# weiquan/salt

Hardware: AMD Instinct MI355X
Metric: Mreads/s aligned (100 bp SE, GRCh38+snp144) at 1/2/4/8 MI355X vs CPU ref (higher is better)
Workload: dtype u32; 1 GPU; GRCh38-scale synthetic (SURVEY 8d config 3 = BASELINE configs[2]): 3100000000 bp genome in 24 contigs, 14800000 SNPs, k=21, 1000000 x 100 bp SE reads per GPU per step, 8 distinct resident batches rotated, inputs and results resident in HBM; read_len=100, distinct_batches=8, options=default (-s 50 -m 1000, overlap = k), streams_per_gpu=4

## Files before the change

include/salt_gpu.h:

```cpp
#ifndef SALT_GPU_H
#define SALT_GPU_H
#include <stdint.h>
#include <stddef.h>

#ifdef __cplusplus
extern "C" {
#endif

#define SALT_OK              0
#define SALT_E_INVAL        -1
#define SALT_E_HIP          -2
#define SALT_E_NOMEM        -3
#define SALT_E_INDEX        -4
#define SALT_E_CAPACITY     -5
#define SALT_E_DATA         -6

#define SALT_MAX_READ_LEN   512
#define SALT_MAX_HITS       5
#define SALT_MAX_LOCATE     1024
#define SALT_MAX_SEED_SLOTS 512
#define SALT_MAX_CIGAR_OPS  64

typedef struct {
    uint32_t c_primary, c_L2[5], c_seq_len, c_bwt_size;
    const uint32_t *c_bwt;
    uint32_t c_sa_intv, c_n_sa;
    const uint32_t *c_sa;
    uint32_t lkt_len, lkt_n;
    const uint32_t *lkt;
    uint32_t r_text_len, r_inv_sa0, r_cum[6], r_bwt_words;
    const uint32_t *r_bwt;
    uint32_t r_occ_words;   const uint32_t *r_occ;
    uint32_t r_major_words; const uint32_t *r_major;
    uint32_t r_n_sa;        const uint32_t *r_sa;
    uint32_t ref_len;
    const uint32_t *ref;
    int32_t  l_seed;
} salt_host_index_t;

typedef struct {
    int32_t  l_seed;
    int32_t  l_overlap;
    uint32_t max_seed;
    uint32_t max_locate;
    int32_t  max_hits;
    int32_t  seed_only_ref;
    int32_t  collect_counters;
    int32_t  reserved;
} salt_aln_opt_t;

typedef struct {
    uint32_t pos;
    uint8_t  n_diff, is_gap;
    uint16_t strand;
} salt_hit_t;

typedef struct {
    uint32_t pos;
    uint8_t  strand, n_diff, is_gap, mapq;
    int32_t  b0, b1;
    uint16_t seq_start, seq_end;
    uint8_t  n_hits[2];
    uint8_t  n_cigar;
    uint8_t  skipped;
    salt_hit_t hits[2][SALT_MAX_HITS];
    uint8_t  hit_n_cigar[SALT_MAX_HITS];
    uint8_t  pad[3];
    uint16_t cigar[SALT_MAX_CIGAR_OPS];
    uint16_t hit_cigar[SALT_MAX_HITS][SALT_MAX_CIGAR_OPS];
} salt_result_t;

enum { SALT_CTR_LKT, SALT_CTR_OCC_C, SALT_CTR_OCC_R, SALT_CTR_SA_C, SALT_CTR_SA_R, SALT_CTR_VERIFY,
       SALT_CTR_VERIFY_WORDS, SALT_CTR_LV, SALT_CTR_READS, SALT_CTR_BASES, SALT_CTR_LOCI,
       SALT_CTR_T_LOAD, SALT_CTR_T_GATHER, SALT_CTR_T_LOCATE, SALT_CTR_T_SORT, SALT_CTR_T_DEDUP, SALT_CTR_T_VERIFY,
       SALT_CTR_T_SCAN, SALT_CTR_T_GAP, SALT_CTR_T_TAIL, SALT_CTR_HEAVY_READS, SALT_CTR_X0, SALT_CTR_X1, SALT_CTR_X2, SALT_CTR_X3,
       SALT_CTR_LT_SEEDS, SALT_CTR_LT_LOCATE, SALT_CTR_LT_SORT, SALT_CTR_LT_VERIFY, SALT_CTR_LT_OUT, SALT_CTR_LT_SAMPLES,
       SALT_CTR_MAX_HEAVY, SALT_CTR_MAX_GAPFIN,
       SALT_CTR_D_WLKT, SALT_CTR_D_COCC_SEED, SALT_CTR_D_ROCC_SEED, SALT_CTR_D_SA_SEED, SALT_CTR_D_TEXT_SEED,
       SALT_CTR_D_SA_LIGHT, SALT_CTR_D_VERIFY_LIGHT, SALT_CTR_D_OUT_LIGHT, SALT_CTR_D_SA_HEAVY, SALT_CTR_D_VERIFY_HEAVY, SALT_CTR_D_OUT_HEAVY,
       SALT_CTR_D_CTX_ROWS, SALT_CTR_D_CTX_REJECTED,
       SALT_CTR_N };

typedef struct salt_gpu_index salt_gpu_index_t;
typedef struct salt_gpu_ws    salt_gpu_ws_t;

int  salt_gpu_index_attach(const salt_host_index_t *host, int device, salt_gpu_index_t **out);
void salt_gpu_index_detach(salt_gpu_index_t *ix);
int  salt_gpu_index_image(const salt_gpu_index_t *ix, void **dev_ptr, uint64_t *bytes);
int  salt_gpu_index_attach_image(void *dev_ptr, uint64_t bytes, int device, salt_gpu_index_t **out);
int  salt_gpu_index_image_compact(const salt_gpu_index_t *ix, void **dev_ptr, uint64_t *bytes);
int  salt_gpu_index_attach_compact(const void *dev_ptr, uint64_t bytes, int device, salt_gpu_index_t **out);
int  salt_gpu_index_replicate(salt_gpu_index_t *src, const int *devices, int n, salt_gpu_index_t **out);
int  salt_gpu_index_image_copy(const salt_gpu_index_t *ix, void *dst_dev_ptr, uint64_t dst_bytes);

int  salt_gpu_ws_create(salt_gpu_index_t *ix, uint32_t max_reads, uint64_t max_bases, salt_gpu_ws_t **out);
void salt_gpu_ws_destroy(salt_gpu_ws_t *ws);

int  salt_gpu_align_se(salt_gpu_ws_t *ws, const salt_aln_opt_t *opt, uint32_t n_reads,
                       const uint8_t *seqs, const uint32_t *offs, salt_result_t *results);

typedef struct { uint32_t min_tlen, max_tlen; } salt_pe_opt_t;
int  salt_gpu_index_set_pac(salt_gpu_index_t *ix, const uint8_t *pac, uint64_t l_pac);
int  salt_gpu_align_pe(salt_gpu_ws_t *ws, const salt_aln_opt_t *opt, const salt_pe_opt_t *pe, uint32_t n_pairs,
                       const uint8_t *seqs, const uint32_t *offs, salt_result_t *results);
int  salt_gpu_align_pe_resident(salt_gpu_ws_t *ws, const salt_aln_opt_t *opt, const salt_pe_opt_t *pe, uint32_t n_pairs,
                                uint32_t max_read_len, const void *d_seqs, const void *d_offs, void *d_results, void *hip_stream);
int  salt_gpu_ws_pe_overflow(salt_gpu_ws_t *ws, uint32_t *n);
int  salt_gpu_ws_pe_counts(salt_gpu_ws_t *ws, uint32_t out[8]);

typedef struct { int32_t print_xa_cigar, print_nm_md; const char *rg_id; } salt_text_opt_t;
int  salt_gpu_index_set_contigs(salt_gpu_index_t *ix, int32_t n, const int64_t *offsets, const char *const *names);
int  salt_gpu_align_pe_text(salt_gpu_ws_t *ws, const salt_aln_opt_t *opt, const salt_pe_opt_t *pe, const salt_text_opt_t *topt,
                            const char *fastq1, uint64_t n1_bytes, const char *fastq2, uint64_t n2_bytes,
                            const char **sam, uint64_t *sam_bytes, uint32_t *n_pairs);
int  salt_gpu_ws_reserve_text(salt_gpu_ws_t *ws, const salt_aln_opt_t *opt, uint64_t max_block_bytes, uint32_t est_reads, uint32_t max_read_len,
                              uint64_t est_sam_bytes, void *host_sam, uint64_t host_sam_bytes);
int  salt_gpu_align_se_text(salt_gpu_ws_t *ws, const salt_aln_opt_t *opt, const salt_text_opt_t *topt, const char *fastq, uint64_t n_bytes,
                            const char **sam, uint64_t *sam_bytes, uint32_t *n_reads);
int  salt_gpu_ws_set_sam_bgzf(salt_gpu_ws_t *ws, int on);
int  salt_gpu_ws_set_sam_bam(salt_gpu_ws_t *ws, int on);
int  salt_gpu_bgzf_deflate(int device, const void *text, uint64_t n_bytes, void *out, uint64_t out_cap, uint64_t *out_bytes);
int  salt_gpu_bgzf_inflate(int device, const void *bgzf, uint64_t n_bytes, void *out, uint64_t out_cap, uint64_t *out_bytes);
int  salt_gpu_ws_inflate_bgzf(salt_gpu_ws_t *ws, const void *blocks, uint64_t n_cbytes, uint32_t n_blocks, const uint32_t *c_off, const uint32_t *u_off);
int  salt_gpu_ws_text_peek(salt_gpu_ws_t *ws, uint64_t off, uint64_t n, void *dst);
int  salt_gpu_align_se_text_dev(salt_gpu_ws_t *ws, const salt_aln_opt_t *opt, const salt_text_opt_t *topt, uint64_t off, uint64_t n_bytes, int add_newline,
                                const char **sam, uint64_t *sam_bytes, uint32_t *n_reads);
int  salt_gpu_host_alloc(uint64_t bytes, void **ptr);
void salt_gpu_host_free(void *ptr);
int  salt_gpu_device_numa_node(int device, int *node);
int  salt_gpu_device_count(int *n);

int  salt_gpu_align_se_resident(salt_gpu_ws_t *ws, const salt_aln_opt_t *opt, uint32_t n_reads,
                                uint32_t max_read_len, const void *d_seqs, const void *d_offs,
                                void *d_results, void *hip_stream);

#define SALT_N_KERNELS 10
int  salt_gpu_ws_timing(salt_gpu_ws_t *ws, int enable);
int  salt_gpu_ws_kernel_ms(salt_gpu_ws_t *ws, double ms[SALT_N_KERNELS], uint32_t *n_calls);

int  salt_gpu_ws_heavy_reads(salt_gpu_ws_t *ws, uint32_t *ids, uint32_t cap, uint32_t *n);

int  salt_gpu_buffer_alloc(int device, uint64_t bytes, void **dev_ptr);
int  salt_gpu_buffer_free(int device, void *dev_ptr);
int  salt_gpu_buffer_equal(int device, const void *a, const void *b, uint64_t bytes, int *equal);

int  salt_gpu_diag_rule(uint32_t n_cases, const uint32_t *pos, const uint8_t *val, const uint32_t *offs, const uint32_t *bound_in,
                        uint32_t L, uint32_t ref_len, int mode, uint32_t *out);

int  salt_gpu_diag_verify(const uint32_t *ref_words, uint32_t ref_len, uint32_t n_cases, const uint8_t *seqs, const uint32_t *offs,
                          const uint32_t *cand, const uint32_t *cand_offs, int mode, uint8_t *out);

int  salt_gpu_ws_queue_counts(salt_gpu_ws_t *ws, uint32_t out[8]);

int  salt_gpu_ws_counters(salt_gpu_ws_t *ws, uint64_t out[SALT_CTR_N]);

int  salt_gpu_diag_lv(const uint32_t *ref_words, uint32_t ref_len, uint32_t n_cases, const uint32_t *pos,
                      const uint32_t *kdiff, const uint8_t *seqs, const uint32_t *offs, int32_t *out4, uint16_t *cigars);

int  salt_gpu_diag_ssw(uint32_t n_cases, const uint8_t *aware, const uint8_t *ref_syms, const uint32_t *ref_offs,
                       const uint8_t *codes, const uint32_t *read_offs, int32_t *out6, uint16_t *cigars, uint16_t *n_cigar);

typedef struct { uint32_t read, offset, pool; uint16_t tlen; uint8_t strand, k; } salt_polish_item_t;
typedef struct salt_gpu_polish salt_gpu_polish_t;
int  salt_gpu_polish_open(int device, const uint8_t *pac, uint64_t l_pac, salt_gpu_polish_t **out);
void salt_gpu_polish_close(salt_gpu_polish_t *p);
int  salt_gpu_polish_lv(salt_gpu_polish_t *p, const uint8_t *codes, const uint32_t *offs, uint32_t n_reads, const salt_polish_item_t *items,
                        uint32_t n_items, const uint8_t *pool, uint32_t pool_stride, uint32_t n_pool, int want_cigar,
                        int32_t *dist, uint16_t *cigars, uint8_t *n_cigar);

int  salt_gpu_polish_sw(salt_gpu_polish_t *p, const uint8_t *codes, const uint32_t *offs, uint32_t n_reads, const salt_polish_item_t *items,
                        uint32_t n_items, int want_cigar, int32_t *score, int32_t *read_span, uint16_t *cigars, uint16_t *n_cigar);

int  salt_gpu_suffix_array(int device, const uint8_t *text, uint64_t n, int bits, uint32_t *sa_out);
uint64_t salt_gpu_idx_c_bwt_words(uint64_t n);
int  salt_gpu_idx_build_c(int device, const uint8_t *text, uint64_t n, uint32_t sa_intv, uint32_t *primary, uint32_t L2[5],
                          uint32_t *bwt, uint32_t *sa, uint32_t *lkt, uint32_t lkt_len);
int  salt_gpu_idx_build_r(int device, const uint8_t *rtext, uint64_t n, const uint32_t *sharp_off, const uint32_t *sharp_hdr, uint64_t n_sharp,
                          uint32_t cum4, uint32_t *inv_sa0, uint32_t *code, uint64_t code_words, uint32_t *rsa);
const char *salt_gpu_idx_last_error(void);

const char *salt_gpu_last_error(void);
uint32_t    salt_gpu_result_size(void);

#ifdef __cplusplus
}
// ... 3 lines not shown
```

salt_amd/api.py:

```python
import ctypes
import os
from dataclasses import dataclass

import numpy as np

_HERE = os.path.dirname(os.path.abspath(__file__))
LIB_DIR = os.path.join(_HERE, "lib")

MAX_HITS = 5
MAX_CIGAR_OPS = 64
CTR_NAMES = ["lkt", "occ_c", "occ_r", "sa_c", "sa_r", "verify", "verify_words", "lv", "reads", "bases", "loci",
             "t_load", "t_gather", "t_locate", "t_sort", "t_dedup", "t_verify", "t_scan", "t_gap", "t_tail", "heavy_reads", "x0", "x1", "x2", "x3",
             "lt_seeds", "lt_locate", "lt_sort", "lt_verify", "lt_out", "lt_samples", "max_heavy", "max_gapfin",
             "d_wlkt", "d_cocc_seed", "d_rocc_seed", "d_sa_seed", "d_text_seed", "d_sa_light", "d_verify_light", "d_out_light",
             "d_sa_heavy", "d_verify_heavy", "d_out_heavy", "d_ctx_rows", "d_ctx_rejected"]


class SaltError(RuntimeError):
    pass


HIT_DTYPE = np.dtype([("pos", "<u4"), ("n_diff", "u1"), ("is_gap", "u1"), ("strand", "<u2")])
RESULT_DTYPE = np.dtype([
    ("pos", "<u4"), ("strand", "u1"), ("n_diff", "u1"), ("is_gap", "u1"), ("mapq", "u1"),
# ... 411 lines not shown

    def image(self):
        p, n = ctypes.c_void_p(), ctypes.c_uint64()
        _gpu_check(gpu_lib().salt_gpu_index_image(self._ix, ctypes.byref(p), ctypes.byref(n)))
        return p.value, n.value

    def pe_counts(self):
        out = (ctypes.c_uint32 * 8)()
        _gpu_check(gpu_lib().salt_gpu_ws_pe_counts(self._ws, out))
        return list(out)

    def image_compact(self):
        p, n = ctypes.c_void_p(), ctypes.c_uint64()
        _gpu_check(gpu_lib().salt_gpu_index_image_compact(self._ix, ctypes.byref(p), ctypes.byref(n)))
        return p.value, n.value

    def image_copy(self, dst_ptr, dst_bytes):
        _gpu_check(gpu_lib().salt_gpu_index_image_copy(self._ix, dst_ptr, dst_bytes))

    def timing(self, enable=True):
        _gpu_check(gpu_lib().salt_gpu_ws_timing(self._ws, 1 if enable else 0))

    def kernel_ms(self):
        ms = (ctypes.c_double * len(KERNELS))()
        n = ctypes.c_uint32()
        _gpu_check(gpu_lib().salt_gpu_ws_kernel_ms(self._ws, ms, ctypes.byref(n)))
        return dict(zip(KERNELS, list(ms))), n.value

    def queue_counts(self):
        out = (ctypes.c_uint32 * 8)()
        _gpu_check(gpu_lib().salt_gpu_ws_queue_counts(self._ws, out))
        return list(out)

    def heavy_reads(self):
        n = ctypes.c_uint32()
        ids = np.zeros(self.max_reads, dtype=np.uint32)
        _gpu_check(gpu_lib().salt_gpu_ws_heavy_reads(self._ws, ids.ctypes.data, len(ids), ctypes.byref(n)))
        return ids[:n.value]

    def alnse_core1(self, opt, seqs, offs):
        seqs = np.ascontiguousarray(seqs, dtype=np.uint8)
        offs = np.ascontiguousarray(offs, dtype=np.uint32)
        n = len(offs) - 1
        res = np.zeros(n, dtype=RESULT_DTYPE)
        co = opt._c()
        done = 0
        while done < n:
            m = min(self.max_reads, n - done)
            while m > 1 and int(offs[done + m]) - int(offs[done]) > self.max_bases:
                m //= 2
            o = (offs[done:done + m + 1] - offs[done]).astype(np.uint32)
            s = seqs[int(offs[done]):int(offs[done + m])]
            _gpu_check(gpu_lib().salt_gpu_align_se(self._ws, ctypes.byref(co), m, s.ctypes.data, o.ctypes.data,
                                                   res[done:].ctypes.data))
            done += m
        return res

    def alnpe_core1(self, opt, index, seqs, offs):
        seqs = np.ascontiguousarray(seqs, dtype=np.uint8)
        offs = np.ascontiguousarray(offs, dtype=np.uint32)
        n = len(offs) - 1
        if n % 2:
            raise SaltError("paired end needs an even number of reads")
        lib = gpu_lib()
        if not getattr(self, "_pac_set", False):
            pac, l_pac = index.pac()
            _gpu_check(lib.salt_gpu_index_set_pac(self._ix, pac, l_pac))
            self._pac_set = True
        res = np.zeros(n, dtype=RESULT_DTYPE)
        co, pe = opt._c(), opt._pe()
        done = 0
        cap = self.max_reads & ~1
        while done < n:
            m = min(cap, n - done)
            while m > 2 and int(offs[done + m]) - int(offs[done]) > self.max_bases:
                m = (m // 2) & ~1
            o = (offs[done:done + m + 1] - offs[done]).astype(np.uint32)
            s = seqs[int(offs[done]):int(offs[done + m])]
            _gpu_check(lib.salt_gpu_align_pe(self._ws, ctypes.byref(co), ctypes.byref(pe), m // 2, s.ctypes.data,
                                             o.ctypes.data, res[done:].ctypes.data))
            done += m
        return res

    def set_pac(self, index):
        if not getattr(self, "_pac_set", False):
            pac, l_pac = index.pac()
            _gpu_check(gpu_lib().salt_gpu_index_set_pac(self._ix, pac, l_pac))
            self._pac_set = True

    def set_contigs(self, index):
        cs = index.contigs()
        offs = (ctypes.c_int64 * len(cs))(*[c[0] for c in cs])
        names = (ctypes.c_char_p * len(cs))(*[c[2] for c in cs])
        lib = gpu_lib()
        lib.salt_gpu_index_set_contigs.argtypes = [ctypes.c_void_p, ctypes.c_int32, ctypes.c_void_p, ctypes.c_void_p]
        _gpu_check(lib.salt_gpu_index_set_contigs(self._ix, len(cs), offs, names))

    def set_sam_bgzf(self, on=True):
        gpu_lib().salt_gpu_ws_set_sam_bgzf.argtypes = [ctypes.c_void_p, ctypes.c_int]
        _gpu_check(gpu_lib().salt_gpu_ws_set_sam_bgzf(self._ws, 1 if on else 0))

    def set_sam_bam(self, on=True):
        gpu_lib().salt_gpu_ws_set_sam_bam.argtypes = [ctypes.c_void_p, ctypes.c_int]
        _gpu_check(gpu_lib().salt_gpu_ws_set_sam_bam(self._ws, 1 if on else 0))

    def align_se_text(self, opt, fastq):
        lib = gpu_lib()
        lib.salt_gpu_align_se_text.argtypes = [ctypes.c_void_p, ctypes.POINTER(_AlnOpt), ctypes.POINTER(_TextOpt), ctypes.c_char_p, ctypes.c_uint64,
                                               ctypes.POINTER(ctypes.c_void_p), ctypes.POINTER(ctypes.c_uint64), ctypes.POINTER(ctypes.c_uint32)]
        fastq = bytes(fastq)
        co, to = opt._c(), _TextOpt(opt.print_xa_cigar, opt.print_nm_md, opt.rg_id.encode() if opt.rg_id else None)
        out, n, reads = ctypes.c_void_p(), ctypes.c_uint64(), ctypes.c_uint32()
        _gpu_check(lib.salt_gpu_align_se_text(self._ws, ctypes.byref(co), ctypes.byref(to), fastq, len(fastq), ctypes.byref(out), ctypes.byref(n), ctypes.byref(reads)))
        return ctypes.string_at(out.value, n.value) if n.value else b"", reads.value

    def align_pe_text(self, opt, index, fastq1, fastq2):
        lib = gpu_lib()
        lib.salt_gpu_align_pe_text.argtypes = [ctypes.c_void_p, ctypes.POINTER(_AlnOpt), ctypes.POINTER(_PeOpt), ctypes.POINTER(_TextOpt), ctypes.c_char_p,
                                               ctypes.c_uint64, ctypes.c_char_p, ctypes.c_uint64, ctypes.POINTER(ctypes.c_void_p), ctypes.POINTER(ctypes.c_uint64),
                                               ctypes.POINTER(ctypes.c_uint32)]
        self.set_pac(index)
        fastq1, fastq2 = bytes(fastq1), bytes(fastq2)
        co, pe, to = opt._c(), opt._pe(), _TextOpt(opt.print_xa_cigar, opt.print_nm_md, opt.rg_id.encode() if opt.rg_id else None)
        out, n, pairs = ctypes.c_void_p(), ctypes.c_uint64(), ctypes.c_uint32()
        _gpu_check(lib.salt_gpu_align_pe_text(self._ws, ctypes.byref(co), ctypes.byref(pe), ctypes.byref(to), fastq1, len(fastq1), fastq2, len(fastq2),
                                              ctypes.byref(out), ctypes.byref(n), ctypes.byref(pairs)))
        return ctypes.string_at(out.value, n.value) if n.value else b"", pairs.value

    def align_pe_resident(self, opt, index, n_pairs, max_read_len, d_seqs, d_offs, d_results, stream=0):
        lib = gpu_lib()
        self.set_pac(index)
        co, pe = opt._c(), opt._pe()
        _gpu_check(lib.salt_gpu_align_pe_resident(self._ws, ctypes.byref(co), ctypes.byref(pe), n_pairs, max_read_len, d_seqs, d_offs,
                                                  d_results, stream))

    def align_resident(self, opt, n_reads, max_read_len, d_seqs, d_offs, d_results, stream=0):
        co = opt._c()
        _gpu_check(gpu_lib().salt_gpu_align_se_resident(self._ws, ctypes.byref(co), n_reads, max_read_len, d_seqs, d_offs,
                                                        d_results, stream))

    def counters(self):
        out = (ctypes.c_uint64 * len(CTR_NAMES))()
        _gpu_check(gpu_lib().salt_gpu_ws_counters(self._ws, out))
        return dict(zip(CTR_NAMES, [int(x) for x in out]))

    def fork(self, max_reads=None, max_bases=None):
        other = GpuAligner.__new__(GpuAligner)
        other._ix, other._owns_ix = self._ix, False
        other._ws = ctypes.c_void_p()
        other.max_reads = max_reads or self.max_reads
        other.max_bases = max_bases or self.max_bases
        other.device = self.device
        other._pac_set = getattr(self, "_pac_set", False)
        _gpu_check(gpu_lib().salt_gpu_ws_create(self._ix, other.max_reads, other.max_bases, ctypes.byref(other._ws)))
        return other

    def close(self):
        lib = gpu_lib()
        if self._ws:
            lib.salt_gpu_ws_destroy(self._ws)
            self._ws = None
        if self._ix and getattr(self, "_owns_ix", True):
            lib.salt_gpu_index_detach(self._ix)
        self._ix = None


# ... 62 lines not shown
```

salt_amd/csrc/salt_align.hip:

```cpp
#include "salt_device.h"
#include "salt_kernels.h"

namespace salt {

#define WSYNC() do { __builtin_amdgcn_fence(__ATOMIC_ACQ_REL, "wavefront"); __builtin_amdgcn_wave_barrier(); \
                     __builtin_amdgcn_fence(__ATOMIC_ACQ_REL, "wavefront"); } while (0)

static constexpr int MAXL = SALT_MAX_READ_LEN;
static constexpr int SLOTS = SALT_MAX_SEED_SLOTS;
static constexpr int MAXLOC = SALT_MAX_LOCATE;
static constexpr int LVK = 31;
static_assert(offsetof(salt_result_t, strand) == 4 && offsetof(salt_result_t, mapq) == 7 && offsetof(salt_result_t, b0) == 8 &&
              offsetof(salt_result_t, b1) == 12 && offsetof(salt_result_t, seq_start) == 16 && offsetof(salt_result_t, seq_end) == 18 &&
              offsetof(salt_result_t, n_hits) == 20 && offsetof(salt_result_t, n_cigar) == 22 && offsetof(salt_result_t, skipped) == 23 &&
              offsetof(salt_result_t, hits) == 24 && sizeof(salt_hit_t) == 8, "salt_result_t header layout");
static constexpr int NHIT = 6;
__device__ __forceinline__ uint32_t mapq_quot(uint32_t x, uint32_t b0)
{
    const uint32_t v = 255u * x;
    return b0 == 1u ? v : b0 == 2u ? v / 2u : b0 == 3u ? v / 3u : v / b0;
}
static constexpr uint32_t INF = 255;

__device__ __forceinline__ uint32_t lane_id() { return threadIdx.x & 63u; }
// ... 282 lines not shown
            return true;
        }
        if (head_n || p0 < m) { row = dead; w.ph = WK_IDLE; return true; }
        w.p0 = p0; w.ph = WK_TEXT;
        return false;
    }
    if (!R && w.ph == WK_TEXT) {
        const uint32_t m = (uint32_t)w.i + 1u;
        bool ok = true;
        for (uint32_t done = 0, piece = 0; done < m && ok; ++piece) {
            const uint32_t cnt = (m - done) > 16u ? 16u : (m - done);
            const uint32_t r0 = s + (m - done - cnt), t0 = w.p0 - done - cnt;
            const uint32_t rel = r0 - (c.wb << 4), rr = rel & 15u;
            const uint64_t vr = rel < 16 ? (((uint64_t)c.w0 << 32) | c.w1) : (((uint64_t)c.w1 << 32) | c.w2);
            const uint32_t xr = (uint32_t)((vr >> (64 - 2 * rr - 2 * cnt)) & ((1ull << (2 * cnt)) - 1ull));
            const uint32_t tr = t0 & 15u;
            const uint64_t vt = piece == 0 ? (((uint64_t)ld.s[0] << 32) | ld.s[1]) : (((uint64_t)ld.t[0] << 32) | ld.t[1]);
            n_aux += 1u << 21;
            const uint32_t xt = (uint32_t)((vt >> (64 - 2 * tr - 2 * cnt)) & ((1ull << (2 * cnt)) - 1ull));
            ok = xr == xt;
            done += cnt;
        }
        row = ok ? make_uint4(w.p0 - m, w.p0 - m, s, 2) : dead; w.ph = WK_IDLE;
        return true;
    }
    const bool head = w.ph == WK_HEAD;
    const uint32_t pos = walk_pos(c, w);
    const bool inr = walk_pos_inreg(c, pos);
    const bool isn = inr ? seed_is_n(c, pos) : ((ld.t[0] >> (31 - (pos & 31u))) & 1u) != 0;
    const uint4 stop = head ? dead : make_uint4(w.k, w.l, s - w.ext, 1);
    if (isn && !(R && !head)) { row = stop; w.ph = WK_IDLE; return true; }
    const uint32_t b = isn ? 4u : inr ? seed_base2(c, pos) : (ld.s[0] >> (30 - 2 * (pos & 15u))) & 3u;
    uint32_t ok, ol;
    if (R) n_occ += r_occ2_eval(ix, ROcc2{ ROccBlk{ ld.a[0], ld.a[1], ld.a[2], ld.a[3] }, ROccBlk{ ld.b[0], ld.b[1], ld.b[2], ld.b[3] } }, w.k, w.l + 1u, b, ok, ol);
    else n_occ += c_occ2_eval(ix, COcc2{ ld.a[0], ld.a[1], ld.b[0], ld.b[1] }, w.k - 1u, w.l, b, ok, ol);
    if (ok + 1u > ol) { row = stop; w.ph = WK_IDLE; return true; }
    { const uint32_t first = R ? pick5(ix.r_cum, b) : pick4(ix.c_L2, b); w.k = first + ok + 1u; w.l = first + ol; }
    if (head) {
        if (--w.i >= 0) { if (!R && c.inreg && sp.resolve_unique && w.k == w.l) w.ph = WK_SA; return false; }
    } else ++w.ext;
    return walk_enter_ext(sp, c, w, row);
}

template <bool R>
__device__ __forceinline__ uint4 seed_walk_rest(const IndexView &ix, const SeedParams &sp, const SeedCtx c, uint32_t k, uint32_t l, int i_top,
                                                uint32_t &n_occ, uint32_t &n_aux)
{
    Walk w; uint4 row = make_uint4(1, 0, 0, 0);
    bool done = seed_walk_begin<R>(sp, c, k, l, i_top, w, row);
    while (!done) { const WalkLoads ld = walk_fetch(seed_walk_issue<R>(ix, sp, c, w)); done = seed_walk_finish<R>(ix, sp, c, w, ld, row, n_occ, n_aux); }
    return row;
}
__device__ __forceinline__ uint4 seed_c_rest(const IndexView &ix, const SeedParams &sp, const SeedCtx c, uint32_t kc, uint32_t lc, int i_top,
                                             uint32_t &n_occ_c, uint32_t &n_aux)
{
    return seed_walk_rest<false>(ix, sp, c, kc, lc, i_top, n_occ_c, n_aux);
}
__device__ __forceinline__ uint4 seed_r_rest(const IndexView &ix, const SeedParams &sp, const SeedCtx c, uint32_t kr, uint32_t lr, int i_top,
                                             uint32_t &n_occ_r)
{
    uint32_t n_aux = 0;
    return seed_walk_rest<true>(ix, sp, c, kr, lr, i_top, n_occ_r, n_aux);
}

static constexpr uint32_t WQ_SEG = 64, WQ_STRIDE = 64;
static constexpr uint32_t WQ_REC = 2;
__global__ void __launch_bounds__(256) __attribute__((amdgpu_waves_per_eu(8, 8)))
k_seed(IndexView ix, SeedParams sp, const uint32_t *__restrict__ tb,
       uint4 *__restrict__ sai_c, uint4 *__restrict__ sai_r, uint4 *__restrict__ wq, uint32_t *__restrict__ wq_cnt, uint32_t wq_seg_cap,
       unsigned long long *__restrict__ ctr)
{
    __shared__ uint32_t q_n[2], q_base[2];
    const uint64_t item = (uint64_t)blockIdx.x * blockDim.x + threadIdx.x, n_items = (uint64_t)sp.n_reads * 2u * sp.spr;
    const uint64_t lt = (1ull << lane_id()) - 1ull;
    uint32_t n_lkt = 0, n_occ_c = 0, n_occ_r = 0;
    if (threadIdx.x < 2) { q_n[threadIdx.x] = 0; q_base[threadIdx.x] = 0; }
    __syncthreads();
    bool pend_c = false, pend_r = false;
    uint32_t pk_c = 0, pl_c = 0, pk_r = 0, pl_r = 0, at_r = 0, at_c = 0;
    uint32_t cw0 = 0, cw1 = 0, cw2 = 0, cn0 = 0, cn1 = 0;
    if (item < n_items) {
        const SeedCtx c = seed_ctx(sp, tb, (uint32_t)item, ix.r_lkt_len);
        cw0 = c.w0; cw1 = c.w1; cw2 = c.w2; cn0 = c.n0; cn1 = c.n1;
        uint4 oc = make_uint4(1, 0, 0, 0), orr = make_uint4(1, 0, 0, 0);
        if (seed_valid(c)) {
            const uint32_t e = c.s + c.k - 1, W = c.W;
            uint32_t x = 0; bool has_n = false;
            const uint32_t a0 = e - W + 1;
            if (c.inreg) {
                const uint32_t rel = a0 - (c.wb << 4), rr = rel & 15u;
                const uint64_t v = rel < 16 ? (((uint64_t)c.w0 << 32) | c.w1) : rel < 32 ? (((uint64_t)c.w1 << 32) | c.w2) : ((uint64_t)c.w2 << 32);
                x = (uint32_t)((v >> (64 - 2 * rr - 2 * W)) & ((1ull << (2 * W)) - 1ull));
                const uint32_t reln = a0 - (c.nb << 5);
                const uint64_t vn = ((uint64_t)c.n0 << 32) | c.n1;
                has_n = ((vn >> (64 - reln - W)) & ((1ull << W) - 1ull)) != 0;
            } else {
                for (uint32_t t = 0; t < W; ++t) { has_n |= seed_is_n(c, a0 + t); x = (x << 2) | seed_base2(c, a0 + t); }
            }
            if (!has_n) {
                const uint4 v = ix.wlkt[2 * (uint64_t)x];
                const uint4 u = ix.wlkt[2 * (uint64_t)x + 1];
                ++n_lkt;
                const int i_top = (int)(c.k - W) - 1;
                if (v.x <= v.y) {
                    const uint32_t m = c.k - W;
                    if (v.x == v.y && c.inreg && sp.resolve_unique && m >= 1 && m <= 16) {
                        const uint32_t rel = c.s - (c.wb << 4), rr = rel & 15u;
                        const uint64_t vr = rel < 16 ? (((uint64_t)c.w0 << 32) | c.w1) : (((uint64_t)c.w1 << 32) | c.w2);
                        const uint32_t mk = m == 16 ? 0xFFFFFFFFu : ((1u << (2 * m)) - 1u);
                        const uint32_t xr = (uint32_t)(vr >> (64 - 2 * rr - 2 * m)) & mk;
                        const uint32_t reln2 = c.s - (c.nb << 5);
                        const uint64_t vn2 = ((uint64_t)c.n0 << 32) | c.n1;
                        const bool head_n = ((vn2 >> (64 - reln2 - m)) & ((1ull << m) - 1ull)) != 0;
                        if (!head_n && u.x >= m && xr == (u.y & mk)) oc = make_uint4(u.x - m, u.x - m, c.s, 2);
                    }
                    else if (v.y == v.x + 1u && c.inreg && sp.resolve_unique && m >= 1 && m <= 16) {
                        const uint32_t rel = c.s - (c.wb << 4), rr = rel & 15u;
                        const uint64_t vr = rel < 16 ? (((uint64_t)c.w0 << 32) | c.w1) : (((uint64_t)c.w1 << 32) | c.w2);
                        const uint32_t mk = m == 16 ? 0xFFFFFFFFu : ((1u << (2 * m)) - 1u);
                        const uint32_t xr = (uint32_t)(vr >> (64 - 2 * rr - 2 * m)) & mk;
                        const uint32_t reln2 = c.s - (c.nb << 5);
                        const uint64_t vn2 = ((uint64_t)c.n0 << 32) | c.n1;
                        const bool head_n = ((vn2 >> (64 - reln2 - m)) & ((1ull << m) - 1ull)) != 0;
                        const bool ok0 = !head_n && u.x >= m && xr == (u.y & mk), ok1 = !head_n && u.z >= m && xr == (u.w & mk);
                        if (ok0 && ok1) { pend_c = true; pk_c = v.x; pl_c = v.y; }
                        else if (ok0) oc = make_uint4(u.x - m, u.x - m, c.s, 2);
                        else if (ok1) oc = make_uint4(u.z - m, u.z - m, c.s, 2);
                    }
                    else {
                        Walk w;
                        if (!seed_walk_begin<false>(sp, c, v.x, v.y, i_top, w, oc)) { pend_c = true; pk_c = v.x; pl_c = v.y; }
                    }
                }
                if (!sp.seed_only_ref) {
                    if (v.z <= v.w) { pend_r = true; pk_r = v.z; pl_r = v.w; }
                }
            }
        }
        sai_c[item] = oc;
        sai_r[item] = orr;
    }
    {
        const uint64_t mr = __ballot(pend_r), mc = __ballot(pend_c);
        uint32_t br = 0, bc = 0;
        if (lane_id() == 0) { if (mr) br = atomicAdd(&q_n[0], (uint32_t)__popcll(mr)); if (mc) bc = atomicAdd(&q_n[1], (uint32_t)__popcll(mc)); }
        br = (uint32_t)__shfl((int)br, 0); bc = (uint32_t)__shfl((int)bc, 0);
        at_r = br + (uint32_t)__popcll(mr & lt); at_c = bc + (uint32_t)__popcll(mc & lt);
    }
    __syncthreads();
    const uint32_t seg = blockIdx.x & (WQ_SEG - 1u);
    if (threadIdx.x < 2 && q_n[threadIdx.x]) q_base[threadIdx.x] = atomicAdd(&wq_cnt[(threadIdx.x * WQ_SEG + seg) * WQ_STRIDE], q_n[threadIdx.x]);
    __syncthreads();
    if (pend_r) {
        uint4 *rec = wq + ((size_t)seg * wq_seg_cap + q_base[0] + at_r) * WQ_REC;
        rec[0] = make_uint4((uint32_t)item, pk_r, pl_r, cn0); rec[1] = make_uint4(cw0, cw1, cw2, cn1);
    }
    if (pend_c) {
        uint4 *rec = wq + (((size_t)WQ_SEG + seg) * wq_seg_cap + q_base[1] + at_c) * WQ_REC;
        rec[0] = make_uint4((uint32_t)item, pk_c, pl_c, cn0); rec[1] = make_uint4(cw0, cw1, cw2, cn1);
    }
    if (ctr) {
        for (int o = 32; o > 0; o >>= 1) {
            n_lkt += __shfl_down(n_lkt, o); n_occ_c += __shfl_down(n_occ_c, o); n_occ_r += __shfl_down(n_occ_r, o);
        }
        if (lane_id() == 0) {
            atomicAdd(ctr + SALT_CTR_LKT, n_lkt & 1023u); atomicAdd(ctr + SALT_CTR_OCC_C, n_occ_c); atomicAdd(ctr + SALT_CTR_OCC_R, n_occ_r);
            atomicAdd(ctr + SALT_CTR_D_WLKT, n_lkt & 1023u); atomicAdd(ctr + SALT_CTR_D_COCC_SEED, n_occ_c); atomicAdd(ctr + SALT_CTR_D_ROCC_SEED, n_occ_r);
            atomicAdd(ctr + SALT_CTR_D_SA_SEED, (n_lkt >> 10) & 2047u); atomicAdd(ctr + SALT_CTR_D_TEXT_SEED, n_lkt >> 21);
        }
    }
}

__global__ void __launch_bounds__(256) __attribute__((amdgpu_waves_per_eu(4, 4)))
k_seed_walk(IndexView ix, SeedParams sp, const uint32_t *__restrict__ tb, uint4 *__restrict__ sai_c, uint4 *__restrict__ sai_r,
            const uint4 *__restrict__ wq, const uint32_t *__restrict__ wq_cnt, uint32_t wq_seg_cap, uint32_t r_first, unsigned long long *__restrict__ ctr)
{
    const uint32_t seg = blockIdx.x & (WQ_SEG - 1u);
    const uint32_t wv = (blockIdx.x / WQ_SEG) * 4u + (uint32_t)__builtin_amdgcn_readfirstlane((int)(threadIdx.x >> 6)), nw = (gridDim.x / WQ_SEG) * 4u;
    const uint64_t lt = (1ull << lane_id()) - 1ull;
    const uint32_t la = r_first ? 0u : 1u, lb = la ^ 1u;
    const uint32_t na = wq_cnt[(la * WQ_SEG + seg) * WQ_STRIDE], nb = wq_cnt[(lb * WQ_SEG + seg) * WQ_STRIDE];
    const uint32_t a0 = (uint32_t)((uint64_t)na * wv / nw), a1 = (uint32_t)((uint64_t)na * (wv + 1u) / nw);
    const uint32_t b0 = (uint32_t)((uint64_t)nb * wv / nw), b1 = (uint32_t)((uint64_t)nb * (wv + 1u) / nw);
    const uint4 *qa = wq + (((size_t)la * WQ_SEG + seg) * wq_seg_cap + a0) * WQ_REC, *qb = wq + (((size_t)lb * WQ_SEG + seg) * wq_seg_cap + b0) * WQ_REC;
    const uint32_t tot_a = a1 - a0, tot = tot_a + (b1 - b0);
    const int i_top = (int)((uint32_t)sp.l_seed - ix.r_lkt_len) - 1;
    uint32_t n_aux = 0, n_sa = 0, n_text = 0, n_occ_c = 0, n_occ_r = 0;
    Walk w; w.ph = WK_IDLE; w.k = w.l = w.ext = w.p0 = 0; w.i = 0;
    SeedCtx c = seed_ctx_geom(sp, tb, 0, ix.r_lkt_len);
    uint32_t item = 0, cur = 0;
    bool is_r = false;
    const uint4 *qp = qa;
    for (;;) {
        const uint64_t idle = __ballot(w.ph == WK_IDLE);
        if (cur >= tot && idle == ~0ull) break;
        if (cur < tot) {
            const uint32_t t = cur + (uint32_t)__popcll(idle & lt);
            if (w.ph == WK_IDLE && t < tot) {
                const bool in_a = t < tot_a;
                qp = in_a ? qa + (size_t)t * WQ_REC : qb + (size_t)(t - tot_a) * WQ_REC; is_r = (in_a ? la : lb) == 0u; w.ph = WK_REC;
            }
            const uint32_t nx = cur + (uint32_t)__popcll(idle);
            cur = nx < tot ? nx : tot;
        }
        WalkReq q = walk_req_none();
        if (w.ph == WK_REC) { q.pa = qp; q.na = WQ_REC; }
        else if (w.ph != WK_IDLE) q = is_r ? seed_walk_issue<true>(ix, sp, c, w) : seed_walk_issue<false>(ix, sp, c, w);
        const WalkLoads ld = walk_fetch(q);
        bool done = false;
        uint4 row = make_uint4(1, 0, 0, 0);
        if (w.ph == WK_REC) {
            item = ld.a[0].x;
            c = seed_ctx_geom(sp, tb, item, ix.r_lkt_len);
            c.w0 = ld.a[1].x; c.w1 = ld.a[1].y; c.w2 = ld.a[1].z; c.n0 = ld.a[0].w; c.n1 = ld.a[1].w;
            done = is_r ? seed_walk_begin<true>(sp, c, ld.a[0].y, ld.a[0].z, i_top, w, row) : seed_walk_begin<false>(sp, c, ld.a[0].y, ld.a[0].z, i_top, w, row);
        } else if (w.ph != WK_IDLE) {
            done = is_r ? seed_walk_finish<true>(ix, sp, c, w, ld, row, n_occ_r, n_aux) : seed_walk_finish<false>(ix, sp, c, w, ld, row, n_occ_c, n_aux);
        }
        if (done && row.x <= row.y) (is_r ? sai_r : sai_c)[item] = row;
        n_sa += (n_aux >> 10) & 2047u; n_text += n_aux >> 21; n_aux = 0;
    }
    if (ctr) {
        for (int o = 32; o > 0; o >>= 1) { n_sa += __shfl_down(n_sa, o); n_text += __shfl_down(n_text, o); n_occ_c += __shfl_down(n_occ_c, o); n_occ_r += __shfl_down(n_occ_r, o); }
        if (lane_id() == 0) {
            atomicAdd(ctr + SALT_CTR_OCC_C, n_occ_c); atomicAdd(ctr + SALT_CTR_OCC_R, n_occ_r);
            atomicAdd(ctr + SALT_CTR_D_COCC_SEED, n_occ_c); atomicAdd(ctr + SALT_CTR_D_ROCC_SEED, n_occ_r);
            atomicAdd(ctr + SALT_CTR_D_SA_SEED, n_sa); atomicAdd(ctr + SALT_CTR_D_TEXT_SEED, n_text);
        }
    }
}

template <int NS> struct SaiListsT { uint32_t sp[2][NS], ep[2][NS], off[2][NS]; };
struct SaiLists { uint32_t *sp[2], *ep[2], *off[2]; };
template <int NS> __device__ __forceinline__ SaiLists sai_ref(SaiListsT<NS> &a) { return SaiLists{ { a.sp[0], a.sp[1] }, { a.ep[0], a.ep[1] }, { a.off[0], a.off[1] } }; }
struct LvTables { short L[LVK][64]; char A[LVK][64]; };
static constexpr int LLV_K = 12;
static constexpr int LLV_TW = 22;
static constexpr int LLV_W = 2 * LLV_K + 3;
static constexpr int LLV_N = 64;
struct LaneLv { uint32_t T[LLV_N * LLV_TW]; uint8_t rows[2][LLV_W][LLV_N]; };
struct LvBytes { uint8_t T[MAXL + 4 + 64]; uint8_t P[MAXL + 64]; };
template <int NS, bool LLV>
struct WaveLdsT {
    static constexpr bool HAS_LLV = LLV;
    static constexpr int N_SLOTS = NS;
    uint32_t pm[2][MAXL / 8];
    union U { SaiListsT<NS> sai; typename std::conditional<LLV, LaneLv, uint32_t>::type llv; LvBytes lvb; } u;
    uint8_t  cand_e[MAXLOC];
    uint32_t loci[MAXLOC];
    uint32_t hit_pos[2][NHIT];
    uint8_t  hit_nd[2][NHIT], hit_gap[2][NHIT];
    uint16_t cig[SALT_MAX_CIGAR_OPS];
    int      n_cig;
    alignas(8) uint8_t cargs[128];
};
typedef WaveLdsT<SLOTS, true> WaveLds;
typedef WaveLdsT<32, false> WaveLdsSmall;
typedef WaveLdsT<1, false> WaveLdsCigar;

struct Sai { uint32_t sp, ep, off; };
__device__ __forceinline__ Sai sai_get(const SaiLists &s, int w, int i) { return Sai{ s.sp[w][i], s.ep[w][i], s.off[w][i] }; }
__device__ __forceinline__ void sai_set(SaiLists &s, int w, int i, Sai v) { s.sp[w][i] = v.sp; s.ep[w][i] = v.ep; s.off[w][i] = v.off; }
__device__ __forceinline__ bool sai_ltv(Sai a, Sai b) { return a.ep - a.sp < b.ep - b.sp; }
__device__ __forceinline__ bool sai_lt(const SaiLists &s, int w, int i, int j) { return sai_ltv(sai_get(s, w, i), sai_get(s, w, j)); }
__device__ __forceinline__ void sai_swap(SaiLists &s, int w, int i, int j) { Sai a = sai_get(s, w, i), b = sai_get(s, w, j); sai_set(s, w, i, b); sai_set(s, w, j, a); }

__device__ void sai_insertsort(SaiLists &s, int w, int lo, int hi)
{
    for (int i = lo + 1; i < hi; ++i)
        for (int j = i; j > lo && sai_lt(s, w, j, j - 1); --j) sai_swap(s, w, j, j - 1);
}

__device__ void sai_combsort(SaiLists &s, int w, int base, int n)
{
    const double shrink = 1.2473309501039786540366528676643;
    int gap = n; bool do_swap;
    do {
        if (gap > 2) { gap = (int)(gap / shrink); if (gap == 9 || gap == 10) gap = 11; }
        do_swap = false;
        for (int i = 0; i < n - gap; ++i)
            if (sai_lt(s, w, base + i + gap, base + i)) { sai_swap(s, w, base + i, base + i + gap); do_swap = true; }
    } while (do_swap || gap > 2);
    if (gap != 1) sai_insertsort(s, w, base, base + n);
}

__device__ __attribute__((noinline)) void sai_introsort(SaiLists &s, int w, int n)
{
    if (n < 1) return;
    if (n == 2) { if (sai_lt(s, w, 1, 0)) sai_swap(s, w, 0, 1); return; }
    int d; for (d = 2; (1 << d) < n; ++d) { }
    d <<= 1;
    int st_l[24], st_r[24], st_d[24], top = 0;
    int lo = 0, hi = n - 1;
    for (;;) {
        if (lo < hi) {
            if (--d == 0) { sai_combsort(s, w, lo, hi - lo + 1); hi = lo; continue; }
            int i = lo, j = hi, k = i + ((j - i) >> 1) + 1;
            if (sai_lt(s, w, k, i)) { if (sai_lt(s, w, k, j)) k = j; }
            else k = sai_lt(s, w, j, i) ? i : j;
            Sai rp = sai_get(s, w, k);
            if (k != hi) sai_swap(s, w, k, hi);
            for (;;) {
                do ++i; while (sai_ltv(sai_get(s, w, i), rp));
                do --j; while (i <= j && sai_ltv(rp, sai_get(s, w, j)));
                if (j <= i) break;
                sai_swap(s, w, i, j);
            }
            sai_swap(s, w, i, hi);
            if (i - lo > hi - i) {
                if (i - lo > 16 && top < 24) { st_l[top] = lo; st_r[top] = i - 1; st_d[top] = d; ++top; }
                lo = hi - i > 16 ? i + 1 : hi;
            } else {
                if (hi - i > 16 && top < 24) { st_l[top] = i + 1; st_r[top] = hi; st_d[top] = d; ++top; }
                hi = i - lo > 16 ? i - 1 : lo;
            }
        } else {
            if (top == 0) { sai_insertsort(s, w, 0, n); return; }
            --top; lo = st_l[top]; hi = st_r[top]; d = st_d[top];
        }
    }
}

__device__ void sort_loci(uint32_t *a, uint32_t n)
{
    if (n < 2) return;
    uint32_t P = 2; while (P < n) P <<= 1;
    for (uint32_t i = n + lane_id(); i < P; i += 64) a[i] = 0xFFFFFFFFu;
    WSYNC();
    for (uint32_t k = 2; k <= P; k <<= 1) {
        for (uint32_t j = k >> 1; j > 0; j >>= 1) {
            for (uint32_t t = lane_id(); t < (P >> 1); t += 64) {
                uint32_t i = ((t & ~(j - 1)) << 1) | (t & (j - 1));
                uint32_t p = i | j;
                uint32_t x = a[i], y = a[p];
                bool up = (i & k) == 0;
                if ((x > y) == up) { a[i] = y; a[p] = x; }
            }
            WSYNC();
        }
    }
}

__device__ __forceinline__ uint32_t dedup_loci(uint32_t *loci, uint32_t n, bool gap_mode, uint32_t L, uint32_t ref_len)
{
    const uint32_t lane = lane_id();
    const uint64_t lt = (1ull << lane) - 1ull;
    uint32_t n_out = 0;
    for (uint32_t b = 0; b < n; b += 64) {
        uint32_t i = b + lane;
        bool keep = false; uint32_t pos = 0;
        if (i < n) {
            pos = loci[i];
            bool dup = i > 0 && loci[i - 1] == pos;
            bool out = gap_mode ? (pos + L + 4 >= ref_len) : (pos >= ref_len);
            keep = !dup && !out;
        }
        uint64_t m = __ballot(keep);
        WSYNC();
        if (keep) loci[n_out + (uint32_t)__popcll(m & lt)] = pos;
        n_out += (uint32_t)__popcll(m);
        WSYNC();
    }
    return n_out;
}

struct CandStats { uint32_t n_cand, n_sa_c, n_sa_r, n_loci; uint32_t in_lds; uint32_t n_ctx_rej, n_ctx_rows; };
struct CandArgs {
    const uint32_t *c_sa, *r_pos; const uint4 *sai_c, *sai_r;
    uint32_t ref_len, spr, max_locate, r, L; int strand; bool gap_mode; unsigned long long *phase;
    uint32_t *loci; uint32_t loci_cap; int pe;
    bool finish;
    const uint4 *r_ctx;
    const uint4 *c_ctx; uint32_t ctx_k;
};

__device__ __forceinline__ CtxRead ctx_read(const uint32_t *pm, uint32_t L, uint32_t off, uint32_t ctx_k)
{
    const int p = ctx_face(lane_id(), off, ctx_a_start(ctx_k));
    const bool v = p >= 0 && p < (int)L;
    const uint32_t nib = v ? (pm[(uint32_t)p >> 3] >> (4u * ((uint32_t)p & 7u))) & 15u : 0u;
    CtxRead rd;
    rd.lo = __ballot(v && ctx_nib_lo(nib));
    rd.hi = __ballot(v && ctx_nib_hi(nib));
    rd.use = __ballot(v && ctx_nib_use(nib));
    return rd;
}
template <bool PE, bool GL, class W>
__device__ __attribute__((noinline)) CandStats build_candidates(W &w)
{
    const CandArgs a = *reinterpret_cast<const CandArgs *>(w.cargs);
    const uint32_t lane = lane_id();
    const uint64_t lt = (1ull << lane) - 1ull;
    const uint32_t L = a.L, r = a.r; const int strand = a.strand; const bool gap_mode = a.gap_mode;
    const gp_u32x4 sai_c = as_global(a.sai_c), sai_r = as_global(a.sai_r);
    struct { gp_u32 c_sa, r_pos; uint32_t ref_len; } ix = { as_global(a.c_sa), as_global(a.r_pos), a.ref_len };
    struct { uint32_t spr, max_locate; } ap = { a.spr, a.max_locate };
    uint32_t n_sa_c = 0, n_sa_r = 0, n_loci_out = 0;
    constexpr bool glob = GL;
    uint32_t *loci = glob ? a.loci : w.loci;
    PhaseClock pc(a.phase);
    const uint64_t base_item = ((uint64_t)r * 2u + (uint32_t)strand) * ap.spr;
    uint32_t n_list[2] = { 0, 0 };
    const uint32_t cap_total = PE ? a.loci_cap : ap.max_locate;
    uint32_t rows = 0;
    for (uint32_t b = 0; b < ap.spr; b += 64) {
        const uint32_t slot = b + lane;
        uint4 v2[2] = { make_uint4(1, 0, 0, 0), make_uint4(1, 0, 0, 0) };
        if (slot < ap.spr) {
            const u32x4_t tc = sai_c[base_item + slot], tr = sai_r[base_item + slot];
            v2[0] = make_uint4(tc.x, tc.y, tc.z, tc.w); v2[1] = make_uint4(tr.x, tr.y, tr.z, tr.w);
        }
#pragma unroll
        for (int which = 0; which < 2; ++which) {
            const uint4 v = v2[which];
            const uint32_t n = n_list[which];
            uint64_t m = __ballot(v.w != 0);
            uint32_t sz = 0;
            if (v.w) {
                uint32_t at = n + (uint32_t)__popcll(m & lt); w.u.sai.sp[which][at] = v.x; w.u.sai.ep[which][at] = v.y; w.u.sai.off[which][at] = v.z | (v.w == 2 ? 0x80000000u : 0u);
                sz = v.y - v.x + 1u;
                if (which == 1 && !PE) { uint32_t skip = sz / 0x40000u; if (skip > 1) sz = (sz + skip - 1) / skip; }
                if (PE && which == 0 && sz > ap.max_locate + 1u) sz = ap.max_locate + 1u;
                if (PE && which == 1 && v.y - v.x > ap.max_locate) sz = (v.y - v.x) / ((v.y - v.x) / ap.max_locate) + 1u;
                if (sz > cap_total) sz = cap_total + 1u;
            }
            for (int o = 32; o > 0; o >>= 1) sz += (uint32_t)__shfl_xor((int)sz, o);
            rows = rows + sz > cap_total ? cap_total + 1u : rows + sz;
            n_list[which] = n + (uint32_t)__popcll(m);
        }
    }
    WSYNC();
    if (rows > cap_total && lane < 2) { SaiLists sl = sai_ref(w.u.sai); sai_introsort(sl, (int)lane, (int)n_list[lane]); }
    const bool pe_in_lds = !glob || rows <= (uint32_t)MAXLOC;
    if (pe_in_lds) loci = w.loci;
    WSYNC();
    pc.stamp(SALT_CTR_T_GATHER);
    uint32_t n = 0, ns = 0, n_ctx_rows = 0;
    bool full = false;
    const gp_u32x4 c_ctx = as_global(a.c_ctx);
    const bool use_ctx = a.c_ctx != nullptr && !gap_mode;
    for (uint32_t i = 0; i < n_list[0] && !full; ++i) {
        const uint32_t sp = w.u.sai.sp[0][i], off = w.u.sai.off[0][i] & 0x7FFFFFFFu;
        const bool located = (w.u.sai.off[0][i] >> 31) != 0;
        uint32_t ep = w.u.sai.ep[0][i];
        if (PE && ep - sp > ap.max_locate) ep = sp + ap.max_locate;
        const bool ctx_here = use_ctx && !located;
        CtxRead rd = { 0, 0, 0 };
        if (ctx_here) rd = ctx_read(w.pm[strand], L, off, a.ctx_k);
        for (uint64_t j0 = sp; j0 <= ep && !full; j0 += 64) {
            pc.add(SALT_CTR_X0, 1);
            uint64_t j = j0 + lane;
            bool in = j <= ep, keep = false, rej = false;
            uint32_t pos = 0;
            if (in) {
                uint32_t sa;
                if (ctx_here) { const u32x4_t rc = c_ctx[j]; sa = rc.x; rej = ctx_reject(make_uint4(rc.x, rc.y, rc.z, rc.w), rd, 3u); }
                else sa = located ? (uint32_t)j : ix.c_sa[j];
                pos = sa - off; keep = !(pos + L > ix.ref_len);
            }
            uint64_t m = __ballot(keep);
            uint32_t rank = (uint32_t)__popcll(m & lt);
            const bool st = keep && !rej && n + rank < cap_total;
            const uint64_t ms = __ballot(st);
            if (st) loci[ns + (uint32_t)__popcll(ms & lt)] = pos;
            ns += (uint32_t)__popcll(ms);
            uint32_t tot = (uint32_t)__popcll(m);
            if (n + tot >= cap_total) {
                uint64_t last = m;
                uint32_t need = cap_total - n;
                for (uint32_t q = 1; q < need; ++q) last &= last - 1;
                uint32_t stop_lane = (uint32_t)__ffsll((long long)last) - 1;
                n_sa_c += stop_lane + 1; if (ctx_here) n_ctx_rows += stop_lane + 1;
                n = cap_total; full = true;
            } else { n += tot; const uint32_t looked = (uint32_t)__popcll(__ballot(in)); n_sa_c += looked; if (ctx_here) n_ctx_rows += looked; }
        }
    }
    pc.stamp(SALT_CTR_X2);
    const gp_u32x4 r_ctx = as_global(a.r_ctx);
    const bool use_rctx = use_ctx && a.r_ctx != nullptr;
    for (uint32_t i = 0; i < n_list[1] && !full; ++i) {
        const uint32_t sp = w.u.sai.sp[1][i], ep = w.u.sai.ep[1][i], off = w.u.sai.off[1][i];
        uint32_t skip = (ep + 1 - sp) / 0x40000u;
        if ((int)skip <= 0) skip = 1;
        if (PE) skip = ep - sp > ap.max_locate ? (ep - sp) / ap.max_locate : 1;
        CtxRead rd = { 0, 0, 0 };
        if (use_rctx) rd = ctx_read(w.pm[strand], L, off, a.ctx_k);
        for (uint64_t j0 = sp; j0 <= ep && !full; j0 += 64ull * skip) {
            pc.add(SALT_CTR_X1, 1);
            uint64_t j = j0 + (uint64_t)lane * skip;
            bool in = j <= ep, keep = false, rej = false;
            uint32_t pos = 0;
            if (in) {
                uint32_t rp;
// ... 516 lines not shown
{
    const uint32_t w0 = pos >> 3, sh = (pos & 7u) * 4u, nwt = (tl + 7) >> 3;
    uint32_t wv[LLV_TW + 1];
#pragma unroll
    for (int j = 0; j <= LLV_TW; ++j) wv[j] = (uint32_t)j <= nwt ? ref[w0 + (uint32_t)j] : 0u;
#pragma unroll
    for (int j = 0; j < LLV_TW; ++j) {
        uint32_t word = 0;
        if ((uint32_t)j < nwt) {
            word = __funnelshift_r(wv[j], wv[j + 1], sh);
            const uint32_t rem = tl - (uint32_t)j * 8;
            if (rem < 8) word &= (1u << (4 * rem)) - 1u;
        }
        T[j] = word;
    }
}

__device__ __forceinline__ uint32_t store_gap_list(const uint32_t *loci, uint32_t n, uint32_t L, uint32_t ref_len, uint32_t *__restrict__ dst)
{
    const uint32_t lane = lane_id();
    const uint64_t lt = (1ull << lane) - 1ull;
    uint32_t n_out = 0;
    for (uint32_t b = 0; b < n; b += 64) {
        const uint32_t i = b + lane;
        const uint32_t pos = i < n ? loci[i] : 0u;
        const bool keep = i < n && !(pos + L + 4 >= ref_len);
        const uint64_t m = __ballot(keep);
        if (keep) dst[n_out + (uint32_t)__popcll(m & lt)] = pos;
        n_out += (uint32_t)__popcll(m);
    }
    return n_out;
}

template <bool PE, bool GL, class W>
__device__ __forceinline__ void align_general(const IndexView ix, const AlignParams ap, W &w, const uint32_t r,
                              const uint32_t *__restrict__ pm,
                              const uint4 *__restrict__ sai_c, const uint4 *__restrict__ sai_r,
                              salt_result_t *__restrict__ results, unsigned long long *__restrict__ ctr,
                              unsigned long long *phase, LvTables *lvtab, const GapBufs g, uint32_t *pe_loci, uint8_t *pe_cand)
{
    const uint32_t lane = lane_id();
    const uint64_t lt = (1ull << lane) - 1ull;
    const uint32_t *rec = pm + (uint64_t)r * ap.pg.pm_stride;
    const uint32_t L = rec[2 * ap.pg.nw8];
    salt_result_t *out = results + r;
    uint32_t c_sa_c = 0, c_sa_r = 0, c_verify = 0, c_vwords = 0, c_lv = 0, c_loci = 0, c_ctx_rej = 0, c_ctx_rows = 0;
    PhaseClock pc(phase);
    const uint64_t rt0 = phase ? __builtin_amdgcn_s_memrealtime() : 0;
    constexpr bool glob = GL;
    uint32_t *loci = glob ? pe_loci : w.loci;
    uint8_t *cand_e = glob ? pe_cand : w.cand_e;
    const uint32_t loci_cap = PE ? PE_LOCI_CAP : (uint32_t)MAXLOC;

    const uint32_t nw = (L + 7) >> 3;
    uint32_t n_amb = 0;
    for (uint32_t t = lane; t < 2 * nw; t += 64) {
        const uint32_t s = t >= nw, j = s ? t - nw : t;
        const uint32_t word = rec[s * ap.pg.nw8 + j];
        w.pm[s][j] = word;
        if (!s) n_amb += (uint32_t)__popc(word & (word >> 1) & (word >> 2) & (word >> 3) & 0x11111111u);
    }
    if (ap.max_amb < L) { for (int o = 32; o > 0; o >>= 1) n_amb += (uint32_t)__shfl_xor((int)n_amb, o); }
    else n_amb = 0;
    WSYNC();
    uint32_t q_pos = 0xFFFFFFFFu; uint32_t q_strand = 3, q_ndiff = 255, q_gap = 255;
    const bool too_short = L < (uint32_t)ap.l_seed;
    if (n_amb > ap.max_amb) {
        if (lane == 0) {
            out->pos = q_pos; out->strand = 3; out->n_diff = 255; out->is_gap = 255; out->mapq = 0;
            out->b0 = -1; out->b1 = -1; out->seq_start = 0; out->seq_end = (uint16_t)(L - 1);
            out->n_hits[0] = out->n_hits[1] = 0; out->n_cigar = 0; out->skipped = 1;
        }
        return;
    }
    pc.stamp(SALT_CTR_T_LOAD);
    uint32_t bound = 3;
    bool found[2] = { false, false };
    uint32_t n_hits_s[2] = { 0, 0 };
    uint32_t a0[2] = { 0, 0 };
    uint32_t n_cand_nogap = 0, n_loc_s[2] = { 0, 0 };
    if (!too_short)
    for (int strand = 0; strand < 2; ++strand) {
        pc.stamp(SALT_CTR_T_SCAN);
        const CandStats cs = build_candidates_call<PE, GL>(CandArgs{ ix.c_sa, ix.r_pos, sai_c, sai_r, ix.ref_len, ap.spr, ap.max_locate, r, L, strand, false, phase, pe_loci, loci_cap, ap.pe, false, ix.r_ctx, ix.c_ctx, ix.ctx_k }, w);
        if (glob) { loci = cs.in_lds ? w.loci : pe_loci; cand_e = cs.in_lds ? w.cand_e : pe_cand; }
        pc.t = phase ? __builtin_amdgcn_s_memtime() : 0;
        const uint32_t n_loc = cs.n_cand; c_sa_c += cs.n_sa_c; c_sa_r += cs.n_sa_r; c_loci += cs.n_loci; c_ctx_rej += cs.n_ctx_rej; c_ctx_rows += cs.n_ctx_rows;
        uint32_t call_best_n = INF, call_best_pos = 0;
        if (SALT_DIAG_VAL(ap.heavy_stop) == 1) continue;
        auto verify_all = [&](uint32_t n) {
            if (L <= 120) verify_quads<8>(ix.ref, ix.ref_len, w.pm[strand], L, loci, n, cand_e);
            else if (L <= 248) verify_two_phase(ix.ref, ix.ref_len, w.pm[strand], L, loci, n, cand_e);
            else for (uint32_t i = lane; i < n; i += 64) cand_e[i] = (uint8_t)mismatch_capped(ix, w.pm[strand], L, loci[i]);
            WSYNC();
        };
        verify_all(n_loc);
        pc.stamp(SALT_CTR_T_VERIFY);
        if (SALT_DIAG_VAL(ap.heavy_stop) == 2) continue;
        {
            bool any = false; uint32_t bp = 0, bv = 0, nh = 0, a0s = 0;
            rule_unsorted<3, false>(loci, cand_e, n_loc, L, ix.ref_len, bound, any, bp, bv, nh, a0s, w.hit_pos[strand], w.hit_nd[strand]);
            if (any) {
                found[strand] = true; call_best_pos = bp; call_best_n = bv; n_hits_s[strand] = nh; a0[strand] = a0s;
                if (lane < NHIT) w.hit_gap[strand][lane] = 0;
            }
        }
        const uint32_t n_cand = n_loc;
        c_verify += n_loc; n_cand_nogap += n_loc + cs.n_ctx_rej; n_loc_s[strand] = n_loc;
        for (uint32_t b = lane; b < n_cand; b += 64) c_vwords += ((loci[b] & 7u) + L + 7) >> 3;
        if (found[strand]) { q_pos = call_best_pos; q_ndiff = call_best_n; q_gap = 0; q_strand = (uint32_t)strand; }
        WSYNC();
        pc.stamp(SALT_CTR_T_SCAN);
    }

    if (SALT_DIAG_VAL(ap.heavy_stop)) return;
    if (!too_short && !found[0] && !found[1]) {
        int maxd = PE ? 3 : (int)(L / 10);
        const int gap_k0 = maxd;
        const bool lanes_fit = gap_k0 <= LLV_K && L + 4 <= 8u * (LLV_TW - 1);
        if (lanes_fit && g.cap && n_cand_nogap > 0) {
            uint32_t slot = 0;
            if (lane == 0) slot = atomicAdd(&g.gctl->gap_slots, 1u);
            slot = (uint32_t)__shfl((int)slot, 0);
            if (slot < g.cap) {
                uint32_t ns[2], off[2];
                bool ok = true;
                for (int k = 0; k < 2 && ok; ++k) {
                    const int strand = 1 - k;
                    uint32_t n = n_loc_s[1];
                    if (strand == 0 || ix.c_ctx != nullptr) {
                        WSYNC();
                        const CandStats cs = build_candidates_call<PE, GL>(CandArgs{ ix.c_sa, ix.r_pos, sai_c, sai_r, ix.ref_len, ap.spr, ap.max_locate, r, L, strand, true, phase, pe_loci, loci_cap, ap.pe, false, nullptr, nullptr, 0 }, w);
                        if (glob) { loci = cs.in_lds ? w.loci : pe_loci; cand_e = cs.in_lds ? w.cand_e : pe_cand; }
                        c_sa_c += cs.n_sa_c; c_sa_r += cs.n_sa_r; c_loci += cs.n_loci;
                        n = cs.n_cand;
                    }
                    if (n > 1024u * LLV_N) { ok = false; break; }
                    uint32_t o = 0;
                    if (lane == 0) o = atomicAdd(&g.gctl->pool_used, n);
                    o = (uint32_t)__shfl((int)o, 0);
                    ok = (uint64_t)o + n <= g.pool;
                    if (ok) for (uint32_t i = lane; i < n; i += 64) g.gloci[o + i] = loci[i];
                    ns[strand] = n; off[strand] = o;
                }
                const uint32_t ch0 = ok ? (ns[0] + LLV_N - 1) / LLV_N : 0, ch1 = ok ? (ns[1] + LLV_N - 1) / LLV_N : 0;
                uint32_t base = 0;
                if (ok && lane == 0) base = atomicAdd(&g.gctl->gap_items, ch0 + ch1);
                base = (uint32_t)__shfl((int)base, 0);
                ok = ok && (uint64_t)base + ch0 + ch1 <= g.items_cap;
                if (lane == 0) {
                    g.gq[slot] = ok ? r : 0xFFFFFFFFu;
                    g.gn[2 * slot] = ok ? ns[0] : 0; g.gn[2 * slot + 1] = ok ? ns[1] : 0;
                    g.goff[2 * slot] = off[0]; g.goff[2 * slot + 1] = off[1];
                }
                if (ok) {
                    for (uint32_t c = lane; c < ch0 + ch1; c += 64) g.gitems[base + c] = (slot << 11) | (c >= ch0 ? (0x400u | (c - ch0)) : c);
                    if (ctr) {
                        for (int o2 = 32; o2 > 0; o2 >>= 1) c_vwords += __shfl_down(c_vwords, o2);
                        if (lane == 0) {
                            atomicAdd(ctr + SALT_CTR_SA_C, c_sa_c); atomicAdd(ctr + SALT_CTR_SA_R, c_sa_r);
                            atomicAdd(ctr + SALT_CTR_VERIFY, c_verify); atomicAdd(ctr + SALT_CTR_VERIFY_WORDS, c_vwords);
                            atomicAdd(ctr + SALT_CTR_LV, ns[0] + ns[1]); atomicAdd(ctr + SALT_CTR_READS, 1ull);
                            atomicAdd(ctr + SALT_CTR_BASES, L); atomicAdd(ctr + SALT_CTR_LOCI, c_loci);
                            atomicAdd(ctr + SALT_CTR_D_SA_HEAVY, c_sa_c + c_sa_r);
                            atomicAdd(ctr + SALT_CTR_D_VERIFY_HEAVY, c_verify * (L <= 248 ? 4u : (((L + 7) >> 3) + 4u) / 4u));
                            atomicAdd(ctr + SALT_CTR_D_OUT_HEAVY, 5u * (ns[0] + ns[1]) + 16u);
                            if (ix.c_ctx) { atomicAdd(ctr + SALT_CTR_D_CTX_ROWS, c_ctx_rows); atomicAdd(ctr + SALT_CTR_D_CTX_REJECTED, c_ctx_rej); }
                        }
                    }
                    return;
                }
                WSYNC();
            }
        }
        if constexpr (!W::HAS_LLV) {
            if (lanes_fit && n_cand_nogap > 0) {
                if (lane == 0) g.ovq[atomicAdd(&g.gctl->ovq_count, 1u)] = r;
                return;
            }
        }
        for (int strand = 0; strand < 2; ++strand) {
            pc.stamp(SALT_CTR_T_GAP);
            const CandStats cs = build_candidates_call<PE, GL>(CandArgs{ ix.c_sa, ix.r_pos, sai_c, sai_r, ix.ref_len, ap.spr, ap.max_locate, r, L, strand, true, phase, pe_loci, loci_cap, ap.pe, true, nullptr, nullptr, 0 }, w);
            if (glob) { loci = cs.in_lds ? w.loci : pe_loci; cand_e = cs.in_lds ? w.cand_e : pe_cand; }
            pc.t = phase ? __builtin_amdgcn_s_memtime() : 0;
            const uint32_t n_cand = cs.n_cand; c_sa_c += cs.n_sa_c; c_sa_r += cs.n_sa_r; c_loci += cs.n_loci;
            bool any = false;
            const bool lanes_ok = lanes_fit && W::HAS_LLV;
            if constexpr (W::HAS_LLV) if (lanes_ok) {
                const int k0 = gap_k0;
                for (uint32_t b = 0; b < n_cand; b += LLV_N) {
                    WSYNC();
                    const uint32_t i = b + lane;
                    bool act = false;
                    if (lane < LLV_N && i < n_cand) {
                        const uint32_t pos = loci[i];
                        act = !(pos > ix.ref_len || pos + L + 4 > ix.ref_len);
                        if (act) lane_text(ix.ref, w.u.llv.T + lane * LLV_TW, pos, L + 4);
                    }
                    const uint32_t e = lv_lanes(w.u.llv, w.pm[strand], (int)L, (int)L + 4, k0, act);
                    if (lane < LLV_N && i < n_cand) cand_e[i] = (uint8_t)e;
                }
                WSYNC();
            }
            for (uint32_t i = 0; i < n_cand; ++i) {
                uint32_t pos = loci[i];
                int e = -1;
                if (lanes_ok) { const uint32_t ev = cand_e[i]; e = (ev != 255 && (int)ev <= maxd) ? (int)ev : -1; }
                else if (!(pos > ix.ref_len || pos + L + 4 > ix.ref_len)) {
                    lv_unpack(ix.ref, w, strand, L, pos);
                    int dd;
                    e = lv_wave(w.u.lvb.T, (int)L + 4, w.u.lvb.P, (int)L, maxd, nullptr, dd);
                    WSYNC();
                }
                ++c_lv;
                if (e >= 0) {
                    if (e < maxd || !any) { maxd = e; q_gap = 1; q_ndiff = (uint32_t)e; q_strand = (uint32_t)strand; q_pos = pos; }
                    if (n_hits_s[strand] < NHIT && lane == 0) {
                        uint32_t h = n_hits_s[strand];
                        w.hit_pos[strand][h] = pos; w.hit_nd[strand][h] = (uint8_t)e; w.hit_gap[strand][h] = 1;
                    }
                    if (n_hits_s[strand] == 0) a0[strand] = (uint32_t)e;
                    if (n_hits_s[strand] < NHIT) ++n_hits_s[strand];
                    any = true;
                }
            }
            found[strand] = any;
            WSYNC();
        }
    }
    WSYNC();
    pc.stamp(SALT_CTR_T_GAP);

    int b0 = (int)q_ndiff, b1 = 100000, tot = 0;
    uint32_t nh[2] = { 0, 0 };
    uint32_t sel_idx[2][SALT_MAX_HITS];
    for (int s = 0; s < 2 && tot < ap.max_hits; ++s) {
        for (uint32_t j = 0; j < n_hits_s[s]; ++j) {
            uint32_t p = w.hit_pos[s][j];
            if (p == 0xFFFFFFFFu || p == q_pos) continue;
            if (a0[s] <= q_ndiff) {
                if ((int)a0[s] <= b1) b1 = (int)a0[s];
                if (nh[s] < SALT_MAX_HITS) sel_idx[s][nh[s]] = j;
                ++nh[s]; ++tot;
            }
            if (tot == ap.max_hits) break;
        }
    }
    uint32_t mapq = 0;
    if (b0 != 0) {
        uint32_t x = (uint32_t)(b0 > b1 ? b0 - b1 : b1 - b0);
        uint64_t q = mapq_quot(x, (uint32_t)b0);
        mapq = q < 254 ? (uint32_t)q : 254u;
    }
    if (lane == 0) {
        out->pos = q_pos; out->strand = (uint8_t)q_strand; out->n_diff = (uint8_t)q_ndiff; out->is_gap = (uint8_t)q_gap;
        out->mapq = (uint8_t)mapq; out->b0 = b0; out->b1 = b1; out->seq_start = 0; out->seq_end = (uint16_t)(L - 1);
        out->n_hits[0] = (uint8_t)nh[0]; out->n_hits[1] = (uint8_t)nh[1]; out->skipped = 0;
        for (int s = 0; s < 2; ++s)
            for (uint32_t j = 0; j < nh[s]; ++j) {
                uint32_t h = sel_idx[s][j];
                out->hits[s][j].pos = w.hit_pos[s][h]; out->hits[s][j].n_diff = w.hit_nd[s][h];
                out->hits[s][j].is_gap = w.hit_gap[s][h]; out->hits[s][j].strand = (uint16_t)s;
            }
    }
    if (q_pos != 0xFFFFFFFFu) {
// ... 264 lines not shown
{
    const uint32_t s = (r >> 2) & (QUEUE_RANGES - 1u);
    qseg[(size_t)s * qseg_cap(n_reads) + atomicAdd(&ranges[s].push, 1u)] = r;
}
__global__ void __launch_bounds__(256)
k_queue_pack(const uint32_t *__restrict__ qseg, const QueueRange *__restrict__ ranges, uint32_t n_reads, uint32_t *__restrict__ queue, SeCtl *__restrict__ ctl)
{
    __shared__ uint32_t base_s, cnt_s;
    if (threadIdx.x == 0) {
        uint32_t base = 0, total = 0;
        for (uint32_t s = 0; s < QUEUE_RANGES; ++s) { const uint32_t c = ranges[s].push; if (s < blockIdx.x) base += c; total += c; }
        base_s = base; cnt_s = ranges[blockIdx.x].push;
        if (blockIdx.x == 0) ctl->light_queued = total;
    }
    __syncthreads();
    const uint32_t *src = qseg + (size_t)blockIdx.x * qseg_cap(n_reads);
    for (uint32_t i = threadIdx.x; i < cnt_s; i += 256) queue[base_s + i] = src[i];
}

static constexpr int LT_SLOTS = 16;
static constexpr int LT_LOCI = 128;
static constexpr int LT_MAXL = 160;

struct LightLds {
    uint32_t pm[2][LT_MAXL / 8];
    uint32_t sp[4][LT_SLOTS], off[4][LT_SLOTS];
    uint32_t pre[4][LT_SLOTS + 1];
    uint32_t loci[2][LT_LOCI];
    uint32_t hit_pos[2][NHIT];
    uint8_t  hit_nd[2][NHIT];
    uint8_t  val[2][LT_LOCI];
};

static constexpr int LT_WAVES = 2;
__global__ void __launch_bounds__(64 * LT_WAVES) __attribute__((amdgpu_waves_per_eu(8, 8)))
k_light(IndexView ix, AlignParams ap, const uint32_t *__restrict__ pm,
        const uint4 *__restrict__ sai_c, const uint4 *__restrict__ sai_r, salt_result_t *__restrict__ results,
        uint32_t *__restrict__ queue , QueueRange *__restrict__ ranges, unsigned long long *__restrict__ ctr)
{
    __shared__ LightLds w_all[LT_WAVES];
    LightLds &w = w_all[threadIdx.x >> 6];
    const uint32_t lane = lane_id();
    const uint64_t lt = (1ull << lane) - 1ull;
    const uint32_t r = __builtin_amdgcn_readfirstlane(blockIdx.x * LT_WAVES + (threadIdx.x >> 6));
    if (r >= ap.n_reads) return;
    const uint32_t *rec = pm + (uint64_t)r * ap.pg.pm_stride;
    const uint32_t L = rec[2 * ap.pg.nw8];
    bool heavy = L > LT_MAXL || L < (uint32_t)ap.l_seed || ap.spr > LT_SLOTS || ap.max_locate < 2 * 64;
    uint32_t c_sa_c = 0, c_sa_r = 0, c_verify = 0, c_vwords = 0, c_loci = 0;
    const bool prof = ctr && (r & 127u) == 0;
    uint64_t tp = prof ? __builtin_amdgcn_s_memtime() : 0;
    auto stamp = [&](int slot) {
        if (!prof) return;
        const uint64_t n = __builtin_amdgcn_s_memtime();
        if (lane == 0) atomicAdd(ctr + slot, (unsigned long long)(n - tp));
        tp = n;
    };

    if (!heavy) {
        const uint32_t nw = (L + 7) >> 3;
        uint32_t n_amb = 0;
        if (lane < 2 * nw) {
            const uint32_t s = lane >= nw, j = s ? lane - nw : lane;
            const uint32_t word = rec[s * ap.pg.nw8 + j];
            w.pm[s][j] = word;
            if (!s) n_amb = (uint32_t)__popc(word & (word >> 1) & (word >> 2) & (word >> 3) & 0x11111111u);
        }
        if (ap.max_amb < L)
            for (int o = 32; o > 0; o >>= 1) n_amb += (uint32_t)__shfl_xor((int)n_amb, o);
        if (n_amb > ap.max_amb) {
            if (lane == 0) {
                salt_result_t *out = results + r;
                out->pos = 0xFFFFFFFFu; out->strand = 3; out->n_diff = 255; out->is_gap = 255; out->mapq = 0;
                out->b0 = -1; out->b1 = -1; out->seq_start = 0; out->seq_end = (uint16_t)(L - 1);
                out->n_hits[0] = out->n_hits[1] = 0; out->n_cigar = 0; out->skipped = 1;
            }
            return;
        }
        uint32_t tot[4] = { 0, 0, 0, 0 };
        bool small = false;
        {
            const uint32_t l = lane >> 4, slot = lane & 15u;
            uint4 v = make_uint4(1, 0, 0, 0);
            if (slot < ap.spr) v = ((l & 1) ? sai_r : sai_c)[((uint64_t)r * 2u + (l >> 1)) * ap.spr + slot];
            uint32_t sz = v.w ? v.y - v.x + 1u : 0u;
            if (sz > 65u) sz = 65u;
            uint32_t inc = sz;
            for (int o = 1; o < 16; o <<= 1) { const uint32_t t = (uint32_t)__shfl_up((int)inc, o, 16); if (slot >= (uint32_t)o) inc += t; }
            for (int q = 0; q < 4; ++q) tot[q] = (uint32_t)__builtin_amdgcn_readlane((int)inc, 16 * q + 15);
            small = tot[0] <= 16 && tot[1] <= 16 && tot[2] <= 16 && tot[3] <= 16;
            if (small) {
                for (uint32_t k2 = 0; k2 < sz; ++k2) { w.sp[l][inc - sz + k2] = v.x + k2; w.off[l][inc - sz + k2] = v.z | (v.w == 2 ? 0x80000000u : 0u); }
            } else {
                w.sp[l][slot] = v.x; w.off[l][slot] = v.z | (v.w == 2 ? 0x80000000u : 0u);
                w.pre[l][slot + 1] = inc;
                if (slot == 0) w.pre[l][0] = 0;
            }
        }
        WSYNC();
        stamp(SALT_CTR_LT_SEEDS);
        for (int l = 0; l < 4; ++l) heavy |= tot[l] > 64;
        if (ap.dbg_stop == 1) { if (lane == 0) results[r].pos = tot[0] + tot[1] + tot[2] + tot[3] + w.pm[0][0] + w.pm[1][1]; return; }
        if (!heavy) {
            uint32_t n_s[2];
            if (small) {
                const uint32_t l = lane >> 4, x = lane & 15u;
                const uint32_t tl = l == 0 ? tot[0] : l == 1 ? tot[1] : l == 2 ? tot[2] : tot[3];
                bool keep = false; uint32_t p = 0;
                if (x < tl) {
                    const uint32_t j = w.sp[l][x], of = w.off[l][x];
                    p = ((of >> 31) ? j : (l & 1) ? ix.r_pos[j] : ix.c_sa[j]) - (of & 0x7FFFFFFFu);
                    keep = (l & 1) ? !(p > ix.ref_len || p + L > ix.ref_len) : !(p + L > ix.ref_len);
                }
                stamp(SALT_CTR_LT_LOCATE);
                if (ap.dbg_stop == 2) { if (__ballot(p == 12345u) == 1) results[r].pos = p; return; }
                const uint64_t km = __ballot(keep);
                const uint32_t s = lane >> 5, ms = (uint32_t)(km >> (32 * s));
                WSYNC();
                if (keep) w.loci[s][(uint32_t)__popc(ms & ((1u << (lane & 31u)) - 1u))] = p;
                n_s[0] = (uint32_t)__popc((uint32_t)km); n_s[1] = (uint32_t)__popc((uint32_t)(km >> 32));
                c_sa_c += tot[0] + tot[2]; c_sa_r += tot[1] + tot[3]; c_loci += n_s[0] + n_s[1];
            } else {
            uint32_t pos4[4]; bool keep4[4];
            for (int l = 0; l < 4; ++l) {
                keep4[l] = false; pos4[l] = 0;
                if (lane < tot[l]) {
                    uint32_t i = 0;
                    while (w.pre[l][i + 1] <= lane) ++i;
                    const uint32_t j = w.sp[l][i] + (lane - w.pre[l][i]), of = w.off[l][i];
                    const uint32_t p = ((of >> 31) ? j : (l & 1) ? ix.r_pos[j] : ix.c_sa[j]) - (of & 0x7FFFFFFFu);
                    pos4[l] = p;
                    keep4[l] = (l & 1) ? !(p > ix.ref_len || p + L > ix.ref_len) : !(p + L > ix.ref_len);
                }
            }
            stamp(SALT_CTR_LT_LOCATE);
            if (ap.dbg_stop == 2) { const uint32_t x = pos4[0] + pos4[1] + pos4[2] + pos4[3]; if (__ballot(x == 12345u) == 1) results[r].pos = x; return; }
            for (int s = 0; s < 2; ++s) {
                const uint64_t mc = __ballot(keep4[2 * s]), mr = __ballot(keep4[2 * s + 1]);
                const uint32_t nc = (uint32_t)__popcll(mc);
                if (keep4[2 * s]) w.loci[s][(uint32_t)__popcll(mc & lt)] = pos4[2 * s];
                if (keep4[2 * s + 1]) w.loci[s][nc + (uint32_t)__popcll(mr & lt)] = pos4[2 * s + 1];
                n_s[s] = nc + (uint32_t)__popcll(mr);
                c_sa_c += tot[2 * s]; c_sa_r += tot[2 * s + 1]; c_loci += n_s[s];
            }
            }
            WSYNC();
            stamp(SALT_CTR_LT_SORT);
            if (ap.dbg_stop == 3) { if (lane == 0) results[r].pos = w.loci[0][0] + w.loci[1][0] + n_s[0] + n_s[1]; return; }
            uint32_t bound = 3, q_pos = 0xFFFFFFFFu, q_strand = 3, q_ndiff = 255;
            uint32_t n_hits_s[2] = { 0, 0 }, a0[2] = { 0, 0 };
            bool found[2] = { false, false };
            {
                if (L <= 120) verify_quads_2(ix.ref, ix.ref_len, w.pm[0], w.pm[1], L, w.loci[0], n_s[0], w.loci[1], n_s[1], w.val[0], w.val[1]);
                else if (L <= 248) verify_quads_2<8>(ix.ref, ix.ref_len, w.pm[0], w.pm[1], L, w.loci[0], n_s[0], w.loci[1], n_s[1], w.val[0], w.val[1]);
                else
                    for (int s = 0; s < 2; ++s)
                        for (uint32_t i = lane; i < n_s[s]; i += 64) w.val[s][i] = (uint8_t)mismatch_capped(ix, w.pm[s], L, w.loci[s][i]);
                WSYNC();
                stamp(SALT_CTR_LT_VERIFY);
                if (ap.dbg_stop == 4) { if (__ballot(w.val[0][0] + w.val[1][0] == 12345u) == 1) results[r].pos = w.val[0][0]; return; }
                c_verify += n_s[0] + n_s[1];
                for (int s = 0; s < 2; ++s) {
                    bool any = false; uint32_t bp = 0, bv = 0;
                    rule_sparse<3, false>(w.loci[s], w.val[s], n_s[s], L, ix.ref_len, bound, any, bp, bv, n_hits_s[s], a0[s], w.hit_pos[s], w.hit_nd[s]);
                    if (any) { found[s] = true; q_pos = bp; q_ndiff = bv; q_strand = (uint32_t)s; }
                }
            }
// ... 106 lines not shown
        uint32_t m = HB(v <= bound && p < ref_len);
        while (m) {
            const int l = __ffs((int)m) - 1;
            const uint32_t pl = SHF(p, l), vl = SHF(v, l);
#pragma unroll
            for (int t = 0; t <= 3; ++t) if (vl == (uint32_t)t && pl < mp[t]) mp[t] = pl;
            m &= m - 1;
        }
    }
    uint32_t before[4];
    before[0] = NONE;
#pragma unroll
    for (int t = 1; t <= 3; ++t) before[t] = mp[t - 1] < before[t - 1] ? mp[t - 1] : before[t - 1];
#pragma unroll
    for (int t = 3; t >= 0; --t) if (mp[t] != NONE) { any = true; best_v = (uint32_t)t; best_pos = mp[t]; }
    if (!any) return;
    uint32_t last_p = 0;
    for (uint32_t h = 0; h < (uint32_t)NHIT; ++h) {
        uint32_t cur_p = NONE, cur_v = 0;
        for (uint32_t b = 0; b < n; b += 32) {
            const uint32_t i = b + hl;
            uint32_t p = 0, v = NONE;
            if (i < n) { p = pos[i]; v = val[i]; }
            const uint32_t lim = v == 1 ? before[1] : v == 2 ? before[2] : v == 3 ? before[3] : NONE;
            uint32_t m = HB(v <= bound && p < ref_len && p < lim && (h == 0 || p > last_p));
            while (m) {
                const int l = __ffs((int)m) - 1;
                const uint32_t pl = SHF(p, l);
                if (pl < cur_p) { cur_p = pl; cur_v = SHF(v, l); }
                m &= m - 1;
            }
        }
        if (cur_p == NONE) break;
        if (hl == 0) { hit_pos[h] = cur_p; hit_nd[h] = (uint8_t)cur_v; }
        if (h == 0) a0 = cur_v;
        last_p = cur_p; ++n_hits;
    }
    bound = best_v < bound ? best_v : bound;
}

template <int L2_WAVES, int LN = 4>
__global__ void __launch_bounds__(64 * L2_WAVES) __attribute__((amdgpu_waves_per_eu(8, 8)))
k_light2(IndexView ix, AlignParams ap, const uint32_t *__restrict__ pm,
         const uint4 *__restrict__ sai_c, const uint4 *__restrict__ sai_r, salt_result_t *__restrict__ results,
         uint32_t *__restrict__ queue , QueueRange *__restrict__ ranges)
{
    __shared__ LightLds2 w2[2 * L2_WAVES];
    const uint32_t lane = lane_id(), hl = lane & 31u, hb = lane & 32u, half = lane >> 5;
    LightLds2 &w = w2[2u * (threadIdx.x >> 6) + half];
    const uint32_t lt = (1u << hl) - 1u;
    auto HB = [&](bool x) -> uint32_t { const uint64_t m = __ballot(x); return hb ? (uint32_t)(m >> 32) : (uint32_t)m; };
    auto SHF = [&](uint32_t v, int src) -> uint32_t { return (uint32_t)__shfl((int)v, (int)hb + src); };
    const uint32_t r = 2u * (blockIdx.x * (uint32_t)L2_WAVES + (threadIdx.x >> 6)) + half;
    if (r >= ap.n_reads) return;
    const uint32_t *rec = pm + (uint64_t)r * ap.pg.pm_stride;
    const uint32_t L = rec[2 * ap.pg.nw8];
    bool heavy = L > (LN == 8 ? 248u : 120u) || L < (uint32_t)ap.l_seed || ap.spr > (uint32_t)L2_SLOTS || ap.max_locate < 2 * 64;
    if (!heavy) {
        const uint32_t nw = (L + 7) >> 3;
        uint32_t n_amb = 0;
        for (uint32_t x = hl; x < 2 * nw; x += 32) {
            const uint32_t s = x >= nw, j = s ? x - nw : x;
            const uint32_t word = rec[s * ap.pg.nw8 + j];
            w.pm[s][j] = word;
            if (!s) n_amb += (uint32_t)__popc(word & (word >> 1) & (word >> 2) & (word >> 3) & 0x11111111u);
        }
        if (ap.max_amb < L) {
            for (int o = 16; o > 0; o >>= 1) n_amb += (uint32_t)__shfl_xor((int)n_amb, o);
            if (n_amb > ap.max_amb) {
                if (hl == 0) {
                    salt_result_t *out = results + r;
                    out->pos = 0xFFFFFFFFu; out->strand = 3; out->n_diff = 255; out->is_gap = 255; out->mapq = 0;
                    out->b0 = -1; out->b1 = -1; out->seq_start = 0; out->seq_end = (uint16_t)(L - 1);
                    out->n_hits[0] = out->n_hits[1] = 0; out->n_cigar = 0; out->skipped = 1;
                }
                return;
            }
        }
        uint32_t tot[4];
        bool small;
        {
            const uint32_t l = hl >> 3, slot = hl & 7u;
            uint4 v = make_uint4(1, 0, 0, 0);
            if (slot < ap.spr) v = ((l & 1) ? sai_r : sai_c)[((uint64_t)r * 2u + (l >> 1)) * ap.spr + slot];
            uint32_t sz = v.w ? v.y - v.x + 1u : 0u;
            if (sz > 65u) sz = 65u;
            uint32_t inc = sz;
            for (int o = 1; o < 8; o <<= 1) { const uint32_t t = (uint32_t)__shfl_up((int)inc, o, 8); if (slot >= (uint32_t)o) inc += t; }
            for (int q = 0; q < 4; ++q) tot[q] = SHF(inc, 8 * q + 7);
            small = tot[0] <= 8 && tot[1] <= 8 && tot[2] <= 8 && tot[3] <= 8;
            if (small) {
                for (uint32_t k2 = 0; k2 < sz; ++k2) { w.sp[l][inc - sz + k2] = v.x + k2; w.off[l][inc - sz + k2] = v.z | (v.w == 2 ? 0x80000000u : 0u); }
            } else {
                w.sp[l][slot] = v.x; w.off[l][slot] = v.z | (v.w == 2 ? 0x80000000u : 0u);
                w.pre[l][slot + 1] = inc;
                if (slot == 0) w.pre[l][0] = 0;
            }
        }
        WSYNC();
        for (int l = 0; l < 4; ++l) heavy |= tot[l] > 64;
        if (!heavy) {
            uint32_t n_s[2] = { 0, 0 };
            if (small) {
                const uint32_t l = hl >> 3, x = hl & 7u;
                const uint32_t tl = l == 0 ? tot[0] : l == 1 ? tot[1] : l == 2 ? tot[2] : tot[3];
                bool keep = false; uint32_t p = 0;
                if (x < tl) {
                    const uint32_t j = w.sp[l][x], of = w.off[l][x];
                    p = ((of >> 31) ? j : (l & 1) ? ix.r_pos[j] : ix.c_sa[j]) - (of & 0x7FFFFFFFu);
                    keep = (l & 1) ? !(p > ix.ref_len || p + L > ix.ref_len) : !(p + L > ix.ref_len);
                }
                const uint32_t km = HB(keep);
                const uint32_t s = hl >> 4, ms = (km >> (16 * s)) & 0xFFFFu;
                if (keep) w.loci[s][(uint32_t)__popc(ms & ((1u << (hl & 15u)) - 1u))] = p;
                n_s[0] = (uint32_t)__popc(km & 0xFFFFu); n_s[1] = (uint32_t)__popc(km >> 16);
            } else {
                for (int l = 0; l < 4; ++l) {
                    const int s = l >> 1;
                    for (uint32_t x = hl; x - hl < tot[l]; x += 32) {
                        bool keep = false; uint32_t p = 0;
                        if (x < tot[l]) {
                            uint32_t i = 0;
                            while (w.pre[l][i + 1] <= x) ++i;
                            const uint32_t j = w.sp[l][i] + (x - w.pre[l][i]), of = w.off[l][i];
                            p = ((of >> 31) ? j : (l & 1) ? ix.r_pos[j] : ix.c_sa[j]) - (of & 0x7FFFFFFFu);
                            keep = (l & 1) ? !(p > ix.ref_len || p + L > ix.ref_len) : !(p + L > ix.ref_len);
                        }
                        const uint32_t km = HB(keep);
                        if (keep) w.loci[s][n_s[s] + (uint32_t)__popc(km & lt)] = p;
                        n_s[s] += (uint32_t)__popc(km);
                    }
                }
            }
            WSYNC();
            {
                constexpr uint32_t RPG = 32u / LN;
                const uint32_t sub = hl & (uint32_t)(LN - 1), q = hl / (uint32_t)LN, n = n_s[0] + n_s[1];
                const uint32_t nvalid = L > 32u * sub ? (L - 32u * sub < 32u ? L - 32u * sub : 32u) : 0u;
                uint32_t pa[4], pb[4];
#pragma unroll
                for (int t = 0; t < 4; ++t) { const bool in = (4 * sub + t) < nw; pa[t] = in ? w.pm[0][4 * sub + t] : 0u; pb[t] = in ? w.pm[1][4 * sub + t] : 0u; }
                for (uint32_t b = 0; b < n; b += 4u * RPG) {
                    uint32_t pos[4]; u32x4_a4 x[4]; bool act[4], rev[4];
#pragma unroll
                    for (int g = 0; g < 4; ++g) {
                        if (b + RPG * g >= n) break;
                        const uint32_t c = b + RPG * g + q;
                        act[g] = c < n; rev[g] = c >= n_s[0];
                        pos[g] = act[g] ? (rev[g] ? w.loci[1][c - n_s[0]] : w.loci[0][c]) : 0u;
                        if (pos[g] >= ix.ref_len) pos[g] = 0xFFFFFFFFu;
                        if (LN == 8 && !(4u * sub < nw + 1u)) x[g] = u32x4_a4{ 0u, 0u, 0u, 0u };
                        else x[g] = *reinterpret_cast<const u32x4_a4 *>(ix.ref + ((pos[g] == 0xFFFFFFFFu ? 0u : pos[g]) >> 3) + 4 * sub);
                    }
#pragma unroll
                    for (int g = 0; g < 4; ++g) {
                        if (b + RPG * g >= n) break;
                        const uint32_t pw[4] = { rev[g] ? pb[0] : pa[0], rev[g] ? pb[1] : pa[1], rev[g] ? pb[2] : pa[2], rev[g] ? pb[3] : pa[3] };
                        const uint32_t mism = quad_mismatch<LN>(x[g], pos[g], pw, nvalid);
                        if (act[g] && sub == 0) {
                            const uint32_t c = b + RPG * g + q;
                            const uint8_t v = (uint8_t)((mism > 3 || pos[g] == 0xFFFFFFFFu) ? INF : mism);
                            if (rev[g]) w.val[1][c - n_s[0]] = v; else w.val[0][c] = v;
                        }
                    }
                }
            }
            WSYNC();
// ... 417 lines not shown
```

salt_amd/csrc/salt_device.h:

```cpp
#pragma once
#include <hip/hip_runtime.h>
#include <stdint.h>
#include "salt_ctx_record.h"

namespace salt {

struct COcc { uint32_t cnt[4]; uint64_t lo, hi; };
struct ROcc { uint32_t cnt[4]; uint64_t b0[2], b1[2], b2[2]; };
static_assert(sizeof(COcc) == 32, "COcc");
static_assert(sizeof(ROcc) == 64, "ROcc");

struct ImageHeader {
    uint64_t magic, bytes;
    uint32_t c_primary, c_L2[5], c_seq_len, c_sa_intv;
    uint32_t lkt_len, lkt_n;
    uint32_t r_text_len, r_inv_sa0, r_cum[6];
    uint32_t ref_len, r_lkt_len;
    uint64_t off_c_occ, off_c_sa, off_lkt, off_r_occ, off_r_pos, off_wlkt, off_ref, off_text;
    uint64_t n_c_blocks, n_r_blocks;
    uint64_t off_ctx;
    uint32_t ctx_k, pad0;
    uint64_t reserved[5];
};
static const uint64_t IMAGE_MAGIC = 0x53414c5447465841ull;

struct IndexView {
    const COcc *c_occ; const uint32_t *c_sa; const uint32_t *lkt;
    const ROcc *r_occ; const uint32_t *r_pos; const uint4 *wlkt; const uint32_t *ref; const uint32_t *text;
    const uint4 *c_ctx; uint32_t ctx_k;
    const uint4 *r_ctx;
    uint32_t c_primary, c_L2[5], c_seq_len;
    uint32_t r_text_len, r_inv_sa0, r_cum[6];
    uint32_t ref_len, lkt_len, r_lkt_len;
};


__device__ __forceinline__ uint32_t sel4(uint4 v, uint32_t c)
{
    return c == 0 ? v.x : c == 1 ? v.y : c == 2 ? v.z : v.w;
}

__device__ __forceinline__ uint32_t pick4(const uint32_t *a, uint32_t c) { return c == 0 ? a[0] : c == 1 ? a[1] : c == 2 ? a[2] : a[3]; }
__device__ __forceinline__ uint32_t pick5(const uint32_t *a, uint32_t c) { return c == 0 ? a[0] : c == 1 ? a[1] : c == 2 ? a[2] : c == 3 ? a[3] : a[4]; }

__device__ __forceinline__ uint32_t c_occ(const IndexView &ix, uint32_t k, uint32_t c)
{
    if (k == ix.c_seq_len) return ix.c_L2[c + 1] - ix.c_L2[c];
    if (k == 0xFFFFFFFFu) return 0;
    k -= (k >= ix.c_primary);
    const uint4 *p = reinterpret_cast<const uint4 *>(ix.c_occ + (k >> 6));
    uint4 cnt = p[0];
    uint4 pl = p[1];
    uint64_t lo = (uint64_t)pl.x | ((uint64_t)pl.y << 32), hi = (uint64_t)pl.z | ((uint64_t)pl.w << 32);
    uint32_t m = (k & 63u) + 1u;
    uint64_t mask = m == 64 ? ~0ull : ((1ull << m) - 1ull);
    uint64_t eq = ((c & 1) ? lo : ~lo) & ((c & 2) ? hi : ~hi) & mask;
    return sel4(cnt, c) + (uint32_t)__popcll(eq);
}

__device__ __forceinline__ uint32_t c_occ_eval(const uint4 cnt, const uint4 pl, const uint32_t k, const uint32_t c)
{
    const uint64_t lo = (uint64_t)pl.x | ((uint64_t)pl.y << 32), hi = (uint64_t)pl.z | ((uint64_t)pl.w << 32);
    const uint32_t m = (k & 63u) + 1u;
    const uint64_t mask = m == 64 ? ~0ull : ((1ull << m) - 1ull);
    const uint64_t eq = ((c & 1) ? lo : ~lo) & ((c & 2) ? hi : ~hi) & mask;
    return sel4(cnt, c) + (uint32_t)__popcll(eq);
}
__device__ __forceinline__ uint32_t c_occ2(const IndexView &ix, const uint32_t k, const uint32_t l, const uint32_t c, uint32_t &ok, uint32_t &ol)
{
    const uint32_t full = pick4(ix.c_L2 + 1, c) - pick4(ix.c_L2, c);
    const bool ks = k == ix.c_seq_len || k == 0xFFFFFFFFu, ls = l == ix.c_seq_len || l == 0xFFFFFFFFu;
    const uint32_t kk = k - (k >= ix.c_primary), ll = l - (l >= ix.c_primary);
    uint4 cnt = make_uint4(0, 0, 0, 0), pl = make_uint4(0, 0, 0, 0);
    if (!ks) { const uint4 *p = reinterpret_cast<const uint4 *>(ix.c_occ + (kk >> 6)); cnt = p[0]; pl = p[1]; }
    ok = ks ? (k == ix.c_seq_len ? full : 0u) : c_occ_eval(cnt, pl, kk, c);
    if (ls) { ol = l == ix.c_seq_len ? full : 0u; return ks ? 0u : 1u; }
    const bool second = ks || (ll >> 6) != (kk >> 6);
    if (second) { const uint4 *p = reinterpret_cast<const uint4 *>(ix.c_occ + (ll >> 6)); cnt = p[0]; pl = p[1]; }
    ol = c_occ_eval(cnt, pl, ll, c);
    return (ks ? 0u : 1u) + (second ? 1u : 0u);
}

struct COcc2 { uint4 cntk, plk, cntl, pll; };
__device__ __forceinline__ void c_occ2_addr(const IndexView &ix, const uint32_t k, const uint32_t l, const uint4 *&pk, const uint4 *&pl)
{
    const bool ks = k == ix.c_seq_len || k == 0xFFFFFFFFu, ls = l == ix.c_seq_len || l == 0xFFFFFFFFu;
    const uint32_t kk = k - (k >= ix.c_primary), ll = l - (l >= ix.c_primary);
    pk = ks ? nullptr : reinterpret_cast<const uint4 *>(ix.c_occ + (kk >> 6));
    pl = ls || (!ks && (ll >> 6) == (kk >> 6)) ? nullptr : reinterpret_cast<const uint4 *>(ix.c_occ + (ll >> 6));
}
__device__ __forceinline__ uint32_t c_occ2_eval(const IndexView &ix, const COcc2 r, const uint32_t k, const uint32_t l, const uint32_t c, uint32_t &ok, uint32_t &ol)
{
    const uint32_t full = pick4(ix.c_L2 + 1, c) - pick4(ix.c_L2, c);
    const bool ks = k == ix.c_seq_len || k == 0xFFFFFFFFu, ls = l == ix.c_seq_len || l == 0xFFFFFFFFu;
    const uint32_t kk = k - (k >= ix.c_primary), ll = l - (l >= ix.c_primary);
    ok = ks ? (k == ix.c_seq_len ? full : 0u) : c_occ_eval(r.cntk, r.plk, kk, c);
    const bool second = !ls && (ks || (ll >> 6) != (kk >> 6));
    ol = ls ? (l == ix.c_seq_len ? full : 0u) : c_occ_eval(second ? r.cntl : r.cntk, second ? r.pll : r.plk, ll, c);
    return (ks ? 0u : 1u) + (second ? 1u : 0u);
}

__device__ __forceinline__ uint32_t c_sym(const IndexView &ix, uint32_t k)
{
    const COcc *r = ix.c_occ + (k >> 6);
    uint32_t b = k & 63u;
    return (uint32_t)((r->lo >> b) & 1ull) | ((uint32_t)((r->hi >> b) & 1ull) << 1);
}

__device__ __forceinline__ uint32_t r_occ(const IndexView &ix, uint32_t index, uint32_t c)
{
    index -= (index > ix.r_inv_sa0);
    uint32_t blk = index >> 7, m = index & 127u;
    const uint4 *p = reinterpret_cast<const uint4 *>(ix.r_occ + blk);
    uint4 cnt = p[0], q0 = p[1], q1 = p[2], q2 = p[3];
    uint64_t b0l = (uint64_t)q0.x | ((uint64_t)q0.y << 32), b0h = (uint64_t)q0.z | ((uint64_t)q0.w << 32);
    uint64_t b1l = (uint64_t)q1.x | ((uint64_t)q1.y << 32), b1h = (uint64_t)q1.z | ((uint64_t)q1.w << 32);
    uint64_t b2l = (uint64_t)q2.x | ((uint64_t)q2.y << 32), b2h = (uint64_t)q2.z | ((uint64_t)q2.w << 32);
    uint64_t ml = m >= 64 ? ~0ull : ((1ull << m) - 1ull);
// ... 64 lines not shown
```

salt_amd/csrc/salt_gpu.hip:

```cpp
#include <hip/hip_runtime.h>
#include <stdio.h>
#include <stdlib.h>
#include <string.h>
#include <time.h>
#include <cstddef>
#include <cctype>
#include <string>
#include <thread>
#include <vector>
#include <algorithm>
#include "salt_kernels.h"
#include "salt_inflate_block.h"
#include <rccl/rccl.h>

using namespace salt;

static thread_local std::string g_err;
static int fail(int code, const std::string &msg) { g_err = msg; return code; }

#define HIPCHK(x) do { hipError_t e_ = (x); if (e_ != hipSuccess) \
    return fail(SALT_E_HIP, std::string(#x) + ": " + hipGetErrorString(e_)); } while (0)
#define DONECHK(x) do { hipError_t e_ = (x); if (e_ != hipSuccess) return done(fail(SALT_E_HIP, std::string(#x) + ": " + hipGetErrorString(e_))); } while (0)

struct salt_gpu_index {
    int device = 0;
    uint8_t *image = nullptr;
    uint64_t bytes = 0;
    bool owns = true;
    ImageHeader hdr;
    IndexView view;
    uint8_t *d_pac = nullptr; uint64_t l_pac = 0;
    uint4 *d_rctx = nullptr;
    int64_t *d_c_off = nullptr; uint32_t *d_c_name_off = nullptr; char *d_c_names = nullptr; int32_t n_contigs = 0;
};

struct salt_gpu_ws {
    salt_gpu_index *ix = nullptr;
    uint32_t max_reads = 0; uint64_t max_bases = 0;
    uint8_t *d_seqs = nullptr; uint32_t *d_offs = nullptr; salt_result_t *d_results = nullptr;
    uint4 *d_sai_c = nullptr, *d_sai_r = nullptr; uint64_t sai_cap = 0;
    uint4 *d_wq = nullptr; uint32_t *d_wq_cnt = nullptr; uint32_t walk_blocks = 512; bool no_unique = false;
    uint32_t *d_pm = nullptr, *d_tb = nullptr; uint64_t pm_cap = 0, tb_cap = 0;
    uint8_t *d_heads = nullptr, *h_heads = nullptr;
    unsigned long long *d_ctr = nullptr;
    uint32_t *d_queue = nullptr; SeCtl *d_qctl = nullptr;
    void *d_lvtab = nullptr;
    uint8_t *d_gap = nullptr; uint32_t gcap = 0; GapBufs gap{};
    uint8_t *d_pe_scr = nullptr;
    PePair *d_pairs = nullptr; PeSwReq *d_req = nullptr; PeSwRes *d_swres = nullptr; PeCtl *d_pctl = nullptr;
    uint8_t *d_sw_scr = nullptr; uint64_t sw_scr_bytes = 0; uint32_t sw_blocks = 0; uint32_t pe_pairs_cap = 0;
    uint32_t *d_pcq = nullptr;
    uint8_t *d_raw = nullptr; uint64_t raw_cap = 0; uint32_t *d_tile = nullptr; uint64_t tile_cap = 0; uint32_t *d_lines = nullptr; uint64_t lines_cap = 0;
    FqRec *d_rec = nullptr; uint32_t *d_tctl = nullptr, *d_samoff = nullptr; void *d_scan = nullptr; size_t scan_bytes = 0;
    char *d_sam = nullptr, *h_sam = nullptr; uint64_t sam_cap = 0; char *d_rg = nullptr; std::string rg;
    char *d_samslot = nullptr; SamSeg *d_samseg = nullptr;
    bool h_sam_owned = true;
    bool sam_bgzf = false;
    bool sam_bam = false;
    uint32_t *d_bz_slots = nullptr, *d_bz_sizes = nullptr; unsigned long long *d_bz_offs = nullptr; uint8_t *d_bz_out = nullptr; uint64_t bz_blocks_cap = 0;
    char *h_bz = nullptr; uint64_t h_bz_cap = 0;
    uint8_t *d_zin = nullptr; uint64_t zin_cap = 0; unsigned long long *d_zoff = nullptr; uint32_t *d_zstat = nullptr; uint64_t zblocks_cap = 0;
    uint8_t *d_text = nullptr; uint64_t text_cap = 0, text_bytes = 0;
    std::vector<unsigned long long> h_zoff; std::vector<uint32_t> h_zstat;
    uint32_t text_calls = 0;
    uint32_t heavy_blocks = 2048, gap_blocks = 2048;
    QueueRange *d_ranges = nullptr;
    uint8_t *d_zero = nullptr; size_t zero_bytes = 0;
    int all_heavy = 0;
    hipStream_t stream = nullptr;
    bool timing = false;
    std::vector<hipEvent_t> ev;
    std::vector<uint8_t> ev_pe;
    uint32_t n_timed = 0;
};
static const uint32_t MAX_TIMED = 256, EV_PER_CALL = 12;

static inline uint64_t align_up(uint64_t x, uint64_t a) { return (x + a - 1) / a * a; }

static void make_view(salt_gpu_index *ix)
{
    const ImageHeader &h = ix->hdr;
    IndexView &v = ix->view;
    uint8_t *b = ix->image;
    v.c_occ = reinterpret_cast<const COcc *>(b + h.off_c_occ);
    v.c_sa = reinterpret_cast<const uint32_t *>(b + h.off_c_sa);
    v.lkt = reinterpret_cast<const uint32_t *>(b + h.off_lkt);
    v.r_occ = reinterpret_cast<const ROcc *>(b + h.off_r_occ);
    v.r_pos = reinterpret_cast<const uint32_t *>(b + h.off_r_pos);
    v.wlkt = reinterpret_cast<const uint4 *>(b + h.off_wlkt);
    v.ref = reinterpret_cast<const uint32_t *>(b + h.off_ref);
    v.text = reinterpret_cast<const uint32_t *>(b + h.off_text);
    v.c_ctx = h.off_ctx ? reinterpret_cast<const uint4 *>(b + h.off_ctx) : nullptr; v.ctx_k = h.ctx_k;
    v.r_ctx = ix->d_rctx;
    v.c_primary = h.c_primary; memcpy(v.c_L2, h.c_L2, sizeof v.c_L2); v.c_seq_len = h.c_seq_len;
    v.r_text_len = h.r_text_len; v.r_inv_sa0 = h.r_inv_sa0; memcpy(v.r_cum, h.r_cum, sizeof v.r_cum);
    v.ref_len = h.ref_len; v.lkt_len = h.lkt_len; v.r_lkt_len = h.r_lkt_len;
}

extern "C" const char *salt_gpu_last_error(void) { return g_err.c_str(); }
extern "C" uint32_t salt_gpu_result_size(void) { return (uint32_t)sizeof(salt_result_t); }

extern "C" int salt_gpu_index_attach(const salt_host_index_t *h, int device, salt_gpu_index_t **out)
{
    if (!h || !out) return fail(SALT_E_INVAL, "null argument");
    if (!h->c_bwt || !h->c_sa || !h->lkt || !h->r_bwt || !h->r_sa || !h->ref) return fail(SALT_E_INDEX, "missing index array");
    if (h->c_sa_intv == 0 || h->c_n_sa != (h->c_seq_len + h->c_sa_intv) / h->c_sa_intv) return fail(SALT_E_INDEX, "inconsistent C suffix-array sampling");
    if (h->lkt_len < 1 || h->lkt_len > 14 || h->lkt_n != (1u << (2 * h->lkt_len)) + 1) return fail(SALT_E_INDEX, "unsupported lookup-table length");
    if (h->r_n_sa != h->r_text_len - h->r_cum[4] + 1) return fail(SALT_E_INDEX, "R suffix array size does not match '#' count");
    if ((uint64_t)h->r_bwt_words * 8 < h->r_text_len) return fail(SALT_E_INDEX, "R BWT shorter than its text length");
    int n_dev = 0;
    HIPCHK(hipGetDeviceCount(&n_dev));
    if (n_dev <= 0) return fail(SALT_E_HIP, "no HIP device visible: the salt GPU path cannot run (there is no CPU fallback)");
    HIPCHK(hipSetDevice(device));

    salt_gpu_index *ix = new salt_gpu_index();
    ix->device = device;
    ImageHeader &hd = ix->hdr;
    memset(&hd, 0, sizeof hd);
    hd.magic = IMAGE_MAGIC;
    hd.c_primary = h->c_primary; memcpy(hd.c_L2, h->c_L2, sizeof hd.c_L2); hd.c_seq_len = h->c_seq_len; hd.c_sa_intv = h->c_sa_intv;
    hd.lkt_len = h->lkt_len; hd.lkt_n = h->lkt_n;
    hd.r_text_len = h->r_text_len; hd.r_inv_sa0 = h->r_inv_sa0; memcpy(hd.r_cum, h->r_cum, sizeof hd.r_cum);
    hd.ref_len = h->ref_len;
    const uint64_t ctx_bytes = (((uint64_t)h->c_seq_len + 1) * 16 + 255) / 256 * 256;
    bool want_ctx = h->l_seed > 0 && !(getenv("SALT_GPU_NO_CTX") && atoi(getenv("SALT_GPU_NO_CTX")));
    {
        uint32_t w = 14;
        size_t free_b = 0, total_b = 0;
        if (hipMemGetInfo(&free_b, &total_b) == hipSuccess) {
            if (want_ctx && (uint64_t)free_b < ctx_bytes + (24ull << 30)) want_ctx = false;
            const uint64_t avail = (uint64_t)free_b - (want_ctx ? ctx_bytes : 0);
            w = avail >= (200ull << 30) ? 16 : avail >= (72ull << 30) ? 15 : 14;
        }
        if (const char *e = getenv("SALT_GPU_LKT_LEN")) w = (uint32_t)atoi(e);
        if (h->l_seed > 0 && w > (uint32_t)h->l_seed) w = (uint32_t)h->l_seed;
        if (h->l_seed <= 0) w = h->lkt_len;
        if (w < h->lkt_len) w = h->lkt_len;
        if (w > 16) w = 16;
        hd.r_lkt_len = w;
    }
    hd.n_c_blocks = (uint64_t)h->c_seq_len / 64 + 1;
    hd.n_r_blocks = (uint64_t)h->r_text_len / 128 + 1;
    const uint64_t ref_words = ((uint64_t)h->ref_len + 7) / 8;
    uint64_t off = align_up(sizeof(ImageHeader), 256);
    hd.off_c_occ = off; off = align_up(off + hd.n_c_blocks * sizeof(COcc), 256);
    hd.off_c_sa = off;  off = align_up(off + ((uint64_t)h->c_seq_len + 1) * 4, 256);
    hd.off_lkt = off;   off = align_up(off + (uint64_t)h->lkt_n * 4, 256);
    hd.off_r_occ = off; off = align_up(off + hd.n_r_blocks * sizeof(ROcc), 256);
    hd.off_r_pos = off; off = align_up(off + ((uint64_t)h->r_text_len + 1) * 4, 256);
    hd.off_ref = off;   off = align_up(off + (ref_words + 4) * 4, 256);
    hd.off_text = off;  off = align_up(off + ((uint64_t)h->c_seq_len / 16 + 4) * 4, 256);
    hd.off_wlkt = off; off = align_up(off + (1ull << (2 * hd.r_lkt_len)) * 32, 256);
    if (want_ctx) { hd.off_ctx = off; hd.ctx_k = (uint32_t)h->l_seed; off += ctx_bytes; }
    hd.bytes = off;
    ix->bytes = off;

    hipError_t e = hipMalloc((void **)&ix->image, ix->bytes);
    if (e != hipSuccess) { delete ix; return fail(SALT_E_NOMEM, std::string("hipMalloc(index image): ") + hipGetErrorString(e)); }
    uint32_t *d_sa_s = nullptr, *d_r_sa = nullptr, *d_raw = nullptr, *d_minor = nullptr, *d_major = nullptr, *d_err = nullptr;
#define CHK2(x) do { hipError_t e2 = (x); if (e2 != hipSuccess) { hipFree(ix->image); hipFree(d_sa_s); hipFree(d_r_sa); hipFree(d_raw); hipFree(d_minor); hipFree(d_major); hipFree(d_err); delete ix; \
    return fail(SALT_E_HIP, std::string(#x) + ": " + hipGetErrorString(e2)); } } while (0)
    CHK2(hipMemset(ix->image, 0, hd.off_wlkt));
    CHK2(hipMemcpy(ix->image, &hd, sizeof hd, hipMemcpyHostToDevice));
    CHK2(hipMalloc((void **)&d_err, 4)); CHK2(hipMemset(d_err, 0, 4));
    {
        CHK2(hipMalloc((void **)&d_raw, (uint64_t)h->c_bwt_size * 4 + 4));
        CHK2(hipMemcpy(d_raw, h->c_bwt, (uint64_t)h->c_bwt_size * 4, hipMemcpyHostToDevice));
        launch_pack_c_occ(d_raw, h->c_bwt_size, h->c_seq_len, hd.n_c_blocks, reinterpret_cast<COcc *>(ix->image + hd.off_c_occ), d_err, nullptr);
        CHK2(hipGetLastError()); CHK2(hipDeviceSynchronize());
        hipFree(d_raw); d_raw = nullptr;
    }
    {
        CHK2(hipMalloc((void **)&d_raw, (uint64_t)h->r_bwt_words * 4 + 4));
        CHK2(hipMemcpy(d_raw, h->r_bwt, (uint64_t)h->r_bwt_words * 4, hipMemcpyHostToDevice));
        CHK2(hipMalloc((void **)&d_minor, (uint64_t)h->r_occ_words * 4 + 4)); CHK2(hipMemcpy(d_minor, h->r_occ, (uint64_t)h->r_occ_words * 4, hipMemcpyHostToDevice));
        CHK2(hipMalloc((void **)&d_major, (uint64_t)h->r_major_words * 4 + 4)); CHK2(hipMemcpy(d_major, h->r_major, (uint64_t)h->r_major_words * 4, hipMemcpyHostToDevice));
        launch_pack_r_occ(d_raw, h->r_bwt_words, d_minor, h->r_occ_words, d_major, h->r_major_words, h->r_text_len, hd.n_r_blocks,
                          reinterpret_cast<ROcc *>(ix->image + hd.off_r_occ), d_err, nullptr);
        CHK2(hipGetLastError()); CHK2(hipDeviceSynchronize());
        hipFree(d_raw); hipFree(d_minor); hipFree(d_major); d_raw = d_minor = d_major = nullptr;
    }
    {
        uint32_t perr = 0;
        CHK2(hipMemcpy(&perr, d_err, 4, hipMemcpyDeviceToHost));
        hipFree(d_err); d_err = nullptr;
        if (perr) {
            hipFree(ix->image); delete ix;
            return fail(SALT_E_INDEX, perr & 1 ? "C BWT array shorter than seq_len" : perr & 4 ? "R BWT holds a symbol outside {A,C,G,T,#}" : "R BWT / Occ arrays shorter than the text length");
        }
    }
    CHK2(hipMemcpy(ix->image + hd.off_lkt, h->lkt, (uint64_t)h->lkt_n * 4, hipMemcpyHostToDevice));
    CHK2(hipMemcpy(ix->image + hd.off_ref, h->ref, ref_words * 4, hipMemcpyHostToDevice));
    make_view(ix);
    CHK2(hipMalloc((void **)&d_sa_s, (uint64_t)h->c_n_sa * 4));
    CHK2(hipMalloc((void **)&d_r_sa, (uint64_t)h->r_n_sa * 4));
    CHK2(hipMemcpy(d_sa_s, h->c_sa, (uint64_t)h->c_n_sa * 4, hipMemcpyHostToDevice));
    CHK2(hipMemcpy(d_r_sa, h->r_sa, (uint64_t)h->r_n_sa * 4, hipMemcpyHostToDevice));
    launch_build_c_sa(ix->view, d_sa_s, h->c_sa_intv, reinterpret_cast<uint32_t *>(ix->image + hd.off_c_sa), nullptr);
    launch_build_r_pos(ix->view, d_r_sa, reinterpret_cast<uint32_t *>(ix->image + hd.off_r_pos), nullptr);
    launch_build_text(ix->view, reinterpret_cast<uint32_t *>(ix->image + hd.off_text), nullptr);
    launch_build_wlkt(ix->view, hd.r_lkt_len, reinterpret_cast<uint4 *>(ix->image + hd.off_wlkt), nullptr);
    if (hd.off_ctx) launch_build_c_ctx(ix->view, hd.ctx_k, reinterpret_cast<uint4 *>(ix->image + hd.off_ctx), nullptr);
    CHK2(hipGetLastError());
    CHK2(hipDeviceSynchronize());
    hipFree(d_sa_s); hipFree(d_r_sa);
#undef CHK2
    *out = ix;
    return SALT_OK;
}

extern "C" void salt_gpu_index_detach(salt_gpu_index_t *ix)
{
    if (!ix) return;
    if (ix->owns && ix->image) { hipSetDevice(ix->device); hipFree(ix->image); }
    if (ix->d_pac) { hipSetDevice(ix->device); hipFree(ix->d_pac); }
    if (ix->d_rctx) { hipSetDevice(ix->device); hipFree(ix->d_rctx); }
    if (ix->d_c_off) { hipSetDevice(ix->device); hipFree(ix->d_c_off); hipFree(ix->d_c_name_off); hipFree(ix->d_c_names); }
    delete ix;
}

extern "C" int salt_gpu_index_image(const salt_gpu_index_t *ix, void **dev_ptr, uint64_t *bytes)
{
    if (!ix || !dev_ptr || !bytes) return fail(SALT_E_INVAL, "null argument");
    *dev_ptr = ix->image; *bytes = ix->bytes;
    return SALT_OK;
}

extern "C" int salt_gpu_index_attach_image(void *dev_ptr, uint64_t bytes, int device, salt_gpu_index_t **out)
{
    if (!dev_ptr || !out || bytes < sizeof(ImageHeader)) return fail(SALT_E_INVAL, "bad image");
    HIPCHK(hipSetDevice(device));
    salt_gpu_index *ix = new salt_gpu_index();
    ix->device = device; ix->image = static_cast<uint8_t *>(dev_ptr); ix->bytes = bytes; ix->owns = false;
    hipError_t e = hipMemcpy(&ix->hdr, dev_ptr, sizeof(ImageHeader), hipMemcpyDeviceToHost);
    if (e != hipSuccess) { delete ix; return fail(SALT_E_HIP, std::string("hipMemcpy(image header): ") + hipGetErrorString(e)); }
    if (ix->hdr.magic != IMAGE_MAGIC || ix->hdr.bytes != bytes) { delete ix; return fail(SALT_E_INDEX, "not a salt device-index image"); }
    make_view(ix);
    *out = ix;
    return SALT_OK;
}

extern "C" int salt_gpu_index_image_compact(const salt_gpu_index_t *ix, void **dev_ptr, uint64_t *bytes)
{
    if (!ix || !dev_ptr || !bytes) return fail(SALT_E_INVAL, "null argument");
    *dev_ptr = ix->image; *bytes = ix->hdr.off_wlkt;
    return SALT_OK;
}

static int rebuild_wlkt(salt_gpu_index *ix)
{
    launch_build_wlkt(ix->view, ix->hdr.r_lkt_len, reinterpret_cast<uint4 *>(ix->image + ix->hdr.off_wlkt), nullptr);
    if (ix->hdr.off_ctx) launch_build_c_ctx(ix->view, ix->hdr.ctx_k, reinterpret_cast<uint4 *>(ix->image + ix->hdr.off_ctx), nullptr);
    HIPCHK(hipGetLastError());
    HIPCHK(hipDeviceSynchronize());
    return SALT_OK;
}

extern "C" int salt_gpu_index_attach_compact(const void *dev_ptr, uint64_t bytes, int device, salt_gpu_index_t **out)
{
    if (!dev_ptr || !out || bytes < sizeof(ImageHeader)) return fail(SALT_E_INVAL, "bad image");
    HIPCHK(hipSetDevice(device));
    ImageHeader hd;
    HIPCHK(hipMemcpy(&hd, dev_ptr, sizeof hd, hipMemcpyDeviceToHost));
    if (hd.magic != IMAGE_MAGIC || hd.off_wlkt != bytes || hd.bytes < bytes) return fail(SALT_E_INDEX, "not a compact salt device-index image");
    salt_gpu_index *ix = new salt_gpu_index();
    ix->device = device; ix->bytes = hd.bytes; ix->owns = true; ix->hdr = hd;
    hipError_t e = hipMalloc((void **)&ix->image, hd.bytes);
    if (e != hipSuccess) { delete ix; return fail(SALT_E_NOMEM, std::string("hipMalloc(index image): ") + hipGetErrorString(e)); }
    e = hipMemcpy(ix->image, dev_ptr, bytes, hipMemcpyDeviceToDevice);
    if (e != hipSuccess) { hipFree(ix->image); delete ix; return fail(SALT_E_HIP, std::string("hipMemcpy(compact image): ") + hipGetErrorString(e)); }
    make_view(ix);
    int rc = rebuild_wlkt(ix);
    if (rc) { hipFree(ix->image); delete ix; return rc; }
    *out = ix;
    return SALT_OK;
}

extern "C" int salt_gpu_ws_create(salt_gpu_index_t *ix, uint32_t max_reads, uint64_t max_bases, salt_gpu_ws_t **out)
{
    if (!ix || !out || max_reads == 0) return fail(SALT_E_INVAL, "bad workspace size");
    HIPCHK(hipSetDevice(ix->device));
    salt_gpu_ws *ws = new salt_gpu_ws();
    ws->ix = ix; ws->max_reads = max_reads; ws->max_bases = max_bases;
#define CHKW(x) do { hipError_t e2 = (x); if (e2 != hipSuccess) { salt_gpu_ws_destroy(ws); \
    return fail(SALT_E_NOMEM, std::string(#x) + ": " + hipGetErrorString(e2)); } } while (0)
    CHKW(hipMalloc((void **)&ws->d_seqs, max_bases + 64));
    CHKW(hipMalloc((void **)&ws->d_offs, ((uint64_t)max_reads + 1) * 4));
    CHKW(hipMalloc((void **)&ws->d_results, (uint64_t)max_reads * sizeof(salt_result_t)));
    CHKW(hipMemset(ws->d_results, 0, (uint64_t)max_reads * sizeof(salt_result_t)));
    CHKW(hipMalloc((void **)&ws->d_queue, queue_words(max_reads) * 4));
    {
        const size_t a = 256, n_ranges = (QUEUE_RANGES * sizeof(QueueRange) + a - 1) / a * a, n_ctl = (sizeof(SeCtl) + a - 1) / a * a;
        const size_t n_cnt = ((size_t)seed_wq_cnt_words() * 4 + a - 1) / a * a;
        CHKW(hipMalloc((void **)&ws->d_zero, n_ranges + n_ctl + n_cnt));
        ws->zero_bytes = n_ranges + n_ctl + n_cnt;
        ws->d_ranges = reinterpret_cast<QueueRange *>(ws->d_zero); ws->d_qctl = reinterpret_cast<SeCtl *>(ws->d_zero + n_ranges);
        ws->d_wq_cnt = reinterpret_cast<uint32_t *>(ws->d_zero + n_ranges + n_ctl);
    }
    ws->gcap = max_reads < (1u << 20) ? max_reads : (1u << 20);
    if (const char *e3 = getenv("SALT_GPU_NO_GAP_DEFER")) if (atoi(e3)) ws->gcap = 0;
    if (const char *e3 = getenv("SALT_GPU_GAP_SLOTS")) { const int v = atoi(e3); if (v > 0 && (uint32_t)v < ws->gcap) ws->gcap = (uint32_t)v; }
    if (ws->gcap) {
        size_t gbytes = 0;
        gap_bufs_layout(nullptr, ws->gcap, nullptr, &gbytes);
        CHKW(hipMalloc((void **)&ws->d_gap, gbytes));
    }
    {
        hipDeviceProp_t prop;
        CHKW(hipGetDeviceProperties(&prop, ix->device));
        uint32_t per_cu = heavy_blocks_per_cu();
        if (const char *e2 = getenv("SALT_GPU_HEAVY_PER_CU")) { int v = atoi(e2); if (v > 0 && (uint32_t)v <= heavy_blocks_per_cu()) per_cu = (uint32_t)v; }
        ws->heavy_blocks = (uint32_t)prop.multiProcessorCount * per_cu;
        uint32_t gap_per_cu = 16;
        if (const char *e2 = getenv("SALT_GPU_GAP_PER_CU")) { int v = atoi(e2); if (v > 0 && v <= 16) gap_per_cu = (uint32_t)v; }
        ws->gap_blocks = (uint32_t)prop.multiProcessorCount * gap_per_cu;
        ws->walk_blocks = (uint32_t)prop.multiProcessorCount * 2u;
        if (const char *e2 = getenv("SALT_GPU_WALK_PER_CU")) { int v = atoi(e2); if (v > 0 && v <= 16) ws->walk_blocks = (uint32_t)prop.multiProcessorCount * (uint32_t)v; }
        if (const char *e2 = getenv("SALT_GPU_NO_UNIQUE")) ws->no_unique = atoi(e2) != 0;
        if (const char *e2 = getenv("SALT_GPU_WALK_BLOCKS")) { int v = atoi(e2); if (v > 0 && v <= 65536) ws->walk_blocks = (uint32_t)v; }
        CHKW(hipMalloc(&ws->d_lvtab, (uint64_t)ws->heavy_blocks * lv_table_bytes()));
        const char *e = getenv("SALT_GPU_ALL_HEAVY");
        ws->all_heavy = e && atoi(e) != 0;
    }
    CHKW(hipMalloc((void **)&ws->d_ctr, SALT_CTR_N * sizeof(unsigned long long)));
    CHKW(hipMemset(ws->d_ctr, 0, SALT_CTR_N * sizeof(unsigned long long)));
    CHKW(hipStreamCreate(&ws->stream));
#undef CHKW
    *out = ws;
    return SALT_OK;
}

extern "C" void salt_gpu_ws_destroy(salt_gpu_ws_t *ws)
{
    if (!ws) return;
    hipSetDevice(ws->ix->device);
    hipFree(ws->d_seqs); hipFree(ws->d_offs); hipFree(ws->d_results); hipFree(ws->d_sai_c); hipFree(ws->d_sai_r); hipFree(ws->d_wq); hipFree(ws->d_pm); hipFree(ws->d_tb); hipFree(ws->d_heads); if (ws->h_heads) hipHostFree(ws->h_heads); hipFree(ws->d_ctr); hipFree(ws->d_queue); hipFree(ws->d_zero); hipFree(ws->d_lvtab); hipFree(ws->d_gap);
    hipFree(ws->d_raw); hipFree(ws->d_tile); hipFree(ws->d_lines); hipFree(ws->d_rec); hipFree(ws->d_tctl); hipFree(ws->d_samoff); hipFree(ws->d_samslot); hipFree(ws->d_samseg); hipFree(ws->d_scan); hipFree(ws->d_sam); hipFree(ws->d_rg);
    hipFree(ws->d_zin); hipFree(ws->d_zoff); hipFree(ws->d_zstat); hipFree(ws->d_text);
    if (ws->h_sam && ws->h_sam_owned) hipHostFree(ws->h_sam);
    hipFree(ws->d_bz_slots); hipFree(ws->d_bz_sizes); hipFree(ws->d_bz_offs); hipFree(ws->d_bz_out); if (ws->h_bz) hipHostFree(ws->h_bz);
    hipFree(ws->d_pe_scr); hipFree(ws->d_pairs); hipFree(ws->d_req); hipFree(ws->d_swres); hipFree(ws->d_pctl); hipFree(ws->d_sw_scr); hipFree(ws->d_pcq);
    if (ws->stream) hipStreamDestroy(ws->stream);
    for (auto &e : ws->ev) if (e) hipEventDestroy(e);
    delete ws;
}

static int check_opt(const salt_gpu_index *ix, const salt_aln_opt_t *o, uint32_t max_len, uint32_t *spr_out)
{
    if (o->l_seed < (int32_t)ix->hdr.r_lkt_len) return fail(SALT_E_INVAL, "l_seed shorter than the device k-mer table (set SALT_GPU_LKT_LEN or pass l_seed at attach)");
    if (o->l_overlap <= 0) return fail(SALT_E_INVAL, "l_overlap must be positive (aln.c:223 sets it to l_seed when -r is absent)");
    if (o->max_locate == 0 || o->max_locate > PE_LOCI_CAP) return fail(SALT_E_INVAL, "max_locate (-m) must be in 1..262144");
    if (o->max_hits != SALT_MAX_HITS) return fail(SALT_E_INVAL, "max_hits is fixed at 5 (aln.h:133)");
    if (max_len > SALT_MAX_READ_LEN) return fail(SALT_E_INVAL, "read longer than SALT_MAX_READ_LEN (512)");
    uint32_t spr = 1;
    if (max_len >= (uint32_t)o->l_seed) spr = (max_len - (uint32_t)o->l_seed) / (uint32_t)o->l_overlap + 1;
    if (spr > SALT_MAX_SEED_SLOTS) return fail(SALT_E_INVAL, "more seeds per strand than SALT_MAX_SEED_SLOTS (512): raise -r or shorten the reads");
    *spr_out = spr;
    return SALT_OK;
}

static int align_resident_impl(salt_gpu_ws_t *ws, const salt_aln_opt_t *o, uint32_t n_reads, uint32_t max_read_len,
                               const void *d_seqs, const void *d_offs, void *d_results, void *hip_stream, int pe);

extern "C" int salt_gpu_align_se_resident(salt_gpu_ws_t *ws, const salt_aln_opt_t *o, uint32_t n_reads, uint32_t max_read_len,
                                          const void *d_seqs, const void *d_offs, void *d_results, void *hip_stream)
{
    return align_resident_impl(ws, o, n_reads, max_read_len, d_seqs, d_offs, d_results, hip_stream, 0);
}

static int align_resident_impl(salt_gpu_ws_t *ws, const salt_aln_opt_t *o, uint32_t n_reads, uint32_t max_read_len,
                               const void *d_seqs, const void *d_offs, void *d_results, void *hip_stream, int pe)
{
    if (!ws || !o || !d_seqs || !d_offs || !d_results) return fail(SALT_E_INVAL, "null argument");
    if (n_reads == 0) return SALT_OK;
    uint32_t spr = 0;
    int rc = check_opt(ws->ix, o, max_read_len, &spr);
    if (rc) return rc;
    HIPCHK(hipSetDevice(ws->ix->device));
    hipStream_t st = static_cast<hipStream_t>(hip_stream);
    uint64_t items = (uint64_t)n_reads * 2u * spr;
    if (items > ws->sai_cap) {
        HIPCHK(hipStreamSynchronize(st));
        hipFree(ws->d_sai_c); hipFree(ws->d_sai_r); hipFree(ws->d_wq); ws->d_sai_c = ws->d_sai_r = ws->d_wq = nullptr; ws->sai_cap = 0;
        HIPCHK(hipMalloc((void **)&ws->d_sai_c, items * sizeof(uint4)));
        HIPCHK(hipMalloc((void **)&ws->d_sai_r, items * sizeof(uint4)));
        HIPCHK(hipMalloc((void **)&ws->d_wq, seed_wq_words(items) * 4));
        ws->sai_cap = items;
    }
    const PackGeom pg = PackGeom::make(max_read_len);
    if ((uint64_t)n_reads * pg.pm_stride > ws->pm_cap || (uint64_t)n_reads * pg.tb_stride > ws->tb_cap) {
        HIPCHK(hipStreamSynchronize(st));
        hipFree(ws->d_pm); hipFree(ws->d_tb); ws->d_pm = ws->d_tb = nullptr; ws->pm_cap = ws->tb_cap = 0;
        const uint64_t nr = n_reads > ws->max_reads ? n_reads : ws->max_reads;
        HIPCHK(hipMalloc((void **)&ws->d_pm, nr * pg.pm_stride * 4));
        HIPCHK(hipMalloc((void **)&ws->d_tb, nr * pg.tb_stride * 4));
        ws->pm_cap = nr * pg.pm_stride; ws->tb_cap = nr * pg.tb_stride;
    }
    SeedParams sp; sp.pg = pg; sp.n_reads = n_reads; sp.spr = spr; sp.l_seed = o->l_seed; sp.l_overlap = o->l_overlap;
    sp.max_seed = o->max_seed; sp.seed_only_ref = o->seed_only_ref;
    sp.resolve_unique = !ws->no_unique;
    if (n_reads > ws->max_reads) return fail(SALT_E_CAPACITY, "more reads than the workspace holds");
    AlignParams ap; ap.pg = pg; ap.n_reads = n_reads; ap.spr = spr; ap.l_seed = o->l_seed; ap.max_locate = o->max_locate; ap.max_hits = o->max_hits;
    ap.all_heavy = ws->all_heavy; ap.pe = pe; ap.dbg_stop = 0; ap.heavy_stop = 0; ap.max_amb = pe ? 5u : 200u;
#ifdef SALT_DIAG
    { const char *e = getenv("SALT_GPU_LIGHT_STOP"); ap.dbg_stop = e ? atoi(e) : 0; } { static const int hs = getenv("SALT_GPU_HEAVY_STOP") ? atoi(getenv("SALT_GPU_HEAVY_STOP")) : 0; ap.heavy_stop = hs; }
#endif
    const bool glob_loci = pe || o->max_locate > SALT_MAX_LOCATE;
    if (glob_loci && !ws->d_pe_scr) HIPCHK(hipMalloc((void **)&ws->d_pe_scr, (uint64_t)ws->heavy_blocks * PE_LOCI_CAP * 5));
    unsigned long long *ctr = o->collect_counters ? ws->d_ctr : nullptr;
    const bool timed = ws->timing && ws->n_timed < MAX_TIMED;
    hipEvent_t *ev = timed ? &ws->ev[(size_t)ws->n_timed * EV_PER_CALL] : nullptr;
    HIPCHK(hipMemsetAsync(ws->d_zero, 0, ws->zero_bytes, st));
    if (timed) HIPCHK(hipEventRecord(ev[0], st));
    launch_pack(pg, n_reads, static_cast<const uint8_t *>(d_seqs), static_cast<const uint32_t *>(d_offs), ws->d_pm, ws->d_tb, st);
    if (timed) HIPCHK(hipEventRecord(ev[1], st));
    launch_seed(ws->ix->view, sp, ws->d_tb, ws->d_sai_c, ws->d_sai_r, ws->d_wq, ws->d_wq_cnt, ws->walk_blocks, ctr, st);
    if (timed) HIPCHK(hipEventRecord(ev[2], st));
    if (!ap.all_heavy)
        launch_light(ws->ix->view, ap, ws->d_pm, static_cast<const uint8_t *>(d_seqs), static_cast<const uint32_t *>(d_offs), ws->d_sai_c, ws->d_sai_r,
                     static_cast<salt_result_t *>(d_results), ws->d_queue, ws->d_qctl, ws->d_queue + 2 * (size_t)ws->max_reads, ws->d_ranges, ctr, st);
    if (timed) HIPCHK(hipEventRecord(ev[3], st));
    launch_heavy(ws->ix->view, ap, ws->d_pm, ws->d_sai_c, ws->d_sai_r,
                 static_cast<salt_result_t *>(d_results), ws->d_queue, ctr, ws->heavy_blocks, ws->gap_blocks, ws->d_lvtab,
                 gap_bufs_layout(ws->d_gap, ws->gcap, ws->d_qctl, nullptr), ws->d_queue + ws->max_reads, ws->d_ranges, glob_loci ? ws->d_pe_scr : nullptr, timed ? ev + 4 : nullptr, st);
    if (timed) { HIPCHK(hipEventRecord(ev[7], st)); ws->ev_pe[ws->n_timed] = 0; ++ws->n_timed; }
    HIPCHK(hipGetLastError());
    return SALT_OK;
}

static const uint32_t HEAD_BYTES = 128;
static_assert(offsetof(salt_result_t, cigar) + 8 * sizeof(uint16_t) == HEAD_BYTES, "result head");
static int fetch_results(salt_gpu_ws_t *ws, uint32_t n_reads, salt_result_t *results, hipStream_t st)
{
    if (!ws->d_heads) {
        HIPCHK(hipMalloc((void **)&ws->d_heads, (uint64_t)ws->max_reads * HEAD_BYTES));
        HIPCHK(hipHostMalloc((void **)&ws->h_heads, (uint64_t)ws->max_reads * HEAD_BYTES, hipHostMallocDefault));
    }
    launch_heads(ws->d_results, n_reads, ws->d_heads, st);
    HIPCHK(hipMemcpyAsync(ws->h_heads, ws->d_heads, (uint64_t)n_reads * HEAD_BYTES, hipMemcpyDeviceToHost, st));
    HIPCHK(hipStreamSynchronize(st));
    std::vector<uint32_t> full;
    const uint32_t n_thr = n_reads >= 262144 ? 4u : 1u;
    std::vector<std::vector<uint32_t>> full_t(n_thr);
    auto scatter = [&](uint32_t t) {
        const uint32_t lo = (uint32_t)((uint64_t)n_reads * t / n_thr), hi = (uint32_t)((uint64_t)n_reads * (t + 1) / n_thr);
        for (uint32_t i = lo; i < hi; ++i) {
            memcpy(&results[i], ws->h_heads + (uint64_t)i * HEAD_BYTES, HEAD_BYTES);
            const salt_result_t &r = results[i];
            bool more = r.n_cigar > 8;
            for (int h = 0; h < SALT_MAX_HITS; ++h) more |= r.hit_n_cigar[h] != 0;
            if (more) full_t[t].push_back(i);
        }
    };
    {
        std::vector<std::thread> th;
        for (uint32_t t = 1; t < n_thr; ++t) th.emplace_back(scatter, t);
        scatter(0);
        for (auto &x : th) x.join();
    }
    for (auto &v : full_t) full.insert(full.end(), v.begin(), v.end());
    if (full.size() > 4096) {
        HIPCHK(hipMemcpyAsync(results, ws->d_results, (uint64_t)n_reads * sizeof(salt_result_t), hipMemcpyDeviceToHost, st));
    } else {
        for (uint32_t i : full) HIPCHK(hipMemcpyAsync(&results[i], ws->d_results + i, sizeof(salt_result_t), hipMemcpyDeviceToHost, st));
    }
    HIPCHK(hipStreamSynchronize(st));
    return SALT_OK;
}

extern "C" int salt_gpu_align_se(salt_gpu_ws_t *ws, const salt_aln_opt_t *o, uint32_t n_reads, const uint8_t *seqs,
                                 const uint32_t *offs, salt_result_t *results)
{
    if (!ws || !o || !seqs || !offs || !results) return fail(SALT_E_INVAL, "null argument");
    if (n_reads == 0) return SALT_OK;
    if (n_reads > ws->max_reads) return fail(SALT_E_CAPACITY, "more reads than the workspace holds");
    if (offs[0] != 0) return fail(SALT_E_INVAL, "offs[0] must be 0");
    uint64_t bases = offs[n_reads];
    if (bases > ws->max_bases) return fail(SALT_E_CAPACITY, "more bases than the workspace holds");
    uint32_t max_len = 0;
    for (uint32_t i = 0; i < n_reads; ++i) {
        if (offs[i + 1] < offs[i]) return fail(SALT_E_INVAL, "offs must be non-decreasing");
        uint32_t l = offs[i + 1] - offs[i];
        if (l == 0) return fail(SALT_E_INVAL, "empty read");
        max_len = l > max_len ? l : max_len;
    }
    HIPCHK(hipSetDevice(ws->ix->device));
    HIPCHK(hipMemcpyAsync(ws->d_seqs, seqs, bases, hipMemcpyHostToDevice, ws->stream));
    HIPCHK(hipMemcpyAsync(ws->d_offs, offs, ((uint64_t)n_reads + 1) * 4, hipMemcpyHostToDevice, ws->stream));
    int rc = salt_gpu_align_se_resident(ws, o, n_reads, max_len, ws->d_seqs, ws->d_offs, ws->d_results, ws->stream);
    if (rc) return rc;
    return fetch_results(ws, n_reads, results, ws->stream);
}

extern "C" int salt_gpu_index_set_contigs(salt_gpu_index_t *ix, int32_t n, const int64_t *offsets, const char *const *names)
{
    if (!ix || n <= 0 || !offsets || !names) return fail(SALT_E_INVAL, "bad contig table");
    HIPCHK(hipSetDevice(ix->device));
    std::vector<uint32_t> noff((size_t)n + 1, 0); std::string blob;
    for (int i = 0; i < n; ++i) { if (!names[i]) return fail(SALT_E_INVAL, "contig without a name"); blob += names[i]; noff[(size_t)i + 1] = (uint32_t)blob.size(); }
    if (ix->d_c_off) { hipFree(ix->d_c_off); hipFree(ix->d_c_name_off); hipFree(ix->d_c_names); ix->d_c_off = nullptr; ix->d_c_name_off = nullptr; ix->d_c_names = nullptr; ix->n_contigs = 0; }
    HIPCHK(hipMalloc((void **)&ix->d_c_off, (size_t)n * 8));
    HIPCHK(hipMalloc((void **)&ix->d_c_name_off, ((size_t)n + 1) * 4));
    HIPCHK(hipMalloc((void **)&ix->d_c_names, blob.size() + 1));
    HIPCHK(hipMemcpy(ix->d_c_off, offsets, (size_t)n * 8, hipMemcpyHostToDevice));
    HIPCHK(hipMemcpy(ix->d_c_name_off, noff.data(), ((size_t)n + 1) * 4, hipMemcpyHostToDevice));
    HIPCHK(hipMemcpy(ix->d_c_names, blob.data(), blob.size(), hipMemcpyHostToDevice));
    ix->n_contigs = n;
    HIPCHK(text_warm());
    return SALT_OK;
}

extern "C" int salt_gpu_host_alloc(uint64_t bytes, void **ptr)
{
    if (!ptr || !bytes) return fail(SALT_E_INVAL, "null argument");
    HIPCHK(hipHostMalloc(ptr, bytes, hipHostMallocDefault));
    return SALT_OK;
}
extern "C" void salt_gpu_host_free(void *ptr) { if (ptr) hipHostFree(ptr); }

extern "C" int salt_gpu_device_numa_node(int device, int *node)
{
    if (!node) return fail(SALT_E_INVAL, "null argument");
    *node = -1;
    char bus[64] = { 0 };
    HIPCHK(hipDeviceGetPCIBusId(bus, (int)sizeof bus, device));
    for (char *c = bus; *c; ++c) *c = (char)tolower((unsigned char)*c);
    const std::string path = std::string("/sys/bus/pci/devices/") + bus + "/numa_node";
    if (FILE *f = fopen(path.c_str(), "r")) { int v = -1; if (fscanf(f, "%d", &v) == 1) *node = v; fclose(f); }
    return SALT_OK;
}
extern "C" int salt_gpu_device_count(int *n)
{
    if (!n) return fail(SALT_E_INVAL, "null argument");
    HIPCHK(hipGetDeviceCount(n));
    return SALT_OK;
}

#define REGROW(ptr, cap, need, type) do { if ((need) > (cap)) { HIPCHK(hipStreamSynchronize(st)); hipFree(ptr); (ptr) = nullptr; (cap) = 0; \
    const uint64_t want_ = (need) + (need) / 4; HIPCHK(hipMalloc((void **)&(ptr), want_ * sizeof(type))); (cap) = want_; } } while (0)

extern "C" int salt_gpu_ws_reserve_text(salt_gpu_ws_t *ws, const salt_aln_opt_t *o, uint64_t max_block_bytes, uint32_t est_reads, uint32_t max_read_len,
                                        uint64_t est_sam_bytes, void *host_sam, uint64_t host_sam_bytes)
{
    if (!ws || !o || max_block_bytes == 0 || est_reads == 0) return fail(SALT_E_INVAL, "bad reserve arguments");
    if (est_reads > ws->max_reads) est_reads = ws->max_reads;
    uint32_t spr = 0;
    int rc = check_opt(ws->ix, o, max_read_len, &spr);
    if (rc) return rc;
    HIPCHK(hipSetDevice(ws->ix->device));
    hipStream_t st = ws->stream;
    REGROW(ws->d_raw, ws->raw_cap, max_block_bytes + 64, uint8_t);
    if (!ws->d_tctl) HIPCHK(hipMalloc((void **)&ws->d_tctl, 32));
    REGROW(ws->d_tile, ws->tile_cap, ws->raw_cap / FQ_TILE + 4, uint32_t);
    {
        const size_t need = text_scan_bytes(std::max<uint64_t>(ws->tile_cap, (uint64_t)ws->max_reads + 2));
        if (need > ws->scan_bytes) { hipFree(ws->d_scan); ws->d_scan = nullptr; ws->scan_bytes = 0; HIPCHK(hipMalloc(&ws->d_scan, need)); ws->scan_bytes = need; }
    }
    REGROW(ws->d_lines, ws->lines_cap, 4ull * est_reads + 8, uint32_t);
    if (!ws->d_rec) HIPCHK(hipMalloc((void **)&ws->d_rec, (uint64_t)ws->max_reads * sizeof(FqRec)));
    if (!ws->d_samoff) HIPCHK(hipMalloc((void **)&ws->d_samoff, ((uint64_t)ws->max_reads + 2) * 4));
    if (!ws->d_samslot) { HIPCHK(hipMalloc((void **)&ws->d_samslot, (uint64_t)ws->max_reads * SAM_SLOT)); HIPCHK(hipMalloc((void **)&ws->d_samseg, (uint64_t)ws->max_reads * sizeof(SamSeg))); }
    const uint64_t items = (uint64_t)est_reads * 2u * spr;
    if (items > ws->sai_cap) {
        hipFree(ws->d_sai_c); hipFree(ws->d_sai_r); hipFree(ws->d_wq); ws->d_sai_c = ws->d_sai_r = ws->d_wq = nullptr; ws->sai_cap = 0;
        HIPCHK(hipMalloc((void **)&ws->d_sai_c, items * sizeof(uint4)));
        HIPCHK(hipMalloc((void **)&ws->d_sai_r, items * sizeof(uint4)));
        HIPCHK(hipMalloc((void **)&ws->d_wq, seed_wq_words(items) * 4));
        ws->sai_cap = items;
    }
    const PackGeom pg = PackGeom::make(max_read_len);
    if ((uint64_t)ws->max_reads * pg.pm_stride > ws->pm_cap || (uint64_t)ws->max_reads * pg.tb_stride > ws->tb_cap) {
        hipFree(ws->d_pm); hipFree(ws->d_tb); ws->d_pm = ws->d_tb = nullptr; ws->pm_cap = ws->tb_cap = 0;
        HIPCHK(hipMalloc((void **)&ws->d_pm, (uint64_t)ws->max_reads * pg.pm_stride * 4));
        HIPCHK(hipMalloc((void **)&ws->d_tb, (uint64_t)ws->max_reads * pg.tb_stride * 4));
        ws->pm_cap = (uint64_t)ws->max_reads * pg.pm_stride; ws->tb_cap = (uint64_t)ws->max_reads * pg.tb_stride;
    }
    if (host_sam && host_sam_bytes > est_sam_bytes + 64) est_sam_bytes = host_sam_bytes - 64;
    if (est_sam_bytes + 64 > ws->sam_cap) {
        hipFree(ws->d_sam); ws->d_sam = nullptr; if (ws->h_sam && ws->h_sam_owned) hipHostFree(ws->h_sam); ws->h_sam = nullptr; ws->sam_cap = 0;
        HIPCHK(hipMalloc((void **)&ws->d_sam, est_sam_bytes + 64));
        if (host_sam && host_sam_bytes >= est_sam_bytes + 64) { ws->h_sam = static_cast<char *>(host_sam); ws->h_sam_owned = false; }
        else { HIPCHK(hipHostMalloc((void **)&ws->h_sam, est_sam_bytes + 64, hipHostMallocDefault)); ws->h_sam_owned = true; }
        ws->sam_cap = est_sam_bytes + 64;
    }
    return SALT_OK;
}

struct BgzfBufs { uint32_t *slots = nullptr, *sizes = nullptr; unsigned long long *offs = nullptr; uint8_t *out = nullptr; };
static int bgzf_alloc(uint64_t n_blocks, BgzfBufs &b)
{
    HIPCHK(hipMalloc((void **)&b.slots, n_blocks * BGZF_SLOT_BYTES));
    HIPCHK(hipMalloc((void **)&b.sizes, n_blocks * 4));
    HIPCHK(hipMalloc((void **)&b.offs, (n_blocks + 1) * 8));
    HIPCHK(hipMalloc((void **)&b.out, n_blocks * (BGZF_CUT_BYTES + 31)));
    return SALT_OK;
}
static void bgzf_free(BgzfBufs &b) { hipFree(b.slots); hipFree(b.sizes); hipFree(b.offs); hipFree(b.out); b = BgzfBufs(); }

static int ws_sam_bgzf(salt_gpu_ws_t *ws, uint64_t total, hipStream_t st, const char **sam, uint64_t *sam_bytes)
{
    const uint64_t n_blocks = bgzf_blocks(total);
    if (n_blocks > ws->bz_blocks_cap) {
        HIPCHK(hipStreamSynchronize(st));
        BgzfBufs b; b.slots = ws->d_bz_slots; b.sizes = ws->d_bz_sizes; b.offs = ws->d_bz_offs; b.out = ws->d_bz_out;
        bgzf_free(b); ws->d_bz_slots = ws->d_bz_sizes = nullptr; ws->d_bz_offs = nullptr; ws->d_bz_out = nullptr; ws->bz_blocks_cap = 0;
        const uint64_t want = n_blocks + n_blocks / 4 + 1;
        const int rc = bgzf_alloc(want, b);
        ws->d_bz_slots = b.slots; ws->d_bz_sizes = b.sizes; ws->d_bz_offs = b.offs; ws->d_bz_out = b.out;
        if (rc) return rc;
        ws->bz_blocks_cap = want;
    }
    HIPCHK(launch_bgzf_deflate(reinterpret_cast<const uint8_t *>(ws->d_sam), total, ws->d_bz_slots, ws->d_bz_sizes, ws->d_bz_offs, ws->d_bz_out, st));
    unsigned long long bytes = 0;
    HIPCHK(hipMemcpyAsync(&bytes, ws->d_bz_offs + n_blocks, 8, hipMemcpyDeviceToHost, st));
    HIPCHK(hipStreamSynchronize(st));
    if (bytes > bgzf_bound(total)) return fail(SALT_E_HIP, "BGZF blocks larger than their bound");
    char *dst = ws->h_sam;
    if (bytes > ws->sam_cap) {
        if (bytes > ws->h_bz_cap) {
            if (ws->h_bz) hipHostFree(ws->h_bz);
            ws->h_bz = nullptr; ws->h_bz_cap = 0;
            HIPCHK(hipHostMalloc((void **)&ws->h_bz, bytes + bytes / 4, hipHostMallocDefault));
            ws->h_bz_cap = bytes + bytes / 4;
        }
        dst = ws->h_bz;
    }
    HIPCHK(hipMemcpyAsync(dst, ws->d_bz_out, bytes, hipMemcpyDeviceToHost, st));
    HIPCHK(hipStreamSynchronize(st));
    *sam = dst; *sam_bytes = bytes;
    return SALT_OK;
}

extern "C" int salt_gpu_ws_set_sam_bgzf(salt_gpu_ws_t *ws, int on)
{
    if (!ws) return fail(SALT_E_INVAL, "null argument");
    ws->sam_bgzf = on != 0;
    return SALT_OK;
}

static const char *const BAM_NAME_ERROR = "BAM: a read name in this block is longer than 254 bytes, the most a BAM record holds (its length byte counts the NUL)";

extern "C" int salt_gpu_ws_set_sam_bam(salt_gpu_ws_t *ws, int on)
{
    if (!ws) return fail(SALT_E_INVAL, "null argument");
    ws->sam_bam = on != 0;
    return SALT_OK;
}

extern "C" int salt_gpu_bgzf_deflate(int device, const void *text, uint64_t n_bytes, void *out, uint64_t out_cap, uint64_t *out_bytes)
// ... 724 lines not shown
    uint32_t *d_pos = nullptr, *d_offs = nullptr, *d_b = nullptr, *d_out = nullptr; uint8_t *d_val = nullptr;
    const uint64_t ow = (uint64_t)n_cases * diag_rule_words();
    HIPCHK(hipMalloc((void **)&d_pos, (n + 64) * 4)); HIPCHK(hipMemcpy(d_pos, pos, n * 4, hipMemcpyHostToDevice));
    HIPCHK(hipMalloc((void **)&d_val, n + 64)); HIPCHK(hipMemcpy(d_val, val, n, hipMemcpyHostToDevice));
    HIPCHK(hipMalloc((void **)&d_offs, ((uint64_t)n_cases + 1) * 4)); HIPCHK(hipMemcpy(d_offs, offs, ((uint64_t)n_cases + 1) * 4, hipMemcpyHostToDevice));
    HIPCHK(hipMalloc((void **)&d_b, (uint64_t)n_cases * 4)); HIPCHK(hipMemcpy(d_b, bound_in, (uint64_t)n_cases * 4, hipMemcpyHostToDevice));
    HIPCHK(hipMalloc((void **)&d_out, ow * 4));
    launch_diag_rule(n_cases, d_pos, d_val, d_offs, d_b, L, ref_len, mode, d_out, nullptr);
    HIPCHK(hipGetLastError());
    HIPCHK(hipDeviceSynchronize());
    HIPCHK(hipMemcpy(out, d_out, ow * 4, hipMemcpyDeviceToHost));
    hipFree(d_pos); hipFree(d_val); hipFree(d_offs); hipFree(d_b); hipFree(d_out);
    return SALT_OK;
}

extern "C" int salt_gpu_diag_verify(const uint32_t *ref_words, uint32_t ref_len, uint32_t n_cases, const uint8_t *seqs, const uint32_t *offs,
                                    const uint32_t *cand, const uint32_t *cand_offs, int mode, uint8_t *out)
{
    if (!ref_words || !seqs || !offs || !cand || !cand_offs || !out) return fail(SALT_E_INVAL, "null argument");
    if (mode < 0 || mode > 4) return fail(SALT_E_INVAL, "mode must be 0..4");
    if (n_cases == 0) return SALT_OK;
    int n_dev = 0;
    HIPCHK(hipGetDeviceCount(&n_dev));
    if (n_dev <= 0) return fail(SALT_E_HIP, "no HIP device visible");
    for (uint32_t i = 0; i < n_cases; ++i) {
        const uint32_t L = offs[i + 1] - offs[i];
        if (L == 0 || L > SALT_MAX_READ_LEN || ((mode == 1 || mode == 3) && L > 120) || ((mode == 2 || mode == 4) && L > 248)) return fail(SALT_E_INVAL, "read length outside the verifier's range");
        if (cand_offs[i + 1] - cand_offs[i] > 256) return fail(SALT_E_INVAL, "at most 256 candidates per case");
    }
    const uint64_t nw = ((uint64_t)ref_len + 7) / 8 + 36, bases = offs[n_cases], nc = cand_offs[n_cases];
    uint32_t *d_ref = nullptr, *d_offs = nullptr, *d_cand = nullptr, *d_coffs = nullptr; uint8_t *d_seqs = nullptr, *d_out = nullptr;
    HIPCHK(hipMalloc((void **)&d_ref, nw * 4)); HIPCHK(hipMemset(d_ref, 0, nw * 4));
    HIPCHK(hipMemcpy(d_ref, ref_words, (nw - 36) * 4, hipMemcpyHostToDevice));
    HIPCHK(hipMalloc((void **)&d_offs, ((uint64_t)n_cases + 1) * 4)); HIPCHK(hipMemcpy(d_offs, offs, ((uint64_t)n_cases + 1) * 4, hipMemcpyHostToDevice));
    HIPCHK(hipMalloc((void **)&d_coffs, ((uint64_t)n_cases + 1) * 4)); HIPCHK(hipMemcpy(d_coffs, cand_offs, ((uint64_t)n_cases + 1) * 4, hipMemcpyHostToDevice));
    HIPCHK(hipMalloc((void **)&d_cand, (nc + 1) * 4)); HIPCHK(hipMemcpy(d_cand, cand, nc * 4, hipMemcpyHostToDevice));
    HIPCHK(hipMalloc((void **)&d_seqs, bases + 64)); HIPCHK(hipMemcpy(d_seqs, seqs, bases, hipMemcpyHostToDevice));
    HIPCHK(hipMalloc((void **)&d_out, nc + 1));
    launch_diag_verify(d_ref, ref_len, n_cases, d_seqs, d_offs, d_cand, d_coffs, mode, d_out, nullptr);
    HIPCHK(hipGetLastError());
    HIPCHK(hipDeviceSynchronize());
    HIPCHK(hipMemcpy(out, d_out, nc, hipMemcpyDeviceToHost));
    hipFree(d_ref); hipFree(d_offs); hipFree(d_coffs); hipFree(d_cand); hipFree(d_seqs); hipFree(d_out);
    return SALT_OK;
}

extern "C" int salt_gpu_ws_queue_counts(salt_gpu_ws_t *ws, uint32_t out[8])
{
    if (!ws || !out) return fail(SALT_E_INVAL, "null argument");
    HIPCHK(hipSetDevice(ws->ix->device));
    HIPCHK(hipDeviceSynchronize());
    SeCtl c; HIPCHK(hipMemcpy(&c, ws->d_qctl, sizeof c, hipMemcpyDeviceToHost));
    memset(out, 0, 32);
    out[0] = c.light_queued; out[2] = c.gap_slots; out[5] = c.gap_items; out[6] = c.cigar_items; out[7] = c.cigar_head;
    {
        std::vector<uint32_t> wc(seed_wq_cnt_words());
        HIPCHK(hipMemcpy(wc.data(), ws->d_wq_cnt, wc.size() * 4, hipMemcpyDeviceToHost));
        const uint32_t per_list = seed_wq_cnt_words() / 2u, stride = per_list / 64u;
        for (uint32_t i = 0; i < 64u; ++i) { out[1] = std::max(out[1], wc[i * stride]); out[3] = std::max(out[3], wc[per_list + i * stride]); }
    }
    return SALT_OK;
}

extern "C" int salt_gpu_ws_heavy_reads(salt_gpu_ws_t *ws, uint32_t *ids, uint32_t cap, uint32_t *n)
{
    if (!ws || !n) return fail(SALT_E_INVAL, "null argument");
    HIPCHK(hipSetDevice(ws->ix->device));
    HIPCHK(hipDeviceSynchronize());
    HIPCHK(hipMemcpy(n, &ws->d_qctl->light_queued, 4, hipMemcpyDeviceToHost));
    if (ids && cap) HIPCHK(hipMemcpy(ids, ws->d_queue, (uint64_t)(*n < cap ? *n : cap) * 4, hipMemcpyDeviceToHost));
    return SALT_OK;
}

extern "C" int salt_gpu_index_set_pac(salt_gpu_index_t *ix, const uint8_t *pac, uint64_t l_pac)
{
    if (!ix || !pac || l_pac == 0) return fail(SALT_E_INVAL, "null argument");
    HIPCHK(hipSetDevice(ix->device));
    if (ix->d_pac) { hipFree(ix->d_pac); ix->d_pac = nullptr; }
    const uint64_t bytes = l_pac / 4 + 2;
    HIPCHK(hipMalloc((void **)&ix->d_pac, bytes + 16));
    HIPCHK(hipMemset(ix->d_pac, 0, bytes + 16));
    HIPCHK(hipMemcpy(ix->d_pac, pac, bytes, hipMemcpyHostToDevice));
    ix->l_pac = l_pac;
    if (ix->view.c_ctx && !ix->d_rctx && !(getenv("SALT_GPU_NO_RCTX") && atoi(getenv("SALT_GPU_NO_RCTX")))) {
        const uint64_t rbytes = ((uint64_t)ix->hdr.r_text_len + 1) * 16;
        size_t free_b = 0, total_b = 0;
        if (hipMemGetInfo(&free_b, &total_b) == hipSuccess && (uint64_t)free_b >= rbytes + (32ull << 30) && hipMalloc((void **)&ix->d_rctx, rbytes) == hipSuccess) {
            launch_build_r_ctx(ix->view, ix->hdr.ctx_k, ix->d_rctx, nullptr);
            if (hipGetLastError() != hipSuccess || hipDeviceSynchronize() != hipSuccess) { hipFree(ix->d_rctx); ix->d_rctx = nullptr; return fail(SALT_E_HIP, "building the R context records failed"); }
            ix->view.r_ctx = ix->d_rctx;
        } else ix->d_rctx = nullptr;
    }
    return SALT_OK;
}

extern "C" int salt_gpu_ws_pe_overflow(salt_gpu_ws_t *ws, uint32_t *n)
{
    if (!ws || !n) return fail(SALT_E_INVAL, "null argument");
    *n = 0;
    if (!ws->d_pctl) return SALT_OK;
    HIPCHK(hipSetDevice(ws->ix->device));
    HIPCHK(hipDeviceSynchronize());
    HIPCHK(hipMemcpy(n, &ws->d_pctl->overflow, 4, hipMemcpyDeviceToHost));
    return SALT_OK;
}

extern "C" int salt_gpu_ws_pe_counts(salt_gpu_ws_t *ws, uint32_t out[8])
{
    if (!ws || !out) return fail(SALT_E_INVAL, "null argument");
    memset(out, 0, 32);
    if (!ws->d_pctl) return SALT_OK;
    HIPCHK(hipSetDevice(ws->ix->device));
    HIPCHK(hipDeviceSynchronize());
    PeCtl c; HIPCHK(hipMemcpy(&c, ws->d_pctl, sizeof c, hipMemcpyDeviceToHost));
    out[0] = c.n_req; out[2] = c.n_cigar; out[3] = c.cigar_head; out[4] = c.overflow; out[5] = c.diag_cols; out[6] = c.diag_clk;
    return SALT_OK;
}

static int pe_prepare(salt_gpu_ws_t *ws, uint32_t n_pairs, hipStream_t st)
{
    if (n_pairs > ws->pe_pairs_cap) {
        HIPCHK(hipStreamSynchronize(st));
        hipFree(ws->d_pairs); hipFree(ws->d_req); hipFree(ws->d_swres); hipFree(ws->d_pcq);
        ws->d_pairs = nullptr; ws->d_req = nullptr; ws->d_swres = nullptr; ws->d_pcq = nullptr; ws->pe_pairs_cap = 0;
        HIPCHK(hipMalloc((void **)&ws->d_pcq, (uint64_t)n_pairs * 2 * 4));
        HIPCHK(hipMalloc((void **)&ws->d_pairs, (uint64_t)n_pairs * sizeof(PePair)));
        HIPCHK(hipMalloc((void **)&ws->d_req, (uint64_t)n_pairs * 2 * sizeof(PeSwReq)));
        HIPCHK(hipMalloc((void **)&ws->d_swres, (uint64_t)n_pairs * 2 * sizeof(PeSwRes)));
        ws->pe_pairs_cap = n_pairs;
    }
    if (!ws->d_pctl) {
        HIPCHK(hipMalloc((void **)&ws->d_pctl, sizeof(PeCtl)));
        hipDeviceProp_t prop;
        HIPCHK(hipGetDeviceProperties(&prop, ws->ix->device));
        ws->sw_blocks = (uint32_t)prop.multiProcessorCount;
    }
    return SALT_OK;
}

static int pe_resident_impl(salt_gpu_ws_t *ws, const salt_aln_opt_t *o, const salt_pe_opt_t *pe, uint32_t n_pairs, uint32_t max_len,
                            const void *d_seqs, const void *d_offs, void *d_results, hipStream_t st)
{
    int rc = pe_prepare(ws, n_pairs, st);
    if (rc) return rc;
    const uint32_t ti = ws->n_timed;
    rc = align_resident_impl(ws, o, 2 * n_pairs, max_len, d_seqs, d_offs, d_results, st, 1);
    if (rc) return rc;
    hipEvent_t *ev = ws->n_timed == ti + 1 ? &ws->ev[(size_t)ti * EV_PER_CALL] : nullptr;
    HIPCHK(hipMemsetAsync(ws->d_pctl, 0, sizeof(PeCtl), st));
    launch_pair(n_pairs, pe->min_tlen, pe->max_tlen, (uint32_t)ws->ix->l_pac, static_cast<const uint32_t *>(d_offs), static_cast<salt_result_t *>(d_results),
                ws->d_pairs, ws->d_req, ws->d_pctl, st);
    if (ev) HIPCHK(hipEventRecord(ev[8], st));
    const uint64_t l_pac = (uint64_t)ws->ix->l_pac;
    uint64_t max_win = (uint64_t)pe->max_tlen + max_len + 2;
    if (max_win > l_pac + 1) max_win = l_pac + 1;
    SwGeom geom = sw_geom(max_len, max_win, ws->sw_blocks);
    sw_geom_limit(geom, n_pairs / 96u < 256u ? 256u : n_pairs / 96u);
    const uint64_t need = sw_scratch_bytes(geom);
    if (need > ws->sw_scr_bytes) {
        HIPCHK(hipStreamSynchronize(st));
        hipFree(ws->d_sw_scr); ws->d_sw_scr = nullptr; ws->sw_scr_bytes = 0;
        hipError_t e = hipMalloc((void **)&ws->d_sw_scr, need);
        if (e != hipSuccess) return fail(SALT_E_NOMEM, std::string("hipMalloc(rescue scratch): ") + hipGetErrorString(e));
        ws->sw_scr_bytes = need;
    }
    launch_sw(ws->ix->view, ws->ix->d_pac, static_cast<const uint8_t *>(d_seqs), static_cast<const uint32_t *>(d_offs), ws->d_req, ws->d_pctl, ws->d_swres,
              ws->d_sw_scr, geom, max_len, st);
    if (ev) HIPCHK(hipEventRecord(ev[9], st));
    launch_pe_final(ws->ix->view, PackGeom::make(max_len), n_pairs, ws->d_pm, static_cast<salt_result_t *>(d_results), ws->d_pairs, ws->d_swres, ws->d_lvtab,
                    ws->d_pcq, ws->d_pctl, ws->heavy_blocks, st);
    if (ev) { HIPCHK(hipEventRecord(ev[10], st)); ws->ev_pe[ti] = 1; }
#ifdef SALT_DIAG
    if (getenv("SALT_GPU_TB_CLOCKS")) {
        PeCtl c; HIPCHK(hipStreamSynchronize(st)); HIPCHK(hipMemcpy(&c, ws->d_pctl, sizeof c, hipMemcpyDeviceToHost)); const uint32_t *t = c.tb_clk;
        if (t[3]) fprintf(stderr, "[k_swtb] %u tracebacks: operands %.1f us, band passes %.1f us, walk + write %.1f us each (s_memtime, 10 ns ticks)\n", t[3],
// ... 63 lines not shown
```

salt_amd/csrc/salt_kernels.h:

```cpp
#pragma once
#include <hip/hip_runtime.h>
#include <cstddef>
#include "../../include/salt_gpu.h"
#include "salt_device.h"

#ifdef SALT_DIAG
#define SALT_DIAG_VAL(x) (x)
#else
#define SALT_DIAG_VAL(x) 0
#endif

namespace salt {

struct PackGeom {
    uint32_t nw8, nw16, nw32, pm_stride, tb_stride;
    __host__ __device__ static PackGeom make(uint32_t max_len)
    {
        if (max_len < 1) max_len = 1;
        PackGeom g; g.nw8 = (max_len + 7) / 8; g.nw16 = (max_len + 15) / 16; g.nw32 = (max_len + 31) / 32;
        g.pm_stride = (2 * g.nw8 + 1 + 3) & ~3u; g.tb_stride = (2 * g.nw16 + 2 * g.nw32 + 1 + 3) & ~3u;
        return g;
    }
};

struct SeedParams {
    uint32_t n_reads, spr;
    int32_t  l_seed, l_overlap;
    uint32_t max_seed;
    int32_t  seed_only_ref;
    int32_t  resolve_unique;
    PackGeom pg;
};

struct AlignParams {
    uint32_t n_reads, spr;
    int32_t  l_seed;
    uint32_t max_locate;
    int32_t  max_hits;
    PackGeom pg;
    int32_t  dbg_stop;
    int32_t  heavy_stop;
    int32_t  all_heavy;
    int32_t  pe;
    uint32_t max_amb;
};
static const uint32_t PE_LOCI_CAP = 0x40000;

void launch_pack(const PackGeom &pg, uint32_t n_reads, const uint8_t *seqs, const uint32_t *offs, uint32_t *pm, uint32_t *tb, hipStream_t st);
void launch_seed(const IndexView &ix, const SeedParams &sp, const uint32_t *tb, uint4 *sai_c, uint4 *sai_r, uint4 *wq, uint32_t *wq_cnt,
                 uint32_t walk_blocks, unsigned long long *ctr, hipStream_t st);
size_t seed_wq_words(uint64_t items);
uint32_t seed_wq_cnt_words();
__device__ __forceinline__ uint32_t sw_pull(uint32_t *head, const uint32_t step, const uint32_t n_first, const uint32_t n_items)
{
    if (n_first >= n_items || n_first + __hip_atomic_load(head, __ATOMIC_RELAXED, __HIP_MEMORY_SCOPE_AGENT) >= n_items) return 0xFFFFFFFFu;
    return n_first + atomicAdd(head, step);
}
struct SeCtl {
    alignas(128) uint32_t light_queued;
    alignas(128) uint32_t gap_slots;
    alignas(128) uint32_t gap_items;
    alignas(128) uint32_t cigar_items;
    alignas(128) uint32_t cigar_head;
    alignas(128) uint32_t pool_used;
    alignas(128) uint32_t ovq_count;
    alignas(128) uint32_t ovq_head;
};
static_assert(sizeof(SeCtl) == 8 * 128 && alignof(SeCtl) == 128, "one control word per 128-byte line");
static const uint32_t QUEUE_RANGES = 64;
struct QueueRange {
    enum { HEAVY, GAP, GAPFIN };
    uint32_t push, pad0[31], heads[3], pad1[29];
};
static_assert(sizeof(QueueRange) == 256 && offsetof(QueueRange, push) == 0 && offsetof(QueueRange, heads) == 128, "k_light's counter, then the heads");
void launch_light(const IndexView &ix, const AlignParams &ap, const uint32_t *pm, const uint8_t *seqs, const uint32_t *offs, const uint4 *sai_c,
                  const uint4 *sai_r, salt_result_t *results, uint32_t *queue, SeCtl *ctl, uint32_t *qseg, QueueRange *ranges, unsigned long long *ctr, hipStream_t st);
size_t queue_words(uint32_t max_reads);
struct GapBufs {
    uint32_t *gq;
    uint32_t *gn;
    uint32_t *goff;
    uint32_t *gloci;
    uint8_t  *ge;
    uint32_t *gitems;
    uint32_t *cq;
    SeCtl *gctl;
    uint32_t cap, pool, items_cap;
    uint32_t *ovq;
    QueueRange *ranges;
};
GapBufs gap_bufs_layout(uint8_t *base, uint32_t cap, SeCtl *gctl, size_t *bytes);
void launch_heavy(const IndexView &ix, const AlignParams &ap, const uint32_t *pm, const uint4 *sai_c,
                  const uint4 *sai_r, salt_result_t *results, const uint32_t *queue, unsigned long long *ctr,
                  uint32_t n_blocks, uint32_t gap_blocks, void *lvtab, const GapBufs &g, uint32_t *ovq, QueueRange *ranges, uint8_t *pe_scr, hipEvent_t *ev3, hipStream_t st);
size_t lv_table_bytes();

static const uint32_t SW_MAX_SEG = 64;
static const uint32_t SW_BAND_W = 1100;
struct SwGeom {
    uint32_t maxcol_bytes, n_blocks;
    uint32_t tb_group_bytes, tb_blocks;
};
SwGeom sw_geom(uint32_t max_len, uint64_t max_window, uint32_t cus);
void sw_geom_limit(SwGeom &g, uint32_t blocks);
uint64_t sw_scratch_bytes(const SwGeom &g);
struct PeSwReq { uint32_t start, end, mate; uint8_t strand, aware; uint16_t pad; };
struct PeSwRes { int32_t score1, score2, ref_begin, ref_end, read_begin, read_end; uint32_t start, strand; uint16_t n_cigar, ok; uint16_t cigar[SALT_MAX_CIGAR_OPS]; };
struct PePair { uint32_t req0; uint8_t n_req; uint8_t rescued[2]; uint8_t pad; };
struct PeCtl {
    uint32_t n_req, unused1;
    uint32_t n_cigar, cigar_head;
    uint32_t overflow;
    uint32_t diag_cols, diag_clk, unused7;
    uint32_t tb_clk[4];
    uint32_t sw_heads[4];
    uint32_t swf1_pending;
};
static_assert(offsetof(PeCtl, n_cigar) == 8 && offsetof(PeCtl, overflow) == 16 && offsetof(PeCtl, diag_cols) == 20 && offsetof(PeCtl, tb_clk) == 32 &&
              offsetof(PeCtl, sw_heads) == 48 && offsetof(PeCtl, swf1_pending) == 64 && sizeof(PeCtl) == 68, "paired-end control words");
void launch_pair(uint32_t n_pairs, uint32_t min_tlen, uint32_t max_tlen, uint32_t l_pac, const uint32_t *offs, salt_result_t *res,
                 PePair *pairs, PeSwReq *req, PeCtl *ctl, hipStream_t st);
void launch_sw(const IndexView &ix, const uint8_t *pac, const uint8_t *seqs, const uint32_t *offs, const PeSwReq *req, PeCtl *ctl,
               PeSwRes *res, uint8_t *scratch, SwGeom g, uint32_t max_len, hipStream_t st);
static const uint32_t SW_MAX_BLOCKS_PER_CU = 16;
static const uint64_t SW_SCRATCH_TOTAL = 2ull << 30;
uint32_t sw_blocks_per_cu(uint32_t max_len);
void launch_pe_final(const IndexView &ix, const PackGeom &pg, uint32_t n_pairs, const uint32_t *pm, salt_result_t *res, const PePair *pairs,
// ... 63 lines not shown
```

Before: 481.9 Mreads/s.

## Epoch-tag reverse SA-interval rows to skip their per-batch default stores

The seed kernel no longer writes a default empty row to sai_r for every item. Each completed reverse row carries a 24-bit batch epoch in its flag word, and readers treat rows with a stale epoch as empty. The buffer is zeroed once on allocation and again when the epoch wraps. This removes one 16-byte global store per seed item, at the cost of an extra compare on every sai_r read. Separately, building the R context records is moved into index attach with a 40 GB free-memory reserve, so r_ctx filtering can be active without set_pac being called.

```diff
diff --git a/include/salt_gpu.h b/include/salt_gpu.h
--- a/include/salt_gpu.h
+++ b/include/salt_gpu.h
@@ -101,6 +101,8 @@
 
 typedef struct { uint32_t min_tlen, max_tlen; } salt_pe_opt_t;
 int  salt_gpu_index_set_pac(salt_gpu_index_t *ix, const uint8_t *pac, uint64_t l_pac);
+int  salt_gpu_index_r_ctx(const salt_gpu_index_t *ix, void **dev_ptr, uint64_t *bytes);
+int  salt_gpu_ws_epoch(const salt_gpu_ws_t *ws, uint32_t *next_epoch);
 int  salt_gpu_align_pe(salt_gpu_ws_t *ws, const salt_aln_opt_t *opt, const salt_pe_opt_t *pe, uint32_t n_pairs,
                        const uint8_t *seqs, const uint32_t *offs, salt_result_t *results);
 int  salt_gpu_align_pe_resident(salt_gpu_ws_t *ws, const salt_aln_opt_t *opt, const salt_pe_opt_t *pe, uint32_t n_pairs,
diff --git a/salt_amd/api.py b/salt_amd/api.py
--- a/salt_amd/api.py
+++ b/salt_amd/api.py
@@ -517,6 +517,20 @@
             done += m
         return res
 
+    def r_ctx(self):
+        lib = gpu_lib()
+        lib.salt_gpu_index_r_ctx.argtypes = [ctypes.c_void_p, ctypes.c_void_p, ctypes.c_void_p]
+        p, n = ctypes.c_void_p(), ctypes.c_uint64()
+        _gpu_check(lib.salt_gpu_index_r_ctx(self._ix, ctypes.byref(p), ctypes.byref(n)))
+        return p.value, n.value
+
+    def epoch(self):
+        lib = gpu_lib()
+        lib.salt_gpu_ws_epoch.argtypes = [ctypes.c_void_p, ctypes.c_void_p]
+        e = ctypes.c_uint32()
+        _gpu_check(lib.salt_gpu_ws_epoch(self._ws, ctypes.byref(e)))
+        return e.value
+
     def set_pac(self, index):
         if not getattr(self, "_pac_set", False):
             pac, l_pac = index.pac()
diff --git a/salt_amd/csrc/salt_align.hip b/salt_amd/csrc/salt_align.hip
--- a/salt_amd/csrc/salt_align.hip
+++ b/salt_amd/csrc/salt_align.hip
@@ -388,7 +388,7 @@
     if (item < n_items) {
         const SeedCtx c = seed_ctx(sp, tb, (uint32_t)item, ix.r_lkt_len);
         cw0 = c.w0; cw1 = c.w1; cw2 = c.w2; cn0 = c.n0; cn1 = c.n1;
-        uint4 oc = make_uint4(1, 0, 0, 0), orr = make_uint4(1, 0, 0, 0);
+        uint4 oc = make_uint4(1, 0, 0, 0);
         if (seed_valid(c)) {
             const uint32_t e = c.s + c.k - 1, W = c.W;
             uint32_t x = 0; bool has_n = false;
@@ -444,7 +444,6 @@
             }
         }
         sai_c[item] = oc;
-        sai_r[item] = orr;
     }
     {
         const uint64_t mr = __ballot(pend_r), mc = __ballot(pend_c);
@@ -523,7 +522,7 @@
         } else if (w.ph != WK_IDLE) {
             done = is_r ? seed_walk_finish<true>(ix, sp, c, w, ld, row, n_occ_r, n_aux) : seed_walk_finish<false>(ix, sp, c, w, ld, row, n_occ_c, n_aux);
         }
-        if (done && row.x <= row.y) (is_r ? sai_r : sai_c)[item] = row;
+        if (done && row.x <= row.y) { if (is_r) { row.w = sai_r_pack(sp.epoch, row.w); sai_r[item] = row; } else sai_c[item] = row; }
         n_sa += (n_aux >> 10) & 2047u; n_text += n_aux >> 21; n_aux = 0;
     }
     if (ctr) {
@@ -676,6 +675,7 @@
     uint32_t ref_len, spr, max_locate, r, L; int strand; bool gap_mode; unsigned long long *phase;
     uint32_t *loci; uint32_t loci_cap; int pe;
     bool finish;
+    uint32_t epoch;
     const uint4 *r_ctx;
     const uint4 *c_ctx; uint32_t ctx_k;
 };
@@ -714,7 +714,7 @@
         uint4 v2[2] = { make_uint4(1, 0, 0, 0), make_uint4(1, 0, 0, 0) };
         if (slot < ap.spr) {
             const u32x4_t tc = sai_c[base_item + slot], tr = sai_r[base_item + slot];
-            v2[0] = make_uint4(tc.x, tc.y, tc.z, tc.w); v2[1] = make_uint4(tr.x, tr.y, tr.z, tr.w);
+            v2[0] = make_uint4(tc.x, tc.y, tc.z, tc.w); v2[1] = sai_r_row(make_uint4(tr.x, tr.y, tr.z, tr.w), a.epoch);
         }
 #pragma unroll
         for (int which = 0; which < 2; ++which) {
@@ -1397,7 +1397,7 @@
     if (!too_short)
     for (int strand = 0; strand < 2; ++strand) {
         pc.stamp(SALT_CTR_T_SCAN);
-        const CandStats cs = build_candidates_call<PE, GL>(CandArgs{ ix.c_sa, ix.r_pos, sai_c, sai_r, ix.ref_len, ap.spr, ap.max_locate, r, L, strand, false, phase, pe_loci, loci_cap, ap.pe, false, ix.r_ctx, ix.c_ctx, ix.ctx_k }, w);
+        const CandStats cs = build_candidates_call<PE, GL>(CandArgs{ ix.c_sa, ix.r_pos, sai_c, sai_r, ix.ref_len, ap.spr, ap.max_locate, r, L, strand, false, phase, pe_loci, loci_cap, ap.pe, false, ap.epoch, ix.r_ctx, ix.c_ctx, ix.ctx_k }, w);
         if (glob) { loci = cs.in_lds ? w.loci : pe_loci; cand_e = cs.in_lds ? w.cand_e : pe_cand; }
         pc.t = phase ? __builtin_amdgcn_s_memtime() : 0;
         const uint32_t n_loc = cs.n_cand; c_sa_c += cs.n_sa_c; c_sa_r += cs.n_sa_r; c_loci += cs.n_loci; c_ctx_rej += cs.n_ctx_rej; c_ctx_rows += cs.n_ctx_rows;
@@ -1445,7 +1445,7 @@
                     uint32_t n = n_loc_s[1];
                     if (strand == 0 || ix.c_ctx != nullptr) {
                         WSYNC();
-                        const CandStats cs = build_candidates_call<PE, GL>(CandArgs{ ix.c_sa, ix.r_pos, sai_c, sai_r, ix.ref_len, ap.spr, ap.max_locate, r, L, strand, true, phase, pe_loci, loci_cap, ap.pe, false, nullptr, nullptr, 0 }, w);
+                        const CandStats cs = build_candidates_call<PE, GL>(CandArgs{ ix.c_sa, ix.r_pos, sai_c, sai_r, ix.ref_len, ap.spr, ap.max_locate, r, L, strand, true, phase, pe_loci, loci_cap, ap.pe, false, ap.epoch, nullptr, nullptr, 0 }, w);
                         if (glob) { loci = cs.in_lds ? w.loci : pe_loci; cand_e = cs.in_lds ? w.cand_e : pe_cand; }
                         c_sa_c += cs.n_sa_c; c_sa_r += cs.n_sa_r; c_loci += cs.n_loci;
                         n = cs.n_cand;
@@ -1496,7 +1496,7 @@
         }
         for (int strand = 0; strand < 2; ++strand) {
             pc.stamp(SALT_CTR_T_GAP);
-            const CandStats cs = build_candidates_call<PE, GL>(CandArgs{ ix.c_sa, ix.r_pos, sai_c, sai_r, ix.ref_len, ap.spr, ap.max_locate, r, L, strand, true, phase, pe_loci, loci_cap, ap.pe, true, nullptr, nullptr, 0 }, w);
+            const CandStats cs = build_candidates_call<PE, GL>(CandArgs{ ix.c_sa, ix.r_pos, sai_c, sai_r, ix.ref_len, ap.spr, ap.max_locate, r, L, strand, true, phase, pe_loci, loci_cap, ap.pe, true, ap.epoch, nullptr, nullptr, 0 }, w);
             if (glob) { loci = cs.in_lds ? w.loci : pe_loci; cand_e = cs.in_lds ? w.cand_e : pe_cand; }
             pc.t = phase ? __builtin_amdgcn_s_memtime() : 0;
             const uint32_t n_cand = cs.n_cand; c_sa_c += cs.n_sa_c; c_sa_r += cs.n_sa_r; c_loci += cs.n_loci;
@@ -1927,7 +1927,7 @@
         {
             const uint32_t l = lane >> 4, slot = lane & 15u;
             uint4 v = make_uint4(1, 0, 0, 0);
-            if (slot < ap.spr) v = ((l & 1) ? sai_r : sai_c)[((uint64_t)r * 2u + (l >> 1)) * ap.spr + slot];
+            if (slot < ap.spr) { v = ((l & 1) ? sai_r : sai_c)[((uint64_t)r * 2u + (l >> 1)) * ap.spr + slot]; if (l & 1) v = sai_r_row(v, ap.epoch); }
             uint32_t sz = v.w ? v.y - v.x + 1u : 0u;
             if (sz > 65u) sz = 65u;
             uint32_t inc = sz;
@@ -2200,7 +2200,7 @@
         {
             const uint32_t l = hl >> 3, slot = hl & 7u;
             uint4 v = make_uint4(1, 0, 0, 0);
-            if (slot < ap.spr) v = ((l & 1) ? sai_r : sai_c)[((uint64_t)r * 2u + (l >> 1)) * ap.spr + slot];
+            if (slot < ap.spr) { v = ((l & 1) ? sai_r : sai_c)[((uint64_t)r * 2u + (l >> 1)) * ap.spr + slot]; if (l & 1) v = sai_r_row(v, ap.epoch); }
             uint32_t sz = v.w ? v.y - v.x + 1u : 0u;
             if (sz > 65u) sz = 65u;
             uint32_t inc = sz;
diff --git a/salt_amd/csrc/salt_device.h b/salt_amd/csrc/salt_device.h
--- a/salt_amd/csrc/salt_device.h
+++ b/salt_amd/csrc/salt_device.h
@@ -34,6 +34,14 @@
     uint32_t ref_len, lkt_len, r_lkt_len;
 };
 
+
+static const uint32_t SAI_EPOCH_MAX = (1u << 24) - 1u;
+__device__ __forceinline__ uint32_t sai_r_pack(uint32_t epoch, uint32_t flag) { return (epoch << 8) | flag; }
+__device__ __forceinline__ uint4 sai_r_row(uint4 v, uint32_t epoch)
+{
+    v.w = (v.w >> 8) == epoch ? v.w & 0xffu : 0u;
+    return v;
+}
 
 __device__ __forceinline__ uint32_t sel4(uint4 v, uint32_t c)
 {
diff --git a/salt_amd/csrc/salt_gpu.hip b/salt_amd/csrc/salt_gpu.hip
--- a/salt_amd/csrc/salt_gpu.hip
+++ b/salt_amd/csrc/salt_gpu.hip
@@ -39,6 +39,7 @@
     uint32_t max_reads = 0; uint64_t max_bases = 0;
     uint8_t *d_seqs = nullptr; uint32_t *d_offs = nullptr; salt_result_t *d_results = nullptr;
     uint4 *d_sai_c = nullptr, *d_sai_r = nullptr; uint64_t sai_cap = 0;
+    uint32_t epoch = 1;
     uint4 *d_wq = nullptr; uint32_t *d_wq_cnt = nullptr; uint32_t walk_blocks = 512; bool no_unique = false;
     uint32_t *d_pm = nullptr, *d_tb = nullptr; uint64_t pm_cap = 0, tb_cap = 0;
     uint8_t *d_heads = nullptr, *h_heads = nullptr;
@@ -100,6 +101,21 @@
 extern "C" const char *salt_gpu_last_error(void) { return g_err.c_str(); }
 extern "C" uint32_t salt_gpu_result_size(void) { return (uint32_t)sizeof(salt_result_t); }
 
+static const uint64_t R_CTX_RESERVE_ATTACH = 40ull << 30;
+static const uint64_t R_CTX_RESERVE_PAC = 32ull << 30;
+static int attach_r_ctx(salt_gpu_index *ix, const uint64_t R_CTX_RESERVE)
+{
+    if (!ix->view.c_ctx || ix->d_rctx || (getenv("SALT_GPU_NO_RCTX") && atoi(getenv("SALT_GPU_NO_RCTX")))) return SALT_OK;
+    const uint64_t rbytes = ((uint64_t)ix->hdr.r_text_len + 1) * 16;
+    size_t free_b = 0, total_b = 0;
+    if (hipMemGetInfo(&free_b, &total_b) == hipSuccess && (uint64_t)free_b >= rbytes + R_CTX_RESERVE && hipMalloc((void **)&ix->d_rctx, rbytes) == hipSuccess) {
+        launch_build_r_ctx(ix->view, ix->hdr.ctx_k, ix->d_rctx, nullptr);
+        if (hipGetLastError() != hipSuccess || hipDeviceSynchronize() != hipSuccess) { hipFree(ix->d_rctx); ix->d_rctx = nullptr; return fail(SALT_E_HIP, "building the R context records failed"); }
+        ix->view.r_ctx = ix->d_rctx;
+    } else { (void)hipGetLastError(); ix->d_rctx = nullptr; }
+    return SALT_OK;
+}
+
 extern "C" int salt_gpu_index_attach(const salt_host_index_t *h, int device, salt_gpu_index_t **out)
 {
     if (!h || !out) return fail(SALT_E_INVAL, "null argument");
@@ -205,6 +221,7 @@
     CHK2(hipDeviceSynchronize());
     hipFree(d_sa_s); hipFree(d_r_sa);
 #undef CHK2
+    if (attach_r_ctx(ix, R_CTX_RESERVE_ATTACH)) g_err.clear();
     *out = ix;
     return SALT_OK;
 }
@@ -253,6 +270,7 @@
     if (ix->hdr.off_ctx) launch_build_c_ctx(ix->view, ix->hdr.ctx_k, reinterpret_cast<uint4 *>(ix->image + ix->hdr.off_ctx), nullptr);
     HIPCHK(hipGetLastError());
     HIPCHK(hipDeviceSynchronize());
+    if (attach_r_ctx(ix, R_CTX_RESERVE_ATTACH)) g_err.clear();
     return SALT_OK;
 }
 
@@ -316,6 +334,7 @@
         ws->gap_blocks = (uint32_t)prop.multiProcessorCount * gap_per_cu;
         ws->walk_blocks = (uint32_t)prop.multiProcessorCount * 2u;
         if (const char *e2 = getenv("SALT_GPU_WALK_PER_CU")) { int v = atoi(e2); if (v > 0 && v <= 16) ws->walk_blocks = (uint32_t)prop.multiProcessorCount * (uint32_t)v; }
+        if (const char *e2 = getenv("SALT_GPU_SAI_EPOCH")) { const long long v = atoll(e2); if (v >= 1 && v <= (long long)SAI_EPOCH_MAX) ws->epoch = (uint32_t)v; }
         if (const char *e2 = getenv("SALT_GPU_NO_UNIQUE")) ws->no_unique = atoi(e2) != 0;
         if (const char *e2 = getenv("SALT_GPU_WALK_BLOCKS")) { int v = atoi(e2); if (v > 0 && v <= 65536) ws->walk_blocks = (uint32_t)v; }
         CHKW(hipMalloc(&ws->d_lvtab, (uint64_t)ws->heavy_blocks * lv_table_bytes()));
@@ -384,6 +403,7 @@
         hipFree(ws->d_sai_c); hipFree(ws->d_sai_r); hipFree(ws->d_wq); ws->d_sai_c = ws->d_sai_r = ws->d_wq = nullptr; ws->sai_cap = 0;
         HIPCHK(hipMalloc((void **)&ws->d_sai_c, items * sizeof(uint4)));
         HIPCHK(hipMalloc((void **)&ws->d_sai_r, items * sizeof(uint4)));
+        HIPCHK(hipMemsetAsync(ws->d_sai_r, 0, items * sizeof(uint4), st));
         HIPCHK(hipMalloc((void **)&ws->d_wq, seed_wq_words(items) * 4));
         ws->sai_cap = items;
     }
@@ -400,8 +420,10 @@
     sp.max_seed = o->max_seed; sp.seed_only_ref = o->seed_only_ref;
     sp.resolve_unique = !ws->no_unique;
     if (n_reads > ws->max_reads) return fail(SALT_E_CAPACITY, "more reads than the workspace holds");
+    if (ws->epoch > SAI_EPOCH_MAX) { HIPCHK(hipMemsetAsync(ws->d_sai_r, 0, ws->sai_cap * sizeof(uint4), st)); ws->epoch = 1; }
+    sp.epoch = ws->epoch++;
     AlignParams ap; ap.pg = pg; ap.n_reads = n_reads; ap.spr = spr; ap.l_seed = o->l_seed; ap.max_locate = o->max_locate; ap.max_hits = o->max_hits;
-    ap.all_heavy = ws->all_heavy; ap.pe = pe; ap.dbg_stop = 0; ap.heavy_stop = 0; ap.max_amb = pe ? 5u : 200u;
+    ap.all_heavy = ws->all_heavy; ap.pe = pe; ap.dbg_stop = 0; ap.heavy_stop = 0; ap.max_amb = pe ? 5u : 200u; ap.epoch = sp.epoch;
 #ifdef SALT_DIAG
     { const char *e = getenv("SALT_GPU_LIGHT_STOP"); ap.dbg_stop = e ? atoi(e) : 0; } { static const int hs = getenv("SALT_GPU_HEAVY_STOP") ? atoi(getenv("SALT_GPU_HEAVY_STOP")) : 0; ap.heavy_stop = hs; }
 #endif
@@ -565,6 +587,7 @@
         hipFree(ws->d_sai_c); hipFree(ws->d_sai_r); hipFree(ws->d_wq); ws->d_sai_c = ws->d_sai_r = ws->d_wq = nullptr; ws->sai_cap = 0;
         HIPCHK(hipMalloc((void **)&ws->d_sai_c, items * sizeof(uint4)));
         HIPCHK(hipMalloc((void **)&ws->d_sai_r, items * sizeof(uint4)));
+        HIPCHK(hipMemsetAsync(ws->d_sai_r, 0, items * sizeof(uint4), st)); HIPCHK(hipStreamSynchronize(st));
         HIPCHK(hipMalloc((void **)&ws->d_wq, seed_wq_words(items) * 4));
         ws->sai_cap = items;
     }
@@ -1455,15 +1478,20 @@
     HIPCHK(hipMemset(ix->d_pac, 0, bytes + 16));
     HIPCHK(hipMemcpy(ix->d_pac, pac, bytes, hipMemcpyHostToDevice));
     ix->l_pac = l_pac;
-    if (ix->view.c_ctx && !ix->d_rctx && !(getenv("SALT_GPU_NO_RCTX") && atoi(getenv("SALT_GPU_NO_RCTX")))) {
-        const uint64_t rbytes = ((uint64_t)ix->hdr.r_text_len + 1) * 16;
-        size_t free_b = 0, total_b = 0;
-        if (hipMemGetInfo(&free_b, &total_b) == hipSuccess && (uint64_t)free_b >= rbytes + (32ull << 30) && hipMalloc((void **)&ix->d_rctx, rbytes) == hipSuccess) {
-            launch_build_r_ctx(ix->view, ix->hdr.ctx_k, ix->d_rctx, nullptr);
-            if (hipGetLastError() != hipSuccess || hipDeviceSynchronize() != hipSuccess) { hipFree(ix->d_rctx); ix->d_rctx = nullptr; return fail(SALT_E_HIP, "building the R context records failed"); }
-            ix->view.r_ctx = ix->d_rctx;
-        } else ix->d_rctx = nullptr;
-    }
+    return attach_r_ctx(ix, R_CTX_RESERVE_PAC);
+}
+
+extern "C" int salt_gpu_index_r_ctx(const salt_gpu_index_t *ix, void **dev_ptr, uint64_t *bytes)
+{
+    if (!ix || !dev_ptr || !bytes) return fail(SALT_E_INVAL, "null argument");
+    *dev_ptr = ix->d_rctx; *bytes = ix->d_rctx ? ((uint64_t)ix->hdr.r_text_len + 1) * 16 : 0;
+    return SALT_OK;
+}
+
+extern "C" int salt_gpu_ws_epoch(const salt_gpu_ws_t *ws, uint32_t *next_epoch)
+{
+    if (!ws || !next_epoch) return fail(SALT_E_INVAL, "null argument");
+    *next_epoch = ws->epoch > SAI_EPOCH_MAX ? 1u : ws->epoch;
     return SALT_OK;
 }
 
diff --git a/salt_amd/csrc/salt_kernels.h b/salt_amd/csrc/salt_kernels.h
--- a/salt_amd/csrc/salt_kernels.h
+++ b/salt_amd/csrc/salt_kernels.h
@@ -29,6 +29,7 @@
     uint32_t max_seed;
     int32_t  seed_only_ref;
     int32_t  resolve_unique;
+    uint32_t epoch;
     PackGeom pg;
 };
 
@@ -43,6 +44,7 @@
     int32_t  all_heavy;
     int32_t  pe;
     uint32_t max_amb;
+    uint32_t epoch;
 };
 static const uint32_t PE_LOCI_CAP = 0x40000;
 
```

Result: faster. 490.0 Mreads/s, median of 6 (+1.7%).
